# kai422/DAS3R

Measured on AMD Instinct MI355X. Metric: render fwd+bwd Msplats/s at 1080p, higher is better.
Workload: dtype f32; 1 GPU; 1M random splats, 1920x1080, SH degree 3, forward+backward (BASELINE.json configs[3], constant P); splats_per_gpu=1000000, splats_per_gpu_final=1000000, init_steps=30, sh_degree=3, num_rendered=2614506, api=GaussianRasterizer.forward + autograd backward (drop-in surface), parallelism=1 independent scenes, one per GPU

## Files before the change

das3r_amd/_lib.py:

```python
import ctypes as C
import os

_HERE = os.path.dirname(os.path.abspath(__file__))
LIB_PATH = os.path.join(_HERE, "libdas3r_hip.so")
ABI_VERSION = 16

ALLOC_FN = C.CFUNCTYPE(C.c_void_p, C.c_void_p, C.c_size_t)


class RasterArgs(C.Structure):
    _fields_ = [("P", C.c_int32), ("sh_degree", C.c_int32), ("M", C.c_int32), ("image_width", C.c_int32),
                ("image_height", C.c_int32), ("tanfovx", C.c_float), ("tanfovy", C.c_float), ("scale_modifier", C.c_float),
                ("bg", C.c_void_p), ("viewmatrix", C.c_void_p), ("projmatrix", C.c_void_p), ("campos", C.c_void_p),
                ("prefiltered", C.c_int32), ("debug", C.c_int32), ("capacity_hint", C.c_int64)]


class PreTransform(C.Structure):
    _fields_ = [("xyz", C.c_void_p), ("rot", C.c_void_p), ("scaling", C.c_void_p), ("opacity_raw", C.c_void_p), ("conf_flat", C.c_void_p),
                ("mask_index", C.c_void_p), ("R", C.c_void_p), ("t", C.c_void_p), ("Lq", C.c_void_p)]


class RasterIn(C.Structure):
    _fields_ = [("means3D", C.c_void_p), ("opacities", C.c_void_p), ("shs", C.c_void_p), ("colors_precomp", C.c_void_p),
                ("scales", C.c_void_p), ("rotations", C.c_void_p), ("cov3D_precomp", C.c_void_p), ("pre", C.POINTER(PreTransform))]


class RasterOut(C.Structure):
    _fields_ = [("out_color", C.c_void_p), ("radii", C.c_void_p), ("out_invdepth", C.c_void_p)]


class RasterSaved(C.Structure):
    _fields_ = [("geom", C.c_void_p), ("binning", C.c_void_p), ("img", C.c_void_p), ("num_rendered", C.c_int64), ("capacity", C.c_int64),
                ("check_word", C.c_void_p), ("check_tag", C.c_uint32), ("flags", C.c_uint32)]


class AdamSlot(C.Structure):
    _fields_ = [("param", C.c_void_p), ("exp_avg", C.c_void_p), ("exp_avg_sq", C.c_void_p), ("step_size", C.c_float), ("bc2_sqrt", C.c_float)]


class Chain(C.Structure):
    _fields_ = [("g_conf_flat", C.c_void_p), ("g_small", C.c_void_p), ("slots", C.POINTER(AdamSlot)), ("beta1", C.c_float), ("beta2", C.c_float),
                ("eps", C.c_float)]


class RasterGrads(C.Structure):
    _fields_ = [("dL_dmeans2D", C.c_void_p), ("dL_dopacities", C.c_void_p), ("dL_dmeans3D", C.c_void_p),
                ("dL_dshs", C.c_void_p), ("dL_dcolors_precomp", C.c_void_p), ("dL_dscales", C.c_void_p),
                ("dL_drotations", C.c_void_p), ("dL_dcov3D", C.c_void_p), ("scratch", C.c_void_p), ("chain", C.POINTER(Chain))]


class RasterLayout(C.Structure):
    _fields_ = [(n, C.c_size_t) for n in
                ("geom_bytes", "binning_bytes", "img_bytes", "depth_key", "xy", "conic_opacity", "rgbd", "splat_stride", "clamped",
                 "tiles_touched", "sorted_idx", "offsets", "point_list", "final_T", "n_contrib", "ranges")]


EXPORTS = ("das3r_raster_forward", "das3r_raster_backward", "das3r_raster_backward_depth", "das3r_raster_backward_depth_scratch_bytes", "das3r_raster_check", "das3r_raster_backward_scratch_bytes", "das3r_mark_visible", "das3r_knn3_workspace_bytes",
           "das3r_knn3_mean_dist2", "das3r_raster_get_layout", "das3r_abi_version", "das3r_last_error", "das3r_reload_switches", "das3r_get_stats",
           "das3r_raster_forget_shapes", "das3r_raster_learning",
           "das3r_profile_enable", "das3r_profile_report", "das3r_pretransform_forward", "das3r_pretransform_backward", "das3r_pose_matrices", "das3r_pose_chain",
           "das3r_adam_step", "das3r_adam_step_gated", "das3r_photometric_blocks", "das3r_photometric_forward", "das3r_photometric_backward",
           "das3r_has_experiments", "das3r_pair_counters", "das3r_debug_poison_lds", "das3r_debug_inject_fault", "das3r_debug_mutate",
           "das3r_pose_matrices_qt", "das3r_pose_chain_qt", "das3r_photometric_finish", "das3r_pretransform_backward_adam", "das3r_pretransform_pose_sums",
           "das3r_raster_count_live_pairs", "das3r_photometric_backward_finish", "das3r_pose_chain_qt_rearm", "das3r_ssim_map_forward", "das3r_ssim_map_backward")

_lib = None


def load():
    global _lib
    if _lib is not None:
        return _lib
    if not os.path.exists(LIB_PATH):
        raise RuntimeError(
            f"das3r_amd: HIP library not found at {LIB_PATH}. Build it with `python -c 'import __graft_entry__ as g; "
            f"g.build()'` or `make -C das3r_amd/csrc`. There is no CPU fallback.")
    L = C.CDLL(LIB_PATH)
    for name in EXPORTS:
        if not hasattr(L, name):
            raise RuntimeError(f"das3r_amd: {LIB_PATH} does not export {name}; rebuild it")
    L.das3r_abi_version.restype = C.c_int
    if L.das3r_abi_version() != ABI_VERSION:
        raise RuntimeError("das3r_amd: ABI version mismatch between the Python host layer and libdas3r_hip.so; rebuild")
    L.das3r_last_error.restype = C.c_char_p
    L.das3r_raster_forward.restype = C.c_int64
    L.das3r_raster_forward.argtypes = [C.POINTER(RasterArgs), C.POINTER(RasterIn), C.POINTER(RasterOut), ALLOC_FN, ALLOC_FN,
                                       ALLOC_FN, C.c_void_p, C.POINTER(RasterSaved), C.c_void_p]
    L.das3r_raster_backward.restype = C.c_int
    L.das3r_raster_backward.argtypes = [C.POINTER(RasterArgs), C.POINTER(RasterIn), C.POINTER(RasterSaved), C.c_void_p,
                                        C.POINTER(RasterGrads), C.c_void_p]
    L.das3r_raster_backward_scratch_bytes.restype = C.c_size_t
    L.das3r_raster_backward_depth.restype = C.c_int
    L.das3r_raster_backward_depth.argtypes = [C.POINTER(RasterArgs), C.POINTER(RasterIn), C.POINTER(RasterSaved), C.c_void_p, C.c_void_p,
                                              C.POINTER(RasterGrads), C.c_void_p]
    L.das3r_raster_backward_depth_scratch_bytes.restype = C.c_size_t
    L.das3r_raster_backward_depth_scratch_bytes.argtypes = [C.c_int64]
    L.das3r_raster_backward_scratch_bytes.argtypes = [C.c_int64]
    L.das3r_raster_check.restype = C.c_int
    L.das3r_raster_check.argtypes = [C.POINTER(RasterSaved), C.c_void_p]
    L.das3r_mark_visible.restype = C.c_int
    L.das3r_mark_visible.argtypes = [C.c_int32, C.c_void_p, C.c_void_p, C.c_void_p, C.c_void_p, C.c_void_p]
    L.das3r_knn3_workspace_bytes.restype = C.c_size_t
    L.das3r_knn3_workspace_bytes.argtypes = [C.c_int32]
    L.das3r_knn3_mean_dist2.restype = C.c_int
    L.das3r_knn3_mean_dist2.argtypes = [C.c_int32, C.c_void_p, C.c_void_p, C.c_void_p, C.c_void_p]
    L.das3r_pose_matrices.restype = C.c_int
    L.das3r_pose_matrices.argtypes = [C.c_void_p, C.c_void_p, C.c_void_p]
    L.das3r_pose_chain.restype = C.c_int
    L.das3r_pose_chain.argtypes = [C.c_void_p, C.c_void_p, C.c_void_p, C.c_void_p]
    L.das3r_pretransform_forward.restype = C.c_int
    L.das3r_pretransform_forward.argtypes = [C.c_int32] + [C.c_void_p] * 13 + [C.c_void_p]
    L.das3r_pretransform_backward.restype = C.c_int
    L.das3r_pretransform_backward.argtypes = [C.c_int32] + [C.c_void_p] * 18 + [C.c_void_p]
    L.das3r_pretransform_backward_adam.restype = C.c_int
    L.das3r_pretransform_backward_adam.argtypes = [C.c_int32] + [C.c_void_p] * 10 + [C.POINTER(AdamSlot), C.c_float, C.c_float, C.c_float, C.c_void_p]
    L.das3r_pretransform_pose_sums.restype = C.c_int
    L.das3r_pretransform_pose_sums.argtypes = [C.c_int32] + [C.c_void_p] * 7 + [C.c_void_p]
    L.das3r_photometric_blocks.restype = C.c_int64
    L.das3r_photometric_blocks.argtypes = [C.c_int32, C.c_int32]
    L.das3r_photometric_forward.restype = C.c_int
    L.das3r_photometric_forward.argtypes = [C.c_int32, C.c_int32, C.c_void_p, C.c_void_p, C.c_void_p, C.c_float, C.c_void_p, C.c_void_p, C.c_void_p]
    L.das3r_photometric_backward.restype = C.c_int
    L.das3r_photometric_backward.argtypes = [C.c_int32, C.c_int32, C.c_void_p, C.c_void_p, C.c_void_p, C.c_float, C.c_void_p, C.c_void_p,
                                             C.c_void_p, C.c_void_p, C.c_void_p]
    L.das3r_pose_matrices_qt.restype = C.c_int
    L.das3r_pose_matrices_qt.argtypes = [C.c_void_p, C.c_void_p, C.c_void_p, C.c_void_p]
    L.das3r_pose_chain_qt.restype = C.c_int
    L.das3r_pose_chain_qt.argtypes = [C.c_void_p, C.c_void_p, C.c_void_p, C.c_void_p, C.c_void_p]
    L.das3r_pose_chain_qt_rearm.restype = C.c_int
    L.das3r_pose_chain_qt_rearm.argtypes = [C.c_void_p, C.c_void_p, C.c_void_p, C.c_void_p, C.c_void_p, C.c_void_p, C.c_void_p]
    L.das3r_ssim_map_forward.restype = C.c_int
    L.das3r_ssim_map_forward.argtypes = [C.c_int32, C.c_int32, C.c_void_p, C.c_void_p, C.c_void_p, C.c_void_p, C.c_void_p, C.c_void_p]
    L.das3r_ssim_map_backward.restype = C.c_int
    L.das3r_ssim_map_backward.argtypes = [C.c_int32, C.c_int32, C.c_void_p, C.c_void_p, C.c_void_p, C.c_void_p, C.c_void_p, C.c_void_p, C.c_void_p]
    L.das3r_photometric_backward_finish.restype = C.c_int
    L.das3r_photometric_backward_finish.argtypes = [C.c_int32, C.c_int32, C.c_void_p, C.c_void_p, C.c_void_p, C.c_float, C.c_void_p, C.c_void_p,
                                                    C.c_void_p, C.c_void_p, C.c_void_p, C.c_void_p, C.c_void_p]
    L.das3r_photometric_finish.restype = C.c_int
    L.das3r_photometric_finish.argtypes = [C.c_int32, C.c_int32, C.c_void_p, C.c_float, C.c_void_p, C.c_void_p]
    L.das3r_adam_step_gated.restype = C.c_int
    L.das3r_adam_step_gated.argtypes = [C.c_int32, C.c_void_p, C.c_float, C.c_float, C.c_float, C.c_void_p, C.c_float, C.c_void_p, C.c_void_p]
    L.das3r_adam_step.restype = C.c_int
    L.das3r_adam_step.argtypes = [C.c_int32, C.c_void_p, C.c_float, C.c_float, C.c_float, C.c_void_p]
    L.das3r_raster_get_layout.restype = C.c_int
    L.das3r_raster_get_layout.argtypes = [C.c_int32, C.c_int64, C.c_int32, C.c_int32, C.POINTER(RasterLayout)]
    _lib = L
    return L


def reload_switches():
    L = load()
    L.das3r_reload_switches.restype = None
    L.das3r_reload_switches.argtypes = []
    L.das3r_reload_switches()


def has_experiments():
    L = load()
# ... 110 lines not shown
```

das3r_amd/csrc/api.hip:

```cpp
#include <stdarg.h>
#include <string.h>

#include <vector>

#include "common.h"
#include <algorithm>

namespace das3r {

static thread_local char g_err[512] = "";

void set_error(const char *fmt, ...) {
    va_list ap;
    va_start(ap, fmt);
    vsnprintf(g_err, sizeof(g_err), fmt, ap);
    va_end(ap);
}

struct ProfRec {
    const char *name;
    hipEvent_t start, stop;
};
static bool g_prof_on = false;
static std::vector<ProfRec> g_prof;
bool profile_enabled() { return g_prof_on; }
static std::vector<hipEvent_t> g_event_pool;
static hipEvent_t pooled_event() {
    if (!g_event_pool.empty()) { hipEvent_t e = g_event_pool.back(); g_event_pool.pop_back(); return e; }
    hipEvent_t e = nullptr;
    return hipEventCreate(&e) == hipSuccess ? e : nullptr;
}
void profile_begin(const char *name, hipStream_t s) {
    ProfRec r;
    r.name = name;
    r.start = pooled_event();
    r.stop = pooled_event();
    if (!r.start || !r.stop) return;
    (void)hipEventRecord(r.start, s);
    g_prof.push_back(r);
}
void profile_end(hipStream_t s) {
    if (!g_prof.empty()) (void)hipEventRecord(g_prof.back().stop, s);
}

static Switches g_sw;
static bool g_sw_loaded = false;
static int g_inject_fault = 0;
static int g_mutate = 0;
static void load_switches() {
    Switches w;
    memset(&w, 0, sizeof(w));
    auto env = [](const char *k) -> const char * { const char *e = getenv(k); return (e && e[0]) ? e : nullptr; };
    const char *e;
#ifdef DAS3R_EXPERIMENTS
    if ((e = env("DAS3R_SORT_IPL"))) { const int v = atoi(e); w.sort_ipl = (v == 4 || v == 8 || v == 16) ? v : 0; }
    w.sort_classic = (e = env("DAS3R_SORT")) && e[0] == 'c';
    w.no_sh_stage = getenv("DAS3R_NO_SH_STAGE") != nullptr;
    if ((e = env("DAS3R_ABLATE"))) { w.ablate_set = true; w.ablate = atoi(e); }
    if ((e = env("DAS3R_BWD_PAD_LDS"))) w.bwd_pad_lds = atoi(e);
    if ((e = env("DAS3R_FWD_PAD_LDS"))) w.fwd_pad_lds = atoi(e);
    if ((e = env("DAS3R_SCAN_ITEMS"))) { const int v = atoi(e); w.scan_items = (v == 1 || v == 2 || v == 4 || v == 8 || v == 16) ? v : 0; }
    w.fwd_no_prefetch = (e = env("DAS3R_FWD_PREFETCH")) && e[0] == '0';
#endif
    w.rect_upstream = (e = env("DAS3R_RECT")) && e[0] == 'u';
    w.verbose = env("DAS3R_VERBOSE") != nullptr;
    if ((e = env("DAS3R_BINNING"))) w.binning = e[0] == 'l' ? 1 : (e[0] == 'r' ? -1 : (e[0] == 's' ? (strchr(e, '3') ? 3 : 2) : 0));
    w.capacity_exact = (e = env("DAS3R_CAPACITY")) && e[0] == 'e';
    w.fused_emit_off = (e = env("DAS3R_FUSED_EMIT")) && e[0] == '0';
    w.tile_lpt_off = (e = env("DAS3R_TILE_LPT")) && e[0] == '0';
    if ((e = env("DAS3R_RENDER"))) w.render_fwd = e[0] == 'q' ? 1 : (e[0] == 'r' ? 2 : (e[0] == 'l' ? 3 : (e[0] == 's' ? 4 : (e[0] == 'f' ? 5 : 0))));
    if ((e = env("DAS3R_RENDER_BWD"))) {
        w.render_bwd = e[0] == 'd' ? 1 : (e[0] == 'm' ? 2 : (strncmp(e, "stream", 6) == 0 ? 5 : (e[0] == 's' ? 3 : (e[0] == 'b' ? 6 : (e[0] == 'f' ? 7 : 0)))));
        if (w.render_bwd == 6) {
            const char *d = e;
            while (*d && (*d < '0' || *d > '9')) d++;
            w.render_bwd_mb = *d ? atoi(d) : 128;
            const char *pp = strchr(e, 'p');
            w.render_bwd_pix = pp ? atoi(pp + 1) : 0;
            const char *po = strchr(e, 'o');
            w.render_bwd_occ = po ? atoi(po + 1) : 5;
        }
        if (w.render_bwd == 7) {
            const char *d = e;
            while (*d && (*d < '0' || *d > '9')) d++;
            w.render_bwd_mb = *d ? atoi(d) : 128;
            w.render_bwd_pix = strchr(e, 'q') ? 9 : (strchr(e, 's') ? 8 : 0);
        }
        if (w.render_bwd == 3) {
            const char *d = e;
            while (*d && (*d < '0' || *d > '9')) d++;
            w.render_bwd_mb = (*d ? atoi(d) : 256) + (strncmp(e, "scana", 5) == 0 ? 1000 : 0);
        }
    }
    if ((e = env("DAS3R_BWD_REDUCE"))) { w.bwd_reduce_set = true; w.bwd_reduce_shfl = e[0] == 's'; }
    w.tickets = -1;
    if ((e = env("DAS3R_TICKETS"))) w.tickets = e[0] == 'a' ? 0 : (e[0] == 'n' ? 1 << 30 : ((e[0] >= '1' && e[0] <= '9') ? atoi(e) : -1));
    w.deterministic = (e = env("DAS3R_DETERMINISTIC")) && e[0] != '0';
    w.bwd_buckets = -1;
    if ((e = env("DAS3R_BWD_BUCKETS"))) w.bwd_buckets = atoi(e);
    w.tile_strip = 8;
    w.tile_chunk = -1;
    if ((e = env("DAS3R_TILE_CHUNK"))) { const int v = atoi(e); w.tile_chunk = (v >= 0 && v <= 64 && (v & (v - 1)) == 0) ? v : -1; }
    if ((e = env("DAS3R_TILE_STRIP"))) w.tile_strip = std::max(0, std::min(63, atoi(e)));
    w.inject_fault = g_inject_fault;
    w.mutate = g_mutate;
    g_sw = w;
    __atomic_store_n(&g_sw_loaded, true, __ATOMIC_RELEASE);
}
const Switches &switches() {
    if (!__atomic_load_n(&g_sw_loaded, __ATOMIC_ACQUIRE)) load_switches();
    return g_sw;
}

constexpr int MAX_DEVICES = 64;
static int g_threads_on_device[MAX_DEVICES] = {};
struct ThreadRegistrar {
    bool on[MAX_DEVICES] = {};
    void add(int dev) {
        if (!on[dev]) { on[dev] = true; __atomic_fetch_add(&g_threads_on_device[dev], 1, __ATOMIC_RELAXED); }
    }
    ~ThreadRegistrar() {
        for (int d = 0; d < MAX_DEVICES; d++)
            if (on[d]) __atomic_fetch_sub(&g_threads_on_device[d], 1, __ATOMIC_RELAXED);
    }
};
static thread_local ThreadRegistrar g_registrar;
bool grid_is_resident(int nblocks) {
    const int forced = switches().tickets;
    int dev = 0;
    if (hipGetDevice(&dev) != hipSuccess || dev < 0 || dev >= MAX_DEVICES) return false;
    const bool shared = __atomic_load_n(&g_threads_on_device[dev], __ATOMIC_RELAXED) > 1;
    if (forced >= 0) {
        static bool warned = false;
        if (shared && forced > 0 && !__atomic_exchange_n(&warned, true, __ATOMIC_RELAXED))
            fprintf(stderr, "[das3r] DAS3R_TICKETS is set to a bound while several host threads render on device %d: ticket-free chained "
                            "kernels are only safe when a grid has the device to itself\n", dev);
        return nblocks <= forced;
    }
    if (shared) return false;
    static thread_local int cached_dev = -1, cached_limit = 0;
    if (dev != cached_dev) {
        int cus = 0;
        if (hipDeviceGetAttribute(&cus, hipDeviceAttributeMultiprocessorCount, dev) != hipSuccess) return false;
        cached_dev = dev;
        cached_limit = cus * 2;
    }
    return nblocks <= cached_limit;
}

int sort_ipl_override() { return switches().sort_ipl; }
#ifdef DAS3R_EXPERIMENTS
bool use_onesweep() { return !switches().sort_classic; }
#else
bool use_onesweep() { return true; }
#endif
bool use_tight_rect() { return !switches().rect_upstream; }

void compute_layout(int P, int64_t I, int W, int H, Layout *L) {
    memset(L, 0, sizeof(*L));
    const size_t Pn = P > 0 ? (size_t)P : 1, In = I > 0 ? (size_t)I : 1;
    L->capacity = I;
    L->tiles_x = (W + TILE_X - 1) / TILE_X;
    L->tiles_y = (H + TILE_Y - 1) / TILE_Y;
    L->ntiles = L->tiles_x * L->tiles_y;
    L->tbits = tile_bits(L->ntiles);
    L->tile_passes = (L->tbits + 7) / 8;
    L->dbits = 0;
    L->kbits = L->tbits;
    L->kshift = 0;
    L->part_passes = L->tile_passes;
    L->chunksP = sort_num_chunks(P);
    L->chunksI = sort_num_chunks(I);
    size_t o = 0;
    auto take = [&](size_t b) { size_t r = o; o += align_up(b); return r; };
    L->g_keyA = take(4 * Pn);
    L->g_keyB = take(4 * Pn);
    L->g_valA = take(4 * Pn);
    L->g_valB = take(4 * Pn);
    L->pub.sorted_idx = L->g_valA;
    L->pub.depth_key = L->g_keyA;
    L->pub.xy = take(16 * SPLAT_REC * Pn);
    L->pub.conic_opacity = L->pub.xy + 16;
    L->pub.rgbd = L->pub.xy + 32;
    L->pub.splat_stride = 16 * SPLAT_REC;
    L->pub.clamped = take(Pn);
    L->pub.tiles_touched = take(4 * Pn);
    L->pub.offsets = take(4 * Pn);
    L->g_hist = take(4 * (size_t)RADIX_SIZE * (size_t)(L->chunksP > 0 ? L->chunksP : 1));
    L->g_totals = take(4 * RADIX_SIZE);
    L->g_blocksums = take(4 * (size_t)div_up((int64_t)Pn, 4096));
    L->g_count = take(256);
    L->g_off_by_gid = take(4 * Pn);
    L->g_rect = take(4 * Pn);
    L->g_dhist = take(4 * 256);
    L->g_ghist = take(4 * 4 * RADIX_SIZE);
    L->g_ticket = take(256);
    L->g_status = take(onesweep_status_bytes((int64_t)Pn, 4));
    L->g_scan_status = take(scan_status_bytes((int)Pn));
    L->g_ctrl_bytes = o - L->g_ghist;
    L->pub.geom_bytes = o;
    o = 0;
    L->b_keyA = take(4 * In);
    L->b_keyB = take(4 * In);
    L->b_valA = take(4 * In);
    L->b_valB = take(4 * In);
    L->b_hist = take(4 * (size_t)RADIX_SIZE * (size_t)(L->chunksI > 0 ? L->chunksI : 1));
    L->b_totals = take(4 * RADIX_SIZE);
    L->b_gid_of = take(4 * In);
    L->b_slot = take(4 * In);
    L->b_e2 = take(4 * In);
    L->b_ghist = take(4 * 4 * RADIX_SIZE);
    L->b_ticket = take(256);
    L->b_status = take(onesweep_status_bytes((int64_t)In, L->tile_passes + 1));
    L->b_ctrl_bytes = o - L->b_ghist;
    L->b_ckpt = take(((size_t)In / BUCKET + (size_t)(L->ntiles > 0 ? L->ntiles : 1) + 2) * 256 * 16);
    L->pub.binning_bytes = o;
    const size_t npix_d = (size_t)W * (size_t)H;
    L->d_ckpt = take(((size_t)In / BUCKET + (size_t)(L->ntiles > 0 ? L->ntiles : 1) + 2) * 256 * 16);
    L->d_recs = take(16 * SPLAT_REC * Pn);
    L->d_dpix = take(4 * 3 * (npix_d > 0 ? npix_d : 1));
    L->d_bg = take(16);
    L->d_dz = take(4 * Pn);
    L->d_bytes = o;
    L->pub.point_list = (L->tile_passes & 1) ? L->b_valB : L->b_valA;
    o = 0;
    const size_t npix = (size_t)W * (size_t)H;
    L->pub.final_T = take(4 * (npix > 0 ? npix : 1));
    L->pub.n_contrib = take(4 * (npix > 0 ? npix : 1));
    L->pub.ranges = take(8 * (size_t)(L->ntiles > 0 ? L->ntiles : 1));
    L->i_order = take(4 * (size_t)(L->ntiles > 0 ? L->ntiles : 1));
    L->pub.img_bytes = o;
}

static bool dhist_slots(hipStream_t s, uint32_t **use, uint32_t **next) {
    struct Slot { int dev; hipStream_t stream; uint32_t *buf; uint32_t turn; };
    static thread_local std::vector<Slot> slots;
    int dev = 0;
    if (hipGetDevice(&dev) != hipSuccess) return false;
    Slot *e = nullptr;
    for (auto &c : slots)
        if (c.dev == dev && c.stream == s) e = &c;
    if (!e) {
        uint32_t *buf = nullptr;
        if (hipMalloc((void **)&buf, 2 * 256 * sizeof(uint32_t)) != hipSuccess) return false;
        if (hipMemsetAsync(buf, 0, 2 * 256 * sizeof(uint32_t), s) != hipSuccess) return false;
        slots.push_back(Slot{dev, s, buf, 0u});
        e = &slots.back();
    }
    e->turn++;
    *use = e->buf + 256 * (e->turn & 1u);
    *next = e->buf + 256 * ((e->turn + 1u) & 1u);
    return true;
}

static int validate(const das3r_raster_args *a, const das3r_raster_in *in) {
    if (!a || !in) { set_error("null args"); return DAS3R_ERR_INVALID_ARG; }
    if (a->P < 0 || a->image_width <= 0 || a->image_height <= 0) { set_error("bad extents P=%d W=%d H=%d", a->P, a->image_width, a->image_height); return DAS3R_ERR_INVALID_ARG; }
    if ((int64_t)((a->image_width + TILE_X - 1) / TILE_X) * ((a->image_height + TILE_Y - 1) / TILE_Y) >= (1ll << 22)) {
        set_error("image of %d x %d pixels has 2^22 tiles or more", a->image_width, a->image_height);
        return DAS3R_ERR_INVALID_ARG;
    }
    if (a->P == 0) return DAS3R_OK;
    if (!a->bg || !a->viewmatrix || !a->projmatrix || !a->campos) { set_error("bg/viewmatrix/projmatrix/campos must be device pointers"); return DAS3R_ERR_INVALID_ARG; }
    if (in->pre) {
        const das3r_pretransform *p = in->pre;
        if (!p->xyz || !p->rot || !p->scaling || !p->opacity_raw || !p->conf_flat || !p->R || !p->t || !p->Lq) { set_error("das3r_raster_in.pre: xyz / rot / scaling / opacity_raw / conf_flat / R / t / Lq are required"); return DAS3R_ERR_INVALID_ARG; }
        if (in->cov3D_precomp) { set_error("das3r_raster_in.pre excludes cov3D_precomp"); return DAS3R_ERR_INVALID_ARG; }
    } else if (!in->means3D || !in->opacities) { set_error("means3D/opacities are required"); return DAS3R_ERR_INVALID_ARG; }
    if ((in->shs != nullptr) == (in->colors_precomp != nullptr)) { set_error("Please provide excatly one of either SHs or precomputed colors!"); return DAS3R_ERR_INVALID_ARG; }
    const bool sr = in->pre != nullptr || (in->scales != nullptr && in->rotations != nullptr);
    if ((!in->pre && (in->scales != nullptr) != (in->rotations != nullptr)) || sr == (in->cov3D_precomp != nullptr)) {
        set_error("Please provide exactly one of either scale/rotation pair or precomputed 3D covariance!");
        return DAS3R_ERR_INVALID_ARG;
    }
    if (in->shs) {
        if (a->sh_degree < 0 || a->sh_degree > 3) { set_error("sh_degree must be 0..3 (got %d)", a->sh_degree); return DAS3R_ERR_INVALID_ARG; }
        if (a->M < (a->sh_degree + 1) * (a->sh_degree + 1) || a->M > 16) { set_error("M=%d incompatible with sh_degree=%d (need (D+1)^2 <= M <= 16)", a->M, a->sh_degree); return DAS3R_ERR_INVALID_ARG; }
    }
    if (a->tanfovx <= 0.f || a->tanfovy <= 0.f) { set_error("tanfov must be positive"); return DAS3R_ERR_INVALID_ARG; }
    return DAS3R_OK;
}

}

using namespace das3r;

extern "C" int das3r_abi_version(void) { return DAS3R_ABI_VERSION; }
extern "C" void das3r_reload_switches(void) { load_switches(); }
extern "C" void das3r_debug_inject_fault(uint32_t bits) {
    g_inject_fault = (int)bits;
    load_switches();
}
extern "C" void das3r_debug_mutate(uint32_t what) {
    g_mutate = (int)what;
    load_switches();
}
extern "C" const char *das3r_last_error(void) { return g_err; }

extern "C" int das3r_raster_get_layout(int32_t P, int64_t num_rendered, int32_t W, int32_t H, das3r_raster_layout *out) {
    if (!out || P < 0 || num_rendered < 0 || W <= 0 || H <= 0) { set_error("das3r_raster_get_layout: invalid argument"); return DAS3R_ERR_INVALID_ARG; }
    Layout L;
    compute_layout(P, num_rendered, W, H, &L);
    *out = L.pub;
    return DAS3R_OK;
}

struct Mailbox {
    volatile uint32_t *host = nullptr;
    uint32_t *dev = nullptr;
    uint32_t seq = 0;
};
constexpr uint32_t CHECK_SLOTS = 16, CHECK_WORD0 = 16, MAILBOX_BYTES = 4 * (CHECK_WORD0 + 2 * CHECK_SLOTS);
constexpr uint32_t CROWDED16 = 23u * 16u;
struct Verdict { int P, W, H; int64_t last_I, peak_I; int radix_left, backoff; uint32_t gen; int seg_extra; bool last_seg; bool fine; uint32_t forwards; uint32_t clean; uint32_t longest; };
struct PerDevice {
    Mailbox mb;
    uint32_t pending[CHECK_SLOTS] = {};
    unsigned long long *arrive_ring = nullptr;
    Verdict verdict = {0, 0, 0, -1, 0, 0, 64, 0};
    bool pending_fine = false, pending_valid = false;
    uint32_t pending_forwards = 0;
    char *emit_ring = nullptr;
    bool emit_ring_dirty = false;
    uint32_t emit_last_tag = 0;
};
static int per_device(PerDevice **out) {
    static thread_local PerDevice state[MAX_DEVICES];
    int dev = 0;
    HIP_TRY(hipGetDevice(&dev));
    if (dev < 0 || dev >= MAX_DEVICES) { set_error("device ordinal %d not supported", dev); return DAS3R_ERR_INVALID_ARG; }
    PerDevice &T = state[dev];
    g_registrar.add(dev);
    if (!T.mb.host) {
        uint32_t *h = nullptr;
        HIP_TRY(hipHostMalloc((void **)&h, MAILBOX_BYTES, hipHostMallocMapped));
        memset(h, 0, MAILBOX_BYTES);
        HIP_TRY(hipHostGetDevicePointer((void **)&T.mb.dev, h, 0));
        T.mb.host = h;
    }
    *out = &T;
    return DAS3R_OK;
}
static int mailbox_wait(Mailbox *mb, int idx, uint32_t tag, hipStream_t s) {
    for (long spins = 0; spins < 200000000L; spins++) {
        if (__atomic_load_n(&mb->host[idx], __ATOMIC_ACQUIRE) == tag) return DAS3R_OK;
        __builtin_ia32_pause();
        if ((spins & 0xFFFFF) == 0xFFFFF && hipStreamQuery(s) != hipErrorNotReady) break;
    }
    HIP_TRY(hipStreamSynchronize(s));
    if (__atomic_load_n(&mb->host[idx], __ATOMIC_ACQUIRE) == tag) return DAS3R_OK;
    set_error("the device never delivered the result of this forward to the host mailbox");
    return DAS3R_ERR_HIP;
}

static unsigned long long g_stats[4] = {0, 0, 0, 0};
static void stat_add(int i) { __atomic_fetch_add(&g_stats[i], 1ull, __ATOMIC_RELAXED); }
static int examine_check_slot(volatile uint32_t *slot, uint32_t tag, bool wait, hipStream_t s) {
    uint32_t seen = __atomic_load_n(&slot[1], __ATOMIC_ACQUIRE);
    if (seen != tag && wait) {
        for (long spins = 0; spins < 200000000L && seen != tag; spins++) {
            __builtin_ia32_pause();
            seen = __atomic_load_n(&slot[1], __ATOMIC_ACQUIRE);
            if ((spins & 0xFFFFF) == 0xFFFFF && hipStreamQuery(s) != hipErrorNotReady) break;
        }
        if (seen != tag) {
            HIP_TRY(hipStreamSynchronize(s));
            seen = __atomic_load_n(&slot[1], __ATOMIC_ACQUIRE);
        }
    }
    if (seen != tag) return 1;
    const uint32_t all_flags = slot[0], flags = all_flags & ~16u;
    if (all_flags & 0x80000000u) return DAS3R_OK;
    stat_add(1);
    if (all_flags & 16u) stat_add(2);
    if (flags) stat_add(3);
    if ((all_flags & 16u) && switches().verbose) fprintf(stderr, "das3r: a look-back poll needed the read-modify-write path\n");
    if (flags) {
        slot[0] = all_flags | 0x80000000u;
        set_error("a forward's binning failed its self-check (flags 0x%x); its output is invalid", flags);
        return DAS3R_ERR_HIP;
    }
    return DAS3R_OK;
}

extern "C" int das3r_raster_check(const das3r_raster_saved *saved, das3r_stream_t stream) {
    if (!saved) { set_error("das3r_raster_check: null saved state"); return DAS3R_ERR_INVALID_ARG; }
    if (!saved->check_word || !saved->check_tag) return DAS3R_OK;
    const int r = examine_check_slot((volatile uint32_t *)saved->check_word, saved->check_tag, true, (hipStream_t)stream);
    return r < 0 ? r : DAS3R_OK;
}

extern "C" int das3r_raster_forget_shapes(void) {
    PerDevice *T = nullptr;
    int r = per_device(&T);
    if (r) return r;
    const uint32_t gen = T->verdict.gen;
    T->verdict = Verdict{0, 0, 0, -1, 0, 0, 64, gen};
    return DAS3R_OK;
}

extern "C" int das3r_raster_learning(int32_t set, uint32_t state[2]) {
    if (!state) { set_error("das3r_raster_learning: invalid argument"); return DAS3R_ERR_INVALID_ARG; }
    PerDevice *T = nullptr;
    int r = per_device(&T);
    if (r) return r;
    if (!set) {
        state[0] = T->verdict.fine ? 1u : 0u;
        state[1] = T->verdict.forwards;
        return DAS3R_OK;
    }
    const uint32_t gen = T->verdict.gen;
    T->verdict = Verdict{0, 0, 0, -1, 0, 0, 64, gen};
    T->pending_fine = state[0] != 0u;
    T->pending_forwards = state[1];
    T->pending_valid = true;
    return DAS3R_OK;
}

extern "C" void das3r_get_stats(uint64_t out[4]) {
    for (int i = 0; i < 4; i++) out[i] = (uint64_t)__atomic_load_n(&g_stats[i], __ATOMIC_RELAXED);
}

extern "C" int64_t das3r_raster_forward(const das3r_raster_args *a, const das3r_raster_in *in, const das3r_raster_out *out,
                                        das3r_alloc_fn alloc_geom, das3r_alloc_fn alloc_binning, das3r_alloc_fn alloc_img,
                                        void *user, das3r_raster_saved *saved, das3r_stream_t stream) {
    hipStream_t s = (hipStream_t)stream;
    stat_add(0);
    int rc = validate(a, in);
    if (rc) return rc;
    if (!out || !out->out_color || (a->P > 0 && !out->radii) || !alloc_geom || !alloc_binning || !alloc_img || !saved) {
        set_error("das3r_raster_forward: null output/allocator");
        return DAS3R_ERR_INVALID_ARG;
    }
    if (out->out_invdepth && switches().render_fwd == 4) {
        set_error("das3r_raster_forward: DAS3R_RENDER=slices has no inverse-depth form (das3r_raster_out.out_invdepth)");
        return DAS3R_ERR_INVALID_ARG;
    }
    const int P = a->P, W = a->image_width, H = a->image_height;
    const bool depth = out->out_invdepth != nullptr;
    Layout L;
    compute_layout(P, 0, W, H, &L);
    saved->geom = alloc_geom(user, L.pub.geom_bytes);
    saved->img = alloc_img(user, L.pub.img_bytes);
    saved->binning = nullptr;
    saved->num_rendered = 0;
    saved->capacity = 0;
    saved->check_word = nullptr;
    saved->check_tag = 0;
    saved->flags = 0;
    if (!saved->geom || !saved->img) { set_error("scratch allocation failed (geom %zu B, img %zu B)", L.pub.geom_bytes, L.pub.img_bytes); return DAS3R_ERR_ALLOC; }
    if (P == 0) {
        HIP_TRY(hipMemsetAsync(out->out_color, 0, sizeof(float) * 3 * (size_t)W * H, s));
        if (out->out_invdepth) HIP_TRY(hipMemsetAsync(out->out_invdepth, 0, sizeof(float) * (size_t)W * H, s));
        HIP_TRY(hipMemsetAsync(saved->img + L.pub.ranges, 0, 8 * (size_t)L.ntiles, s));
        saved->binning = alloc_binning(user, 256);
        return 0;
    }
    PerDevice *T = nullptr;
    if ((rc = per_device(&T))) return rc;
    Mailbox *mb = &T->mb;
    auto check_slot = [&](uint32_t i, bool wait) -> int {
        if (!T->pending[i]) return DAS3R_OK;
        const int r = examine_check_slot(mb->host + CHECK_WORD0 + 2 * i, T->pending[i], wait, s);
        if (r == 1) return DAS3R_OK;
        T->pending[i] = 0;
        return r;
    };
    for (uint32_t i = 0; i < CHECK_SLOTS; i++)
        if ((rc = check_slot(i, false))) return rc;
    uint32_t late_tag = 0;
    unsigned long long *&arrive_ring = T->arrive_ring;
    constexpr uint32_t ARRIVE_SLOTS = 16, ARRIVE_WORDS = 8 + 64 * 8;
    if (!arrive_ring) {
        HIP_TRY(hipMalloc((void **)&arrive_ring, ARRIVE_SLOTS * ARRIVE_WORDS * sizeof(unsigned long long)));
        HIP_TRY(hipMemsetAsync(arrive_ring, 0, ARRIVE_SLOTS * ARRIVE_WORDS * sizeof(unsigned long long), s));
        HIP_TRY(hipStreamSynchronize(s));
    }
    Verdict &verdict = T->verdict;
    constexpr int64_t LOCAL_AVG = 384;
    const uint32_t too_long = mb->host[10];
    if (too_long) mb->host[10] = 0;
    const uint32_t want_bits = mb->host[11];
    if (want_bits) mb->host[11] = 0;
    if (verdict.P != P || verdict.W != W || verdict.H != H) {
        const uint32_t gen = verdict.gen + 1u ? verdict.gen + 1u : 1u;
        verdict = Verdict{P, W, H, -1, 0, 0, 64, gen};
        if (T->pending_valid) {
            verdict.fine = T->pending_fine;
            verdict.forwards = T->pending_forwards;
            T->pending_valid = false;
        }
    }
    const bool decide_fine = (verdict.forwards++ & 511u) == 0u;
    auto next_gen = [&]() { verdict.gen = verdict.gen + 1u ? verdict.gen + 1u : 1u; };
    if (verdict.last_I < 0) {
    } else if (too_long == verdict.gen && !(verdict.last_seg && verdict.seg_extra == 0 && L.tile_passes < 3 && seg_dbits(L, L.tile_passes + 1) > 0)) {
        if (verdict.clean >= 256u) verdict.backoff = 64;
        verdict.radix_left = verdict.backoff;
        if (verdict.backoff < 4096) verdict.backoff *= 2;
        verdict.clean = 0;
        next_gen();
    } else if (too_long == verdict.gen || want_bits == verdict.gen) {
        verdict.seg_extra = 1;
        next_gen();
    }
    const int forced = switches().binning;
    bool local = use_onesweep() && (forced == 1 || (forced == 0 && verdict.radix_left == 0 && verdict.last_I <= LOCAL_AVG * L.ntiles));
    constexpr int64_t SEG_AVG = 384;
    const int seg_passes = L.tile_passes + ((forced == 3 || (forced == 0 && verdict.seg_extra)) ? 1 : 0);
    const int seg_bits = (use_onesweep() && seg_passes <= 3) ? seg_dbits(L, seg_passes) : 0;
    bool seg = !local && seg_bits > 0 && (forced >= 2 || (forced == 0 && verdict.radix_left == 0 && verdict.last_I >= 0 &&
                                                           (verdict.last_I >> std::min(seg_bits, 20)) <= SEG_AVG * L.ntiles));
    const uint32_t *seg_dhist = nullptr;
    auto apply_seg = [&]() {
        L.dhist_ptr = seg_dhist;
        if (seg) {
            L.dbits = seg_bits;
            L.kbits = L.tbits + seg_bits;
            L.kshift = std::min(16, 32 - L.kbits);
            L.part_passes = seg_passes;
        }
    };
    verdict.last_seg = seg;
    if (local || seg) verdict.clean++;
    if (forced == 0 && verdict.radix_left > 0) verdict.radix_left--;
    const uint32_t count_tag = ++mb->seq ? mb->seq : ++mb->seq;
    unsigned long long *arrive = arrive_ring + (size_t)(count_tag % ARRIVE_SLOTS) * ARRIVE_WORDS;
    auto bin_and_render = [&](int64_t cap, bool local_order, bool ctrl_zeroed, uint32_t *count_out = nullptr, uint32_t count_out_tag = 0,
                              uint32_t *emit_slot = nullptr ) -> int {
        int r;
        const bool fused_scan = use_onesweep();
        const bool seg = L.dbits > 0;
        if (!emit_slot) {
            if (fused_scan) {
                if ((r = launch_binning_scan_emit(P, cap, out->radii, saved->geom, saved->binning, L, ctrl_zeroed, count_out, count_out_tag, a->debug != 0,
                                                  s, local_order || seg))) return r;
            } else if ((r = launch_scan(P, saved->geom, L, nullptr, 0, a->debug != 0, s))) return r;
        }
        uint32_t *host_late = nullptr;
        if (cap > 0) {
            late_tag = ++mb->seq ? mb->seq : ++mb->seq;
            const uint32_t slot = late_tag % CHECK_SLOTS;
            if ((r = check_slot(slot, true))) return r;
            T->pending[slot] = late_tag;
            host_late = mb->dev + CHECK_WORD0 + 2 * slot;
            saved->check_word = (void *)(mb->host + CHECK_WORD0 + 2 * slot);
            saved->check_tag = late_tag;
        }
        uint32_t *dead_keys = nullptr;
        if ((r = launch_binning(P, cap, W, H, out->radii, saved->geom, saved->binning, saved->img, L, fused_scan, host_late, late_tag,
                                a->debug != 0, s, &dead_keys, emit_slot, mb->dev + 10, verdict.gen))) return r;
        LocalBin lb = {(float4 *)(saved->binning + L.b_ckpt), nullptr, nullptr, nullptr, nullptr, verdict.gen, (uint32_t)(P - 1), (uint32_t)cap};
        if (decide_fine && cap > 0 && use_quad_lanes(L, lb)) {
            const uint32_t tag = ++mb->seq ? mb->seq : ++mb->seq;
            if ((r = launch_list_skew(saved->img, saved->binning, saved->geom, L, (uint32_t)cap, (uint32_t)(P - 1), mb->dev + 13, tag, a->debug != 0, s))) return r;
            if ((r = mailbox_wait(mb, 14, tag, s))) return r;
            const int64_t longest = (int64_t)mb->host[13], mean = (verdict.last_I > 0 ? verdict.last_I : cap) / std::max(L.ntiles, 1);
            verdict.longest = (uint32_t)longest;
            const uint32_t crowd16 = mb->host[15];
            verdict.fine = (longest > mean + (mean * 4) / 5 && longest >= 4096) || crowd16 >= CROWDED16;
            if (switches().verbose) fprintf(stderr, "[das3r] tile lists: longest %lld, mean %lld, %.1f of 64 consecutive entries in one quadrant -> %s kernels\n", (long long)longest,
                                            (long long)mean, crowd16 / 16.0, verdict.fine ? "2x2-region" : "block");
        }
        lb.prefer_regions = verdict.fine;
        lb.tile_order = nullptr;
        if (verdict.fine && cap > 0 && use_quad_lanes(L, lb) && L.ntiles <= 1024 && !switches().tile_lpt_off && (switches().render_fwd == 0 || switches().render_fwd == 5)) {
            if ((r = launch_tile_lpt(saved->img, L, (uint32_t)cap, a->debug != 0, s))) return r;
            lb.tile_order = (const uint32_t *)(saved->img + L.i_order);
        }
        if (verdict.fine && cap > 0 && use_quad_lanes(L, lb)) {
            const uint32_t hint = std::min<uint32_t>(63u, verdict.longest / (uint32_t)BUCKET + 2u);
            saved->flags |= 1u | (hint << 8);
        }
        if (local_order && cap > 0) {
            lb.point_list = (uint32_t *)(saved->binning + L.pub.point_list);
            lb.slot_list = (uint32_t *)(saved->binning + L.b_slot);
            lb.keys = dead_keys;
            lb.host_flag = mb->dev + 10;
        }
        return launch_render_forward(a, in->colors_precomp, out->out_color, saved->geom, saved->binning, saved->img, L, lb, s, out->out_invdepth,
                                     depth ? (float4 *)(saved->binning + L.d_ckpt) : nullptr);
    };
    auto prefiltered_ok = [&]() -> int {
        if (!a->prefiltered || mb->host[12] != count_tag) return DAS3R_OK;
        set_error("Point is filtered although prefiltered is set. This shouldn't happen!");
        return DAS3R_ERR_INVALID_ARG;
    };
    int64_t I, cap;
    if ((local || seg) && verdict.last_I >= 0 && a->capacity_hint != -1 && !switches().capacity_exact) {
        cap = std::max(verdict.last_I + verdict.last_I / 4, verdict.peak_I + verdict.peak_I / 20) + 4096;
        if (cap > (int64_t)0x7FFFFF00) cap = (int64_t)0x7FFFFF00;
        compute_layout(P, cap, W, H, &L);
        apply_seg();
        saved->binning = alloc_binning(user, depth ? L.d_bytes : L.pub.binning_bytes);
        if (!saved->binning) { set_error("scratch allocation failed (binning %zu B)", L.pub.binning_bytes); return DAS3R_ERR_ALLOC; }
        char *&emit_ring = T->emit_ring;
        bool &emit_ring_dirty = T->emit_ring_dirty;
        uint32_t &emit_last_tag = T->emit_last_tag;
        constexpr size_t EMIT_SLOT_BYTES = sizeof(uint32_t) * EMIT_SLOT_WORDS + sizeof(unsigned long long) * EMIT_STATUS_GRANULES;
        const bool fused_emit = local && grid_is_resident(div_up(P, 256)) && !switches().fused_emit_off;
        uint32_t *emit_slot = nullptr;
        if (fused_emit) {
            if (!emit_ring) {
                HIP_TRY(hipMalloc((void **)&emit_ring, ARRIVE_SLOTS * EMIT_SLOT_BYTES));
                emit_ring_dirty = true;
            }
            if (emit_ring_dirty || count_tag < emit_last_tag) {
                HIP_TRY(hipMemsetAsync(emit_ring, 0, ARRIVE_SLOTS * EMIT_SLOT_BYTES, s));
                emit_ring_dirty = false;
            }
            emit_last_tag = count_tag;
            emit_slot = (uint32_t *)(emit_ring + (size_t)(count_tag % ARRIVE_SLOTS) * EMIT_SLOT_BYTES);
            const EmitArgs em = {(unsigned long long *)(emit_slot + EMIT_SLOT_WORDS), count_tag, emit_slot + 64, emit_slot,
                                 (uint32_t *)(saved->binning + L.b_keyA), (uint32_t *)(saved->binning + L.b_gid_of),
                                 (uint32_t *)(saved->geom + L.g_off_by_gid), (uint32_t)cap, L.tbits, (uint32_t *)(saved->geom + L.g_count), mb->dev};
            emit_ring_dirty = true;
            if ((rc = launch_preprocess(a, in, out->radii, saved->geom, saved->img, saved->binning + L.b_ghist, L.b_ctrl_bytes, L, nullptr, mb->dev,
                                        count_tag, s, &em))) return rc;
            if ((rc = bin_and_render(cap, true, true, nullptr, 0, emit_slot))) return rc;
            emit_ring_dirty = false;
        } else {
            uint32_t *dhist = nullptr, *dhist_next = nullptr;
            if (seg && !dhist_slots(s, &dhist, &dhist_next)) {
                dhist = (uint32_t *)(saved->geom + L.g_dhist);
                HIP_TRY(hipMemsetAsync(dhist, 0, 4 * 256, s));
            }
            seg_dhist = dhist;
            apply_seg();
            if ((rc = launch_preprocess(a, in, out->radii, saved->geom, saved->img, saved->binning + L.b_ghist, L.b_ctrl_bytes, L, nullptr, mb->dev,
                                        count_tag, s, nullptr, dhist, dhist_next))) return rc;
            if ((rc = bin_and_render(cap, local, true, mb->dev, count_tag))) return rc;
        }
        if ((rc = mailbox_wait(mb, 2, count_tag, s))) return rc;
        if ((rc = prefiltered_ok())) return rc;
        I = (int64_t)mb->host[0];
        if (I > (int64_t)0x7FFFFF00) { set_error("num_rendered %lld exceeds 2^31", (long long)I); return DAS3R_ERR_OVERFLOW; }
        verdict.last_I = I;
        verdict.peak_I = std::max(I, verdict.peak_I - verdict.peak_I / 1024);
        if (I > cap) {
            cap = I;
            compute_layout(P, cap, W, H, &L);
            saved->binning = alloc_binning(user, depth ? L.d_bytes : L.pub.binning_bytes);
            if (!saved->binning) { set_error("scratch allocation failed (binning %zu B)", L.pub.binning_bytes); return DAS3R_ERR_ALLOC; }
            apply_seg();
            HIP_TRY(hipMemsetAsync(saved->geom + L.g_ghist, 0, L.g_ctrl_bytes, s));
            HIP_TRY(hipMemsetAsync(saved->img + L.pub.ranges, 0, 8 * (size_t)L.ntiles, s));
            if ((rc = bin_and_render(cap, local, false))) return rc;
        }
    } else {
        uint32_t *dhist = nullptr, *dhist_next = nullptr;
        if (seg && !dhist_slots(s, &dhist, &dhist_next)) {
            dhist = (uint32_t *)(saved->geom + L.g_dhist);
            HIP_TRY(hipMemsetAsync(dhist, 0, 4 * 256, s));
        }
        seg_dhist = dhist;
        if ((rc = launch_preprocess(a, in, out->radii, saved->geom, saved->img, nullptr, 0, L, arrive, mb->dev, count_tag, s, nullptr, dhist, dhist_next))) return rc;
        if (!local && !seg && (rc = launch_depth_sort(P, saved->geom, L, 0, nullptr, 0, a->debug != 0, s))) return rc;
        if ((rc = mailbox_wait(mb, 2, count_tag, s))) return rc;
        if ((rc = prefiltered_ok())) return rc;
        I = cap = (int64_t)mb->host[0];
        if (cap > (int64_t)0x7FFFFF00) { set_error("num_rendered %lld exceeds 2^31", (long long)cap); return DAS3R_ERR_OVERFLOW; }
        verdict.last_I = I;
        verdict.peak_I = std::max(I, verdict.peak_I - verdict.peak_I / 1024);
        if (local && forced == 0 && I > LOCAL_AVG * L.ntiles) {
            local = false;
            if ((rc = launch_depth_sort(P, saved->geom, L, 0, nullptr, 0, a->debug != 0, s))) return rc;
        }
        compute_layout(P, cap, W, H, &L);
        apply_seg();
        saved->binning = alloc_binning(user, depth ? L.d_bytes : L.pub.binning_bytes);
        if (!saved->binning) { set_error("scratch allocation failed (binning %zu B)", L.pub.binning_bytes); return DAS3R_ERR_ALLOC; }
        if (!local && !seg && (rc = launch_depth_sort(P, saved->geom, L, 1, saved->binning + L.b_ghist, L.b_ctrl_bytes, a->debug != 0, s))) return rc;
        if ((rc = bin_and_render(cap, local, !local && !seg))) return rc;
    }
    if (a->debug && late_tag && (rc = check_slot(late_tag % CHECK_SLOTS, true))) return rc;
    saved->num_rendered = I;
    saved->capacity = cap;
    if (depth) saved->flags |= DEPTH_SAVED_FLAG;
    return I;
}

extern "C" int das3r_raster_backward(const das3r_raster_args *a, const das3r_raster_in *in, const das3r_raster_saved *saved,
                                     const float *dL_dpix, const das3r_raster_grads *g, das3r_stream_t stream) {
    hipStream_t s = (hipStream_t)stream;
    int rc = validate(a, in);
    if (rc) return rc;
    const int P = a->P;
    if (P == 0) return DAS3R_OK;
    const bool chained = g && g->chain;
    if (!saved || !saved->geom || !saved->img || !dL_dpix || !g || !g->dL_dmeans2D || (!chained && (!g->dL_dopacities || !g->dL_dmeans3D)) ||
        (saved && saved->num_rendered > 0 && !g->scratch)) {
        set_error("das3r_raster_backward: null saved state / gradient buffer");
        return DAS3R_ERR_INVALID_ARG;
    }
    const bool has_sh = in->shs != nullptr, has_cov = in->cov3D_precomp != nullptr;
    if ((has_sh && !g->dL_dshs) || (!has_sh && !g->dL_dcolors_precomp) || (has_cov && !g->dL_dcov3D) ||
        (!has_cov && !chained && (!g->dL_dscales || !g->dL_drotations))) {
        set_error("das3r_raster_backward: gradient buffer missing for a provided input");
        return DAS3R_ERR_INVALID_ARG;
    }
    if ((rc = das3r_raster_check(saved, stream))) return rc;
    Layout L;
    compute_layout(P, saved->capacity > 0 ? saved->capacity : saved->num_rendered, a->image_width, a->image_height, &L);
    float *partial = g->scratch;
    bool quad_rows = false;
    if (saved->num_rendered > 0) {
        if (!saved->binning) { set_error("das3r_raster_backward: binning buffer missing"); return DAS3R_ERR_INVALID_ARG; }
        if ((rc = launch_render_backward(a, dL_dpix, saved->geom, saved->binning, saved->img, L, partial, s, &quad_rows, saved->num_rendered, saved->flags))) return rc;
    }
    return launch_preprocess_backward(a, in, saved->geom, saved->binning, L, g, partial, s, quad_rows);
}

extern "C" int das3r_raster_backward_depth(const das3r_raster_args *a, const das3r_raster_in *in, const das3r_raster_saved *saved,
                                           const float *dL_dpix, const float *dL_dinvdepth, const das3r_raster_grads *g, das3r_stream_t stream) {
    hipStream_t s = (hipStream_t)stream;
    int rc = validate(a, in);
    if (rc) return rc;
    const int P = a->P;
    if (P == 0) return DAS3R_OK;
    const bool chained = g && g->chain;
    if (!saved || !saved->geom || !saved->img || !dL_dpix || !dL_dinvdepth || !g || !g->dL_dmeans2D || (!chained && (!g->dL_dopacities || !g->dL_dmeans3D)) ||
        (saved->num_rendered > 0 && !g->scratch)) {
        set_error("das3r_raster_backward_depth: null saved state / upstream gradient / gradient buffer");
        return DAS3R_ERR_INVALID_ARG;
    }
    if (!(saved->flags & DEPTH_SAVED_FLAG)) {
        set_error("das3r_raster_backward_depth: the saved state is not that of a forward with out_invdepth (das3r_raster_saved.flags bit 1 is clear)");
        return DAS3R_ERR_INVALID_ARG;
    }
    const bool has_sh = in->shs != nullptr, has_cov = in->cov3D_precomp != nullptr;
    if ((has_sh && !g->dL_dshs) || (!has_sh && !g->dL_dcolors_precomp) || (has_cov && !g->dL_dcov3D) ||
        (!has_cov && !chained && (!g->dL_dscales || !g->dL_drotations))) {
        set_error("das3r_raster_backward_depth: gradient buffer missing for a provided input");
        return DAS3R_ERR_INVALID_ARG;
    }
    const int kind = switches().render_bwd;
    if (kind == 2 || kind == 3 || kind == 5) {
        set_error("das3r_raster_backward_depth: DAS3R_RENDER_BWD=%s has no inverse-depth form", kind == 3 ? "scan" : (kind == 2 ? "mfma" : "stream"));
        return DAS3R_ERR_INVALID_ARG;
    }
    if ((rc = das3r_raster_check(saved, stream))) return rc;
    Layout L;
    compute_layout(P, saved->capacity > 0 ? saved->capacity : saved->num_rendered, a->image_width, a->image_height, &L);
    float *partial = g->scratch;
    const float *dz = nullptr;
    bool quad_rows = false;
    if (saved->num_rendered > 0) {
        if (!saved->binning) { set_error("das3r_raster_backward_depth: binning buffer missing"); return DAS3R_ERR_INVALID_ARG; }
        const size_t c = L.capacity > 0 ? (size_t)L.capacity : 1;
        float *partial_depth = (float *)((char *)g->scratch + align_up(c * 9 * sizeof(float) + 16));
        if ((rc = launch_render_backward(a, dL_dpix, saved->geom, saved->binning, saved->img, L, partial, s, &quad_rows, saved->num_rendered, saved->flags))) return rc;
        if ((rc = launch_depth_pass_inputs(P, a->image_width * a->image_height, saved->geom, L, saved->binning, dL_dinvdepth, s, a->debug != 0))) return rc;
        Layout Ld = L;
        Ld.pub.xy = L.d_recs;
        Ld.pub.conic_opacity = L.d_recs + 16;
        Ld.pub.rgbd = L.d_recs + 32;
        Ld.b_ckpt = L.d_ckpt;
        das3r_raster_args ad = *a;
        ad.bg = (const float *)(saved->binning + L.d_bg);
        bool quad_rows_d = false;
        if ((rc = launch_render_backward(&ad, (const float *)(saved->binning + L.d_dpix), saved->binning, saved->binning, saved->img, Ld, partial_depth, s,
                                         &quad_rows_d, saved->num_rendered, saved->flags))) return rc;
        float *dzw = (float *)(saved->binning + L.d_dz);
        if ((rc = launch_depth_fold(P, saved->geom, L, partial, partial_depth, dzw, s, a->debug != 0))) return rc;
        dz = dzw;
    }
    return launch_preprocess_backward(a, in, saved->geom, saved->binning, L, g, partial, s, quad_rows, dz);
}

extern "C" size_t das3r_raster_backward_depth_scratch_bytes(int64_t capacity) {
    const size_t c = capacity > 0 ? (size_t)capacity : 1;
    return align_up(c * 9 * sizeof(float) + 16) + c * 9 * sizeof(float) + 16;
}

extern "C" size_t das3r_raster_backward_scratch_bytes(int64_t capacity) {
    const size_t c = capacity > 0 ? (size_t)capacity : 1;
#ifdef DAS3R_EXPERIMENTS
    if (switches().render_bwd == 5) return std::max(c * 9 * sizeof(float) + 16, stream_scratch_bytes(capacity));
#endif
    return c * 9 * sizeof(float) + 16;
}

extern "C" int das3r_has_experiments(void) {
#ifdef DAS3R_EXPERIMENTS
    return 1;
#else
    return 0;
#endif
}

extern "C" int das3r_mark_visible(int32_t P, const float *means3D, const float *viewmatrix, const float *projmatrix,
                                  uint8_t *present, das3r_stream_t stream) {
    (void)projmatrix;
    if (P < 0 || (P > 0 && (!means3D || !viewmatrix || !present))) { set_error("das3r_mark_visible: invalid argument"); return DAS3R_ERR_INVALID_ARG; }
    return launch_mark_visible(P, means3D, viewmatrix, present, (hipStream_t)stream);
}

__global__ void __launch_bounds__(1024) poison_lds_kernel(uint32_t pattern, uint32_t *sink, int words) {
    extern __shared__ uint32_t lds_words[];
    for (int i = threadIdx.x; i < words; i += 1024) lds_words[i] = pattern;
    __syncthreads();
    if (lds_words[(threadIdx.x * 37) % words] != pattern) *sink = 1u;
}
extern "C" int das3r_debug_poison_lds(uint32_t pattern, das3r_stream_t stream) {
    static uint32_t *sinks[MAX_DEVICES] = {};
    int dev = 0, lds_bytes = 0;
    HIP_TRY(hipGetDevice(&dev));
    if (dev < 0 || dev >= MAX_DEVICES) { set_error("device ordinal %d not supported", dev); return DAS3R_ERR_INVALID_ARG; }
    HIP_TRY(hipDeviceGetAttribute(&lds_bytes, hipDeviceAttributeMaxSharedMemoryPerBlock, dev));
    const int words = lds_bytes / 4 - 64;
    if (words <= 0) { set_error("das3r_debug_poison_lds: no LDS"); return DAS3R_ERR_HIP; }
    if (!sinks[dev]) HIP_TRY(hipMalloc((void **)&sinks[dev], 4));
    HIP_TRY(hipFuncSetAttribute((const void *)poison_lds_kernel, hipFuncAttributeMaxDynamicSharedMemorySize, words * 4));
    hipLaunchKernelGGL(poison_lds_kernel, dim3(1024), dim3(1024), words * 4, (hipStream_t)stream, pattern, sinks[dev], words);
    HIP_TRY(hipGetLastError());
    return DAS3R_OK;
}

static unsigned long long *g_pairs = nullptr;
static int g_pairs_dev = -1;
namespace das3r {
unsigned long long *pair_counters() {
    if (!g_pairs) return nullptr;
    int dev = -1;
    return (hipGetDevice(&dev) == hipSuccess && dev == g_pairs_dev) ? g_pairs : nullptr;
}
}
extern "C" int das3r_pair_counters(int enable, uint64_t out[4]) {
    if (enable) {
        int dev = 0;
        HIP_TRY(hipGetDevice(&dev));
        if (g_pairs && dev != g_pairs_dev) { set_error("das3r_pair_counters: already counting on device %d", g_pairs_dev); return DAS3R_ERR_INVALID_ARG; }
        if (!g_pairs) HIP_TRY(hipMalloc((void **)&g_pairs, (4 + PHASE_WORDS * PHASE_COPIES) * sizeof(unsigned long long)));
        g_pairs_dev = dev;
        HIP_TRY(hipMemset(g_pairs, 0, (4 + PHASE_WORDS * PHASE_COPIES) * sizeof(unsigned long long)));
        HIP_TRY(hipDeviceSynchronize());
        return DAS3R_OK;
    }
    if (g_pairs) {
        HIP_TRY(hipDeviceSynchronize());
        if (out) HIP_TRY(hipMemcpy(out, g_pairs, 4 * sizeof(unsigned long long), hipMemcpyDeviceToHost));
        HIP_TRY(hipFree(g_pairs));
        g_pairs = nullptr;
    } else if (out) {
        out[0] = out[1] = out[2] = out[3] = 0;
    }
    return DAS3R_OK;
}

extern "C" int das3r_raster_count_live_pairs(const das3r_raster_args *a, const das3r_raster_saved *saved, uint64_t out[2], das3r_stream_t stream) {
    if (!a || !saved || !out) { set_error("das3r_raster_count_live_pairs: null argument"); return DAS3R_ERR_INVALID_ARG; }
    out[0] = out[1] = 0;
    if (a->P == 0 || saved->num_rendered <= 0) return DAS3R_OK;
    if (!saved->geom || !saved->binning || !saved->img) { set_error("das3r_raster_count_live_pairs: saved buffers missing"); return DAS3R_ERR_INVALID_ARG; }
    hipStream_t s = (hipStream_t)stream;
    Layout L;
    compute_layout(a->P, saved->capacity > 0 ? saved->capacity : saved->num_rendered, a->image_width, a->image_height, &L);
    unsigned long long *dev = nullptr;
    HIP_TRY(hipMalloc((void **)&dev, 2 * sizeof(unsigned long long)));
    int rc = DAS3R_OK;
    if (hipMemsetAsync(dev, 0, 2 * sizeof(unsigned long long), s) != hipSuccess) rc = DAS3R_ERR_HIP;
    if (!rc) rc = launch_count_live_pairs(a, saved->geom, saved->binning, saved->img, L, dev, s);
    if (!rc && (hipStreamSynchronize(s) != hipSuccess || hipMemcpy(out, dev, 2 * sizeof(unsigned long long), hipMemcpyDeviceToHost) != hipSuccess)) {
        set_error("das3r_raster_count_live_pairs: device error");
        rc = DAS3R_ERR_HIP;
    }
    (void)hipFree(dev);
    return rc;
}

#ifdef DAS3R_EXPERIMENTS
static unsigned long long *g_trace = nullptr;
namespace das3r { unsigned long long *wg_trace() { return g_trace; } }
extern "C" int das3r_debug_wg_trace(int enable, uint64_t *out) {
    const size_t words = (size_t)TRACE_PASSES * TRACE_WGS * TRACE_STAMPS;
    if (enable) {
        if (!g_trace) HIP_TRY(hipMalloc((void **)&g_trace, words * 8));
        HIP_TRY(hipMemset(g_trace, 0, words * 8));
        HIP_TRY(hipDeviceSynchronize());
        return DAS3R_OK;
    }
    if (g_trace) {
        HIP_TRY(hipDeviceSynchronize());
        if (out) HIP_TRY(hipMemcpy(out, g_trace, words * 8, hipMemcpyDeviceToHost));
        HIP_TRY(hipFree(g_trace));
        g_trace = nullptr;
    }
    return DAS3R_OK;
}
extern "C" int das3r_debug_phase_clocks(uint64_t out[16]) {
    for (int i = 0; i < PHASE_WORDS; i++) out[i] = 0;
    if (!g_pairs) return DAS3R_OK;
    HIP_TRY(hipDeviceSynchronize());
    std::vector<unsigned long long> all(PHASE_WORDS * PHASE_COPIES);
    HIP_TRY(hipMemcpy(all.data(), g_pairs + 4, all.size() * sizeof(unsigned long long), hipMemcpyDeviceToHost));
    for (size_t i = 0; i < all.size(); i++) out[i % PHASE_WORDS] += all[i];
// ... 31 lines not shown
```

das3r_amd/csrc/common.h:

```cpp
#pragma once
#include <hip/hip_runtime.h>
#include <stdint.h>
#include <stdio.h>

#include "../../include/das3r_raster.h"
#include "pretransform_math.h"

#define TILE_X 16
#define TILE_Y 16
#define TILE_PIX 256
#define WAVE 64
#define NEAR_PLANE 0.001f

namespace das3r {

void set_error(const char *fmt, ...);

struct Switches {
    int sort_ipl;
    bool sort_classic;
    bool rect_upstream;
    bool verbose;
    int binning;
    bool capacity_exact;
    bool fused_emit_off;
    bool no_sh_stage;
    int render_fwd;
    int render_bwd;
    int render_bwd_mb;
    int tile_chunk;
    int scan_items;
    bool deterministic;
    int render_bwd_occ;
    bool tile_lpt_off;
    int render_bwd_pix;
    bool bwd_reduce_set, bwd_reduce_shfl;
    bool ablate_set;
    int ablate;
    int tickets;
    int bwd_pad_lds, fwd_pad_lds;
    int bwd_buckets;
    int inject_fault;
    int mutate;
    bool fwd_no_prefetch;
    int tile_strip;
};
const Switches &switches();

#define HIP_TRY(expr)                                                                          \
    do {                                                                                       \
        hipError_t _e = (expr);                                                                \
        if (_e != hipSuccess) {                                                                \
            das3r::set_error("%s failed: %s (%s:%d)", #expr, hipGetErrorString(_e), __FILE__, __LINE__); \
            return DAS3R_ERR_HIP;                                                              \
        }                                                                                      \
    } while (0)

#define KERNEL_CHECK(stream, debug, name)                                                      \
    do {                                                                                       \
        hipError_t _e = hipGetLastError();                                                     \
        if (_e == hipSuccess && (debug)) _e = hipStreamSynchronize(stream);                    \
        if (_e != hipSuccess) {                                                                \
            das3r::set_error("kernel %s failed: %s", name, hipGetErrorString(_e));             \
            return DAS3R_ERR_HIP;                                                              \
        }                                                                                      \
    } while (0)

bool profile_enabled();
void profile_begin(const char *name, hipStream_t s);
void profile_end(hipStream_t s);
struct ProfTimer {
    hipStream_t s;
    bool on;
    ProfTimer(const char *name, hipStream_t stream) : s(stream), on(profile_enabled()) {
        if (on) profile_begin(name, s);
    }
    ~ProfTimer() {
        if (on) profile_end(s);
    }
};

unsigned long long *pair_counters();
constexpr int PHASE_WORDS = 16, PHASE_COPIES = 64;
#ifdef DAS3R_EXPERIMENTS
#define PHASE_BEGIN()                                                                      \
    __shared__ unsigned long long phase_w_[8];                                             \
    unsigned long long phase_t_ = 0ull;                                                    \
    if (pairs != nullptr && threadIdx.x == 0) {                                            \
        for (int k_ = 0; k_ < 8; k_++) phase_w_[k_] = 0ull;                                \
        phase_t_ = clock64();                                                              \
    }
#define PHASE_MARK(k)                                                                      \
    if (pairs != nullptr && threadIdx.x == 0) {                                            \
        const unsigned long long now_ = clock64();                                         \
        phase_w_[(k) & 7] += now_ - phase_t_;                                              \
        phase_t_ = now_;                                                                   \
    }
#define PHASE_END(base)                                                                    \
    if (pairs != nullptr && threadIdx.x == 0)                                              \
        for (int k_ = 0; k_ < 8; k_++) atomicAdd(pairs + 4 + (blockIdx.x % PHASE_COPIES) * PHASE_WORDS + (base) + k_, phase_w_[k_]);
constexpr int TRACE_WGS = 16384, TRACE_PASSES = 8, TRACE_STAMPS = 8;
unsigned long long *wg_trace();
static inline unsigned long long *pairs_or_trace() {
    unsigned long long *p = pair_counters();
    if (p == nullptr && wg_trace() != nullptr) p = reinterpret_cast<unsigned long long *>(reinterpret_cast<uintptr_t>(wg_trace()) | 1u);
    return p;
}
#define DECODE_PAIRS_OR_TRACE(arg)                                                                                         \
    unsigned long long *const trace = (reinterpret_cast<uintptr_t>(arg) & 1u)                                              \
                                          ? reinterpret_cast<unsigned long long *>(reinterpret_cast<uintptr_t>(arg) & ~(uintptr_t)1) \
                                          : nullptr;                                                                       \
    unsigned long long *const pairs = trace ? nullptr : (arg);
#define WG_STAMP(k)                                                                                   \
    if (trace != nullptr && threadIdx.x == 0 && s_block < (uint32_t)TRACE_WGS)                        \
        trace[((size_t)(shift >> 3) * TRACE_WGS + s_block) * TRACE_STAMPS + (k)] = wall_clock64();
#define SCAN_STAMP(k)                                                                                 \
    if (wg_trace_ptr != nullptr && threadIdx.x == 0 && s_block < (uint32_t)TRACE_WGS)                 \
        wg_trace_ptr[((size_t)(TRACE_PASSES - 1) * TRACE_WGS + s_block) * TRACE_STAMPS + (k)] = wall_clock64();
#define BLK_STAMP(ptr, r, k)                                                                          \
    if ((ptr) != nullptr && threadIdx.x == 0 && blockIdx.x < (uint32_t)TRACE_WGS)                      \
        (ptr)[((size_t)(r) * TRACE_WGS + blockIdx.x) * TRACE_STAMPS + (k)] = wall_clock64();
#define PAIRS_ARG pairs_or_trace()
#else
#define PAIRS_ARG pair_counters()
#define PHASE_MARK(k)
#define PHASE_BEGIN()
#define PHASE_END(base)
#define WG_STAMP(k)
#define SCAN_STAMP(k)
#define BLK_STAMP(ptr, r, k)
#endif

#define DAS3R_LAUNCH(kernel, grid, block, shmem, stream, ...)                \
    do {                                                                     \
        das3r::ProfTimer _pt(#kernel, stream);                               \
        hipLaunchKernelGGL(kernel, grid, block, shmem, stream, __VA_ARGS__); \
    } while (0)

static inline size_t align_up(size_t x, size_t a = 256) { return (x + a - 1) / a * a; }
static inline int div_up(int64_t a, int64_t b) { return (int)((a + b - 1) / b); }

constexpr int RADIX_BITS = 8;
constexpr int RADIX_SIZE = 1 << RADIX_BITS;
constexpr int SORT_WAVES_PER_BLOCK = 4;
int sort_ipl_override();
static inline int sort_items_per_lane(int64_t n) {
    const int o = sort_ipl_override();
    return o ? o : (n >= (int64_t)(1 << 21) ? 16 : (n >= (1 << 17) ? 8 : 4));
}
static inline int sort_num_chunks(int64_t n) { return n == 0 ? 0 : div_up(n, (int64_t)WAVE * sort_items_per_lane(n)); }
__host__ __device__ static inline int tile_digit_width(int tbits) {
    const int passes = (tbits + 7) / 8;
    return passes > 0 ? (tbits + passes - 1) / passes : 8;
}
static inline int tile_bits(int ntiles) {
    int b = 0;
    while ((1 << b) < ntiles) b++;
    return b < 1 ? 1 : b;
}

constexpr int BUCKET = 1024;
constexpr int SPLAT_REC = 4;

constexpr uint32_t DEPTH_SAVED_FLAG = 2u;
struct Layout {
    das3r_raster_layout pub;
    size_t g_keyA, g_keyB, g_valA, g_valB, g_hist, g_totals, g_blocksums, g_count, g_off_by_gid, g_rect;
    size_t b_keyA, b_keyB, b_valA, b_valB, b_hist, b_totals, b_gid_of, b_slot;
    size_t b_e2;
    size_t b_ckpt;
    size_t d_ckpt, d_recs, d_dpix, d_bg, d_dz, d_bytes;
    size_t g_ghist, g_ticket, g_status, g_scan_status, g_ctrl_bytes;
    int64_t capacity;
    size_t b_ghist, b_ticket, b_status, b_ctrl_bytes;
    int tiles_x, tiles_y, ntiles, tbits, tile_passes;
    int chunksP, chunksI;
    int dbits, kbits, kshift;
    int part_passes;
    size_t g_dhist;
    const uint32_t *dhist_ptr;
    size_t i_order;
};
static inline int seg_dbits(const Layout &L, int passes) { return 8 * (passes < 3 ? passes : 3) - L.tbits; }

struct LocalBin {
    float4 *ckpt;
    uint32_t *point_list, *slot_list;
    uint32_t *keys;
    uint32_t *host_flag;
    uint32_t flag_value;
    uint32_t last_g, cap;
    bool prefer_regions;
    const uint32_t *tile_order;
};
void compute_layout(int P, int64_t I, int W, int H, Layout *L);

struct EmitArgs {
    unsigned long long *status;
    uint32_t tag;
    uint32_t *ghist;
    uint32_t *err;
    uint32_t *tile_keys, *gids, *off_by_gid;
    uint32_t cap;
    int tbits;
    uint32_t *count;
    uint32_t *count_out;
};
constexpr int EMIT_SLOT_WORDS = 64 + 4 * 256;
constexpr int EMIT_STATUS_GRANULES = 1024;

int launch_preprocess(const das3r_raster_args *a, const das3r_raster_in *in, int32_t *radii, char *geom, char *img, char *binning_ctrl,
                      size_t binning_ctrl_bytes, const Layout &L, unsigned long long *arrive, uint32_t *host_out, uint32_t tag,
                      hipStream_t s, const EmitArgs *emit = nullptr, uint32_t *dhist = nullptr, uint32_t *dhist_next = nullptr);
int launch_mark_visible(int P, const float *means3D, const float *viewmatrix, uint8_t *present, hipStream_t s);
int launch_depth_sort(int P, char *geom, const Layout &L, int part, char *binning_ctrl, size_t binning_ctrl_bytes, bool debug, hipStream_t s);
int launch_scan(int P, char *geom, const Layout &L, uint32_t *host_out, uint32_t tag, bool debug, hipStream_t s, bool index_order = false);
int launch_scan_emit(int P, int64_t cap, const int32_t *radii, char *geom, char *binning, const Layout &L, uint32_t *host_out, uint32_t tag,
                     bool debug, hipStream_t s, bool index_order = false);
size_t scan_status_bytes(int P);
int launch_binning_scan_emit(int P, int64_t I, const int32_t *radii, char *geom, char *binning, const Layout &L, bool ctrl_zeroed,
                             uint32_t *host_out, uint32_t tag, bool debug, hipStream_t s, bool index_order = false);
size_t onesweep_status_bytes(int64_t n, int passes);
int launch_onesweep_depth_sort(int P, char *geom, const Layout &L, int part, uint32_t *zero_ptr, uint32_t zero_words, bool debug,
                               hipStream_t s);
int launch_onesweep_partition(int64_t cap, char *geom, char *binning, const Layout &L, uint32_t **keys_final, bool debug, hipStream_t s,
                              uint32_t *ghist_override = nullptr, uint32_t *err_override = nullptr);
bool use_row_private(int64_t instances, int ntiles);
bool use_quad_lanes(const Layout &L, const LocalBin &lb);
inline PreXform pre_xform(const das3r_raster_in *in) {
    PreXform x = {nullptr, nullptr, nullptr, nullptr, nullptr, nullptr, nullptr, nullptr, nullptr};
    if (in && in->pre) {
        const das3r_pretransform *p = in->pre;
        x = PreXform{p->xyz, p->rot, p->scaling, p->opacity_raw, p->conf_flat, p->mask_index, p->R, p->t, p->Lq};
    }
    return x;
}
int launch_render_forward_regions(const das3r_raster_args *a, float *out_color, char *geom, char *binning, char *img, const Layout &L, const LocalBin &lb,
                                  hipStream_t s, float *out_invdepth, float4 *dckpt);
int launch_tile_lpt(char *img, const Layout &L, uint32_t cap, bool debug, hipStream_t s);
int launch_list_skew(const char *img, const char *binning, const char *geom, const Layout &L, uint32_t cap, uint32_t last_g, uint32_t *mailbox_words, uint32_t tag,
                     bool debug, hipStream_t s);
int launch_render_forward_slices(const das3r_raster_args *a, float *out_color, char *geom, char *binning, char *img, const Layout &L, const LocalBin &lb,
                                 hipStream_t s);
int launch_render_forward_lanes(const das3r_raster_args *a, float *out_color, char *geom, char *binning, char *img, const Layout &L,
                                const LocalBin &lb, hipStream_t s, float *out_invdepth, float4 *dckpt);
int launch_render_forward_rows(const das3r_raster_args *a, float *out_color, char *geom, char *binning, char *img, const Layout &L,
                               const LocalBin &lb, hipStream_t s, float *out_invdepth, float4 *dckpt);
int launch_render_backward_mfma(const das3r_raster_args *a, const float *dL_dpix, char *geom, char *binning, char *img, const Layout &L,
                                float *partial, hipStream_t s);
size_t stream_scratch_bytes(int64_t capacity);
int launch_render_backward_stream(const das3r_raster_args *a, const float *dL_dpix, char *geom, char *binning, char *img, const Layout &L,
                                  float *scratch, hipStream_t s);
int launch_render_backward_scan(const das3r_raster_args *a, const float *dL_dpix, char *geom, char *binning, char *img, const Layout &L,
                                float *partial, int mb, int slices, hipStream_t s);
int launch_render_backward_blk(const das3r_raster_args *a, const float *dL_dpix, char *geom, char *binning, char *img, const Layout &L,
                               float *partial, int mb, int slices, hipStream_t s);
int launch_render_backward_regions(const das3r_raster_args *a, const float *dL_dpix, char *geom, char *binning, char *img, const Layout &L,
                               float *partial, int mb, int slices, hipStream_t s);
constexpr int LOCAL_MAX = 1024;
bool grid_is_resident(int nblocks);
bool use_onesweep();
bool use_tight_rect();
int launch_binning(int P, int64_t I, int W, int H, const int32_t *radii, char *geom, char *binning, char *img, const Layout &L,
                   bool fused_scan, uint32_t *host_late, uint32_t tag, bool debug, hipStream_t s, uint32_t **dead_keys = nullptr,
                   uint32_t *emit_slot = nullptr ,
                   uint32_t *seg_host_flag = nullptr, uint32_t seg_flag_value = 0 );
int launch_segment_sort(int64_t cap, const uint32_t *n_ptr, const uint32_t *keys_final, int fbits, uint32_t *point_list, uint32_t *slot_list,
                        const uint32_t *depth_key, uint32_t last_g, uint32_t *scratch_keys, uint32_t *host_flag, uint32_t flag_value, bool debug,
                        hipStream_t s, int dbits, uint2 *ranges, const uint32_t *err, uint32_t *host_late, uint32_t tag, uint32_t inject);
int launch_render_forward(const das3r_raster_args *a, const float *colors_precomp, float *out_color, char *geom, char *binning,
                          char *img, const Layout &L, const LocalBin &lb, hipStream_t s, float *out_invdepth ,
                          float4 *dckpt );
int launch_depth_pass_inputs(int P, int npix, const char *geom, const Layout &L, char *binning, const float *dL_dinvdepth, hipStream_t s, bool debug);
int launch_depth_fold(int P, const char *geom, const Layout &L, float *partial, const float *partial_depth, float *dz, hipStream_t s, bool debug);
int launch_render_backward(const das3r_raster_args *a, const float *dL_dpix, char *geom, char *binning, char *img, const Layout &L,
                           float *partial, hipStream_t s, bool *quad_rows, int64_t num_rendered, uint32_t fwd_flags );
int launch_count_live_pairs(const das3r_raster_args *a, char *geom, char *binning, char *img, const Layout &L, unsigned long long *out, hipStream_t s);
int launch_preprocess_backward(const das3r_raster_args *a, const das3r_raster_in *in, char *geom, char *binning, const Layout &L,
                               const das3r_raster_grads *g, const float *partial, hipStream_t s, bool quad_rows, const float *dz = nullptr );

#ifdef __HIPCC__
__device__ __forceinline__ int lane_id() { return __lane_id(); }

template <int CTRL, int ROW_MASK>
__device__ __forceinline__ float dpp_step(float v) {
    int moved = __builtin_amdgcn_update_dpp(0, __float_as_int(v), CTRL, ROW_MASK, 0xf, true);
    return v + __int_as_float(moved);
}
__device__ __forceinline__ float wave_sum_to_lane63(float v) {
    v = dpp_step<0x111, 0xf>(v);
    v = dpp_step<0x112, 0xf>(v);
    v = dpp_step<0x114, 0xf>(v);
    v = dpp_step<0x118, 0xf>(v);
    v = dpp_step<0x142, 0xa>(v);
    v = dpp_step<0x143, 0xc>(v);
    return v;
}
__device__ __forceinline__ float row_sum_to_lane15(float v) {
    v = dpp_step<0x111, 0xf>(v);
    v = dpp_step<0x112, 0xf>(v);
    v = dpp_step<0x114, 0xf>(v);
    v = dpp_step<0x118, 0xf>(v);
    return v;
}
__device__ __forceinline__ float wave_sum_shfl(float v) {
#pragma unroll
    for (int o = 32; o >= 1; o >>= 1) v += __shfl_xor(v, o, 64);
    return v;
}
#endif

}
```

das3r_amd/csrc/preprocess.hip:

```cpp
#include "common.h"
#include "granule.h"
#include "segkey.h"
#include "splat_math.h"
#include "pretransform_math.h"

namespace das3r {

template <bool HAS_SH, bool HAS_COV, bool STAGE>
__global__ void __launch_bounds__(256) preprocess_kernel(
    int P, int D, int M, const float *__restrict__ means3D, const float *__restrict__ scales, float scale_modifier,
    const float *__restrict__ rotations, const float *__restrict__ opacities, const float *__restrict__ shs,
    const float *__restrict__ cov3D_precomp, const float *__restrict__ colors_precomp, const float *__restrict__ viewmatrix,
    const float *__restrict__ projmatrix, const float *__restrict__ campos, int W, int H, float tanfovx, float tanfovy,
    int tiles_x, int tiles_y, int32_t *__restrict__ radii, uint32_t *__restrict__ depth_key, float4 *__restrict__ xyh,
    float4 *__restrict__ conic_opacity, float4 *__restrict__ rgbd, uint8_t *__restrict__ clamped,
    uint32_t *__restrict__ tiles_touched, uint32_t *__restrict__ rect32, int tight_rect , uint32_t *__restrict__ zero_a, uint32_t zero_a_words, uint32_t *__restrict__ zero_b,
    uint32_t zero_b_words, uint32_t *__restrict__ zero_c, uint32_t zero_c_words, unsigned long long *__restrict__ arrive,
    uint32_t *__restrict__ host_out, uint32_t tag, const EmitArgs em,
    uint32_t *__restrict__ dhist ,
    uint32_t dhist_mask ,
    uint32_t *__restrict__ dhist_next ,
    const PreXform pre ) {
    const int gidx = blockIdx.x * blockDim.x + threadIdx.x;
    bool sampled = false;
    if (dhist != nullptr) {
        uint32_t h = blockIdx.x * 0x9E3779B1u;
        h ^= h >> 15; h *= 0x85EBCA6Bu; h ^= h >> 13; h *= 0xC2B2AE35u; h ^= h >> 16;
        sampled = (h & dhist_mask) == 0u;
    }
    const bool live = gidx < P;
    const int idx = live ? gidx : P - 1;
    float3 p, s_in = make_float3(0.f, 0.f, 0.f);
    float op;
    float4 q_in = make_float4(0.f, 0.f, 0.f, 0.f);
    float c3_in[6] = {0.f, 0.f, 0.f, 0.f, 0.f, 0.f};
    if (!HAS_COV && pre.xyz != nullptr) {
        PoseRegs pose;
        load_pose(pre.Rm, pre.tv, pre.Lq, pose);
        const float rx = pre.xyz[3 * idx], ry = pre.xyz[3 * idx + 1], rz = pre.xyz[3 * idx + 2];
        const float4 rq = reinterpret_cast<const float4 *>(pre.rot)[idx];
        const float r0 = pre.scaling[3 * idx], r1 = pre.scaling[3 * idx + 1], r2 = pre.scaling[3 * idx + 2];
        const float ro = pre.opacity_raw[idx];
        const float rc = pre.conf_flat[pre.mask_index ? pre.mask_index[idx] : (int64_t)idx];
        p = pre_mean(pose, rx, ry, rz);
        q_in = pre_rot(pose, rq);
        s_in = make_float3(pre_scale(r0), pre_scale(r1), pre_scale(r2));
        op = pre_opacity(ro, rc);
    } else {
        p = make_float3(means3D[3 * idx], means3D[3 * idx + 1], means3D[3 * idx + 2]);
        op = opacities[idx];
        if (HAS_COV) {
#pragma unroll
            for (int i = 0; i < 6; i++) c3_in[i] = cov3D_precomp[6 * idx + i];
        } else {
            s_in = make_float3(scales[3 * idx], scales[3 * idx + 1], scales[3 * idx + 2]);
            q_in = reinterpret_cast<const float4 *>(rotations)[idx];
        }
    }
    __shared__ uint32_t s_tiles;
    if (threadIdx.x == 0) s_tiles = 0;
    if (!STAGE) __syncthreads();
    for (uint32_t i = gidx; i < zero_a_words; i += gridDim.x * blockDim.x) zero_a[i] = 0u;
    for (uint32_t i = gidx; i < zero_b_words; i += gridDim.x * blockDim.x) zero_b[i] = 0u;
    for (uint32_t i = gidx; i < zero_c_words; i += gridDim.x * blockDim.x) zero_c[i] = 0u;
    if (dhist_next != nullptr && gidx < DBINS) dhist_next[gidx] = 0u;
    __shared__ float4 sh_lds[STAGE ? 256 * 13 : 256 * 5];
    if (STAGE) {
        const float4 *src = reinterpret_cast<const float4 *>(shs) + (size_t)blockIdx.x * 256 * 12;
        const size_t limit = (size_t)P * 12 - (size_t)blockIdx.x * 256 * 12;
        float4 v[12];
#pragma unroll
        for (int i = 0; i < 12; i++) {
            const size_t f = (size_t)(i * 256 + threadIdx.x);
            v[i] = src[f < limit ? f : limit - 1];
        }
#pragma unroll
        for (int i = 0; i < 12; i++) {
            const int f = i * 256 + threadIdx.x;
            sh_lds[(f / 12) * 13 + (f % 12)] = v[i];
        }
        __syncthreads();
    }
    float V[16], PM[16];
#pragma unroll
    for (int i = 0; i < 16; i++) {
        V[i] = viewmatrix[i];
        PM[i] = projmatrix[i];
    }
    const float focal_x = W / (2.0f * tanfovx), focal_y = H / (2.0f * tanfovy);

    int radius_out = 0;
    uint32_t key_out = 0xFFFFFFFFu, tiles_out = 0;
    uint8_t clamp_out = 0;
    float4 xy_out = make_float4(0.f, 0.f, -1e30f, -1e30f);
    float4 co_out = make_float4(0.f, 0.f, 0.f, 0.f);
    float4 rgbd_out = make_float4(0.f, 0.f, 0.f, 0.f);
    int bx0 = 0, by0 = 0, bx1 = 0, by1 = 0;

    const float3 p_view = xform43(p, V);
    if (p_view.z > NEAR_PLANE) {
        const float4 p_hom = xform44(p, PM);
        const float p_w = 1.0f / (p_hom.w + 0.0000001f);
        const float ndc_x = p_hom.x * p_w, ndc_y = p_hom.y * p_w;

        float c3[6];
        if (HAS_COV) {
#pragma unroll
            for (int i = 0; i < 6; i++) c3[i] = c3_in[i];
        } else {
            cov3d_from_scale_rot(s_in, scale_modifier, q_in, c3);
        }
        float T[2][3];
        float3 t;
        bool cx, cy;
        ewa_T(p_view, V, focal_x, focal_y, tanfovx, tanfovy, T, t, cx, cy);
        float a, b, c;
        cov2d_from_T(T, c3, a, b, c);
        const float det = a * c - b * b;
        if (det != 0.0f) {
            const float det_inv = 1.f / det;
            const float conA = c * det_inv, conB = -b * det_inv, conC = a * det_inv;
            const float mid = 0.5f * (a + c);
            const float lambda1 = mid + sqrtf(fmaxf(0.1f, mid * mid - det));
            const float lambda2 = mid - sqrtf(fmaxf(0.1f, mid * mid - det));
            const float my_radius = ceilf(3.f * sqrtf(fmaxf(lambda1, lambda2)));
            const float px = ((ndc_x + 1.0f) * W - 1.0f) * 0.5f;
            const float py = ((ndc_y + 1.0f) * H - 1.0f) * 0.5f;
            const int r = (int)my_radius;
            int rminx, rminy, rmaxx, rmaxy;
            tile_rect(px, py, r, tiles_x, tiles_y, rminx, rminy, rmaxx, rmaxy);
            const int area = (rmaxx - rminx) * (rmaxy - rminy);
            if (area != 0) {
                float3 col;
                if (HAS_SH && STAGE) {
                    float sh[48];
                    const int n4 = (3 * (D + 1) * (D + 1) + 3) >> 2;
#pragma unroll
                    for (int i = 0; i < 12; i++) {
                        if (i < n4) {
                            const float4 v = sh_lds[threadIdx.x * 13 + i];
                            sh[4 * i] = v.x; sh[4 * i + 1] = v.y; sh[4 * i + 2] = v.z; sh[4 * i + 3] = v.w;
                        }
                    }
                    col = sh_regs_to_rgb(D, sh, p, campos, clamp_out);
                } else if (HAS_SH) {
                    col = sh_to_rgb(D, M, shs + (size_t)idx * M * 3, p, campos, clamp_out);
                } else {
                    col = make_float3(colors_precomp[3 * idx], colors_precomp[3 * idx + 1], colors_precomp[3 * idx + 2]);
                }
                radius_out = r;
                key_out = __float_as_uint(p_view.z);
                float hx = -1e30f, hy = -1e30f;
                if (255.0f * op > 1.0f) {
                    const float tau2 = 2.0f * __logf(255.0f * op) * 1.0005f + 1e-3f;
                    hx = sqrtf(tau2 * a) * 1.0005f + 0.02f;
                    hy = sqrtf(tau2 * c) * 1.0005f + 0.02f;
                }
                xy_out = make_float4(px, py, hx, hy);
                binned_rect(xy_out, r, tiles_x, tiles_y, (tight_rect & 1) != 0, bx0, by0, bx1, by1);
                tiles_out = (uint32_t)((bx1 - bx0) * (by1 - by0));
                co_out = make_float4(conA, conB, conC, op);
                rgbd_out = make_float4(col.x, col.y, col.z, p_view.z);
            }
        }
    } else if ((tight_rect & 2) && live) {
        __hip_atomic_store(host_out + 12, tag, __ATOMIC_RELAXED, __HIP_MEMORY_SCOPE_SYSTEM);
        __threadfence_system();
    }
    if (live) {
    radii[idx] = radius_out;
    depth_key[idx] = key_out;
    tiles_touched[idx] = tiles_out;
    rect32[idx] = tiles_out ? ((uint32_t)bx0 | ((uint32_t)bx1 << 8) | ((uint32_t)by0 << 16) | ((uint32_t)by1 << 24)) : 0u;
    clamped[idx] = clamp_out;
    }
    {
        __syncthreads();
        float4 *rec = sh_lds;
        const int t = threadIdx.x, slot = t * 5;
        rec[slot] = xy_out;
        rec[slot + 1] = co_out;
        rec[slot + 2] = rgbd_out;
        rec[slot + 3] = make_float4(__int_as_float(radius_out), __uint_as_float(tiles_out), 0.f, 0.f);
        __syncthreads();
        float4 *dst = xyh + (size_t)blockIdx.x * 256 * SPLAT_REC;
        const size_t lim = ((size_t)P - (size_t)blockIdx.x * 256) * SPLAT_REC;
#pragma unroll
        for (int i = 0; i < 4; i++) {
            const int f = i * 256 + t;
            if ((size_t)f < lim) dst[f] = rec[f + (f >> 2)];
        }
        if (em.status != nullptr || sampled) __syncthreads();
    }
    if (sampled) {
        uint32_t *lh = reinterpret_cast<uint32_t *>(sh_lds);
        lh[threadIdx.x] = 0u;
        __syncthreads();
        if (live && tiles_out) atomicAdd(&lh[depth_bin(key_out)], tiles_out);
        __syncthreads();
        const uint32_t c = lh[threadIdx.x];
        if (c) atomicAdd(&dhist[threadIdx.x], c);
    }

    if (em.status != nullptr) {
        __shared__ uint32_t ws[4], s_carry;
        uint32_t(*h)[RADIX_SIZE] = reinterpret_cast<uint32_t(*)[RADIX_SIZE]>(sh_lds);
        const int tid = threadIdx.x, lane = __lane_id(), wave = tid >> 6;
        const uint32_t b = blockIdx.x;
        const uint32_t mine = live ? tiles_out : 0u;
        uint32_t total;
        const uint32_t ex = block_exclusive_scan_256(mine, ws, &total);
#pragma unroll
        for (int q = 0; q < 4; q++) h[q][tid] = 0u;
        if (wave == 0) {
            constexpr uint32_t GS = 64u;
            const uint32_t grp = b / GS, r = b % GS, nblocks = gridDim.x;
            const u64 t64 = (u64)em.tag << 32;
            if (lane == 0) granule_store(em.status + b, t64 | total);
            uint32_t in_group = 0, before = 0;
            unsigned spins = 0;
            {
                const bool has = (uint32_t)lane < r;
                u64 x = t64;
                while (true) {
                    if (has) x = granule_poll(em.status + (b - r) + lane, spins);
                    if (__all((x >> 32) == (u64)em.tag)) break;
                    if (spins == SOFT_SPINS && lane == 0) atomicOr(em.err, ERR_HARD_POLL);
                    if (++spins > SPIN_LIMIT) { if (lane == 0) atomicOr(em.err, ERR_TIMEOUT); break; }
                    __builtin_amdgcn_s_sleep(2);
                }
                in_group = has ? (uint32_t)x : 0u;
#pragma unroll
                for (int o = 32; o >= 1; o >>= 1) in_group += (uint32_t)__shfl_xor((int)in_group, o, 64);
            }
            if (r == GS - 1u && lane == 0) granule_store(em.status + nblocks + grp, t64 | (u64)(in_group + total));
            for (uint32_t p0 = 0; p0 < grp; p0 += 64u) {
                const bool has = p0 + (uint32_t)lane < grp;
                u64 x = t64;
                while (true) {
                    if (has) x = granule_poll(em.status + nblocks + p0 + lane, spins);
                    if (__all((x >> 32) == (u64)em.tag)) break;
                    if (spins == SOFT_SPINS && lane == 0) atomicOr(em.err, ERR_HARD_POLL);
                    if (++spins > SPIN_LIMIT) { if (lane == 0) atomicOr(em.err, ERR_TIMEOUT); break; }
                    __builtin_amdgcn_s_sleep(2);
                }
                uint32_t v = has ? (uint32_t)x : 0u;
#pragma unroll
                for (int o = 32; o >= 1; o >>= 1) v += (uint32_t)__shfl_xor((int)v, o, 64);
                before += v;
            }
            if (lane == 0) s_carry = in_group + before;
        }
        __syncthreads();
        uint32_t o = s_carry + ex;
        if (live) {
            em.off_by_gid[idx] = o;
            for (int y = by0; y < by1; y++)
                for (int x = bx0; x < bx1; x++) {
                    if (o < em.cap) {
                        const uint32_t t = (uint32_t)(y * tiles_x + x);
                        em.tile_keys[o] = t;
                        em.gids[o] = (uint32_t)idx;
                        for (int q = 0, sh = 0, dw = tile_digit_width(em.tbits); sh < em.tbits; q++, sh += dw) {
                            const int bits = (em.tbits - sh) < dw ? (em.tbits - sh) : dw;
                            atomicAdd(&h[q][(t >> sh) & ((1u << bits) - 1u)], 1u);
                        }
                    }
                    o++;
                }
        }
        if (b == gridDim.x - 1 && tid == 0) {
            const uint32_t count = s_carry + total, flags = *em.err;
            em.count[0] = count;
            em.count[1] = flags;
            em.count_out[0] = count;
            em.count_out[1] = flags;
            __hip_atomic_store(em.count_out + 2, em.tag, __ATOMIC_RELEASE, __HIP_MEMORY_SCOPE_SYSTEM);
        }
        __syncthreads();
        for (int q = 0, sh = 0, dw = tile_digit_width(em.tbits); sh < em.tbits; q++, sh += dw) {
            const uint32_t c = h[q][tid];
            if (c) atomicAdd(&em.ghist[q * RADIX_SIZE + tid], c);
        }
        return;
    }
    if (arrive == nullptr) return;
    uint32_t wsum = live ? tiles_out : 0u;
#pragma unroll
    for (int o = 32; o >= 1; o >>= 1) wsum += (uint32_t)__shfl_xor((int)wsum, o, 64);
    if (__lane_id() == 0 && wsum) atomicAdd(&s_tiles, wsum);
    __syncthreads();
    if (threadIdx.x == 0) {
        constexpr unsigned long long LOW = (1ull << 40) - 1ull;
        const unsigned r = blockIdx.x & 63u;
        const unsigned long long expected = (gridDim.x - r + 63u) / 64u;
        unsigned long long mine = (1ull << 40) | (unsigned long long)s_tiles;
        unsigned long long *sub = arrive + 8 + 8 * r;
        unsigned long long old = atomicAdd(sub, mine);
        if ((old >> 40) + 1ull == expected) {
            __hip_atomic_store(sub, 0ull, __ATOMIC_RELAXED, __HIP_MEMORY_SCOPE_AGENT);
            mine = (1ull << 40) | ((old + mine) & LOW);
            old = atomicAdd(arrive, mine);
            const unsigned long long subs = gridDim.x < 64u ? gridDim.x : 64u;
            if ((old >> 40) + 1ull == subs) {
                const unsigned long long total = (old + mine) & LOW;
                __hip_atomic_store(arrive, 0ull, __ATOMIC_RELAXED, __HIP_MEMORY_SCOPE_AGENT);
                host_out[0] = (uint32_t)(total > 0xFFFFFFFFull ? 0xFFFFFFFFull : total);
                __hip_atomic_store(host_out + 2, tag, __ATOMIC_RELEASE, __HIP_MEMORY_SCOPE_SYSTEM);
            }
        }
    }
}

__global__ void __launch_bounds__(256) mark_visible_kernel(int P, const float *__restrict__ means3D,
                                                           const float *__restrict__ viewmatrix, uint8_t *__restrict__ present) {
    const int idx = blockIdx.x * blockDim.x + threadIdx.x;
    if (idx >= P) return;
    float V[16];
#pragma unroll
    for (int i = 0; i < 16; i++) V[i] = viewmatrix[i];
    const float3 p = make_float3(means3D[3 * idx], means3D[3 * idx + 1], means3D[3 * idx + 2]);
    present[idx] = xform43(p, V).z > NEAR_PLANE ? 1 : 0;
}

int launch_preprocess(const das3r_raster_args *a, const das3r_raster_in *in, int32_t *radii, char *geom, char *img, char *binning_ctrl,
                      size_t binning_ctrl_bytes, const Layout &L, unsigned long long *arrive, uint32_t *host_out, uint32_t tag,
                      hipStream_t s, const EmitArgs *emit, uint32_t *dhist, uint32_t *dhist_next) {
    const int P = a->P;
    if (P == 0) return DAS3R_OK;
    const EmitArgs em = emit ? *emit : EmitArgs{nullptr, 0u, nullptr, nullptr, nullptr, nullptr, nullptr, 0u, 0, nullptr, nullptr};
    dim3 grid(div_up(P, 256)), block(256);
    uint32_t dhist_mask = 0u;
    while ((grid.x >> __builtin_popcount(dhist_mask)) > 512u) dhist_mask = (dhist_mask << 1) | 1u;
    const bool has_sh = in->shs != nullptr, has_cov = in->cov3D_precomp != nullptr;
    const PreXform pre = pre_xform(in);
#define ARGS                                                                                                              \
    P, a->sh_degree, a->M, in->means3D, in->scales, a->scale_modifier, in->rotations, in->opacities, in->shs,             \
        in->cov3D_precomp, in->colors_precomp, a->viewmatrix, a->projmatrix, a->campos, a->image_width, a->image_height,  \
        a->tanfovx, a->tanfovy, L.tiles_x, L.tiles_y, radii, (uint32_t *)(geom + L.g_keyA), (float4 *)(geom + L.pub.xy),  \
        (float4 *)(geom + L.pub.conic_opacity), (float4 *)(geom + L.pub.rgbd), (uint8_t *)(geom + L.pub.clamped),         \
        (uint32_t *)(geom + L.pub.tiles_touched), (uint32_t *)(geom + L.g_rect), (use_tight_rect() ? 1 : 0) | (a->prefiltered ? 2 : 0), (uint32_t *)(geom + L.g_ghist), (uint32_t)(L.g_ctrl_bytes / 4),                 \
        (uint32_t *)(img + L.pub.ranges), (uint32_t)(2 * L.ntiles), (uint32_t *)binning_ctrl, (uint32_t)(binning_ctrl_bytes / 4), arrive, host_out, tag, em, dhist, dhist_mask, dhist_next, pre
    const bool stage = has_sh && a->M == 16 && a->sh_degree >= 2 && ((uintptr_t)in->shs & 15) == 0 && !switches().no_sh_stage;
    if (has_sh && !has_cov && stage) DAS3R_LAUNCH((preprocess_kernel<true, false, true>), grid, block, 0, s, ARGS);
    else if (has_sh && has_cov && stage) DAS3R_LAUNCH((preprocess_kernel<true, true, true>), grid, block, 0, s, ARGS);
    else if (has_sh && !has_cov) DAS3R_LAUNCH((preprocess_kernel<true, false, false>), grid, block, 0, s, ARGS);
    else if (has_sh && has_cov) DAS3R_LAUNCH((preprocess_kernel<true, true, false>), grid, block, 0, s, ARGS);
    else if (!has_sh && !has_cov) DAS3R_LAUNCH((preprocess_kernel<false, false, false>), grid, block, 0, s, ARGS);
    else DAS3R_LAUNCH((preprocess_kernel<false, true, false>), grid, block, 0, s, ARGS);
#undef ARGS
    KERNEL_CHECK(s, a->debug, "preprocess");
    return DAS3R_OK;
}

int launch_mark_visible(int P, const float *means3D, const float *viewmatrix, uint8_t *present, hipStream_t s) {
    if (P == 0) return DAS3R_OK;
    DAS3R_LAUNCH(mark_visible_kernel, dim3(div_up(P, 256)), dim3(256), 0, s, P, means3D, viewmatrix, present);
    KERNEL_CHECK(s, false, "mark_visible");
    return DAS3R_OK;
}

}
```

das3r_amd/csrc/preprocess_bwd.hip:

```cpp
#include <string.h>

#include <algorithm>
#include <vector>

#include "common.h"
#include "splat_math.h"
#include "pretransform_math.h"
#include "pretransform_chain.h"

namespace das3r {

__device__ __forceinline__ void sh_basis(const int D, const float x, const float y, const float z, float b[16]) {
    b[0] = SH_C0;
    if (D > 0) {
        b[1] = -SH_C1 * y;
        b[2] = SH_C1 * z;
        b[3] = -SH_C1 * x;
        if (D > 1) {
            const float xx = x * x, yy = y * y, zz = z * z, xy = x * y, yz = y * z, xz = x * z;
            b[4] = SH_C2_0 * xy;
            b[5] = SH_C2_1 * yz;
            b[6] = SH_C2_2 * (2.f * zz - xx - yy);
            b[7] = SH_C2_3 * xz;
            b[8] = SH_C2_4 * (xx - yy);
            if (D > 2) {
                b[9] = SH_C3_0 * y * (3.f * xx - yy);
                b[10] = SH_C3_1 * xy * z;
                b[11] = SH_C3_2 * y * (4.f * zz - xx - yy);
                b[12] = SH_C3_3 * z * (2.f * zz - 3.f * xx - 3.f * yy);
                b[13] = SH_C3_4 * x * (4.f * zz - xx - yy);
                b[14] = SH_C3_5 * z * (xx - yy);
                b[15] = SH_C3_6 * x * (xx - 3.f * yy);
            }
        }
    }
}

#define SH_DDIR(SHC, dRdx, dRdy, dRdz)                                                                                          \
    do {                                                                                                                        \
        dRdx = 0.f; dRdy = 0.f; dRdz = 0.f;                                                                                     \
        if (D > 0) {                                                                                                            \
            dRdx = -SH_C1 * SHC(3);                                                                                             \
            dRdy = -SH_C1 * SHC(1);                                                                                             \
            dRdz = SH_C1 * SHC(2);                                                                                              \
            if (D > 1) {                                                                                                        \
                dRdx += SH_C2_0 * y * SHC(4) + SH_C2_2 * 2.f * -x * SHC(6) + SH_C2_3 * z * SHC(7) + SH_C2_4 * 2.f * x * SHC(8); \
                dRdy += SH_C2_0 * x * SHC(4) + SH_C2_1 * z * SHC(5) + SH_C2_2 * 2.f * -y * SHC(6) + SH_C2_4 * 2.f * -y * SHC(8); \
                dRdz += SH_C2_1 * y * SHC(5) + SH_C2_2 * 2.f * 2.f * z * SHC(6) + SH_C2_3 * x * SHC(7);                       \
                if (D > 2) {                                                                                                    \
                    dRdx += SH_C3_0 * SHC(9) * 3.f * 2.f * xy + SH_C3_1 * SHC(10) * yz + SH_C3_2 * SHC(11) * -2.f * xy +       \
                            SH_C3_3 * SHC(12) * -3.f * 2.f * xz + SH_C3_4 * SHC(13) * (-3.f * xx + 4.f * zz - yy) +            \
                            SH_C3_5 * SHC(14) * 2.f * xz + SH_C3_6 * SHC(15) * 3.f * (xx - yy);                                \
                    dRdy += SH_C3_0 * SHC(9) * 3.f * (xx - yy) + SH_C3_1 * SHC(10) * xz +                                      \
                            SH_C3_2 * SHC(11) * (-3.f * yy + 4.f * zz - xx) + SH_C3_3 * SHC(12) * -3.f * 2.f * yz +            \
                            SH_C3_4 * SHC(13) * -2.f * xy + SH_C3_5 * SHC(14) * -2.f * yz + SH_C3_6 * SHC(15) * -3.f * 2.f * xy; \
                    dRdz += SH_C3_1 * SHC(10) * xy + SH_C3_2 * SHC(11) * 4.f * 2.f * yz +                                      \
                            SH_C3_3 * SHC(12) * 3.f * (2.f * zz - xx - yy) + SH_C3_4 * SHC(13) * 4.f * 2.f * xz +              \
                            SH_C3_5 * SHC(14) * (xx - yy);                                                                      \
                }                                                                                                               \
            }                                                                                                                   \
        }                                                                                                                       \
    } while (0)

template <int K>
__device__ __forceinline__ void wave_store_rows(float *__restrict__ dst , const int rows_valid, const float (&v)[K],
                                                float *scratch , const int lane) {
#pragma unroll
    for (int q = 0; q < K; q++) scratch[lane * K + q] = v[q];
    __builtin_amdgcn_fence(__ATOMIC_ACQ_REL, "workgroup");
    const int n = rows_valid * K;
#pragma unroll
    for (int q = 0; q < K; q++) {
        const int e = q * 64 + lane;
        if (e < n) dst[e] = scratch[e];
    }
    __builtin_amdgcn_fence(__ATOMIC_ACQ_REL, "workgroup");
}

struct ChainArgs {
    GeometryAdam A;
    float *g_conf_flat, *g_small, *det_partials;
    uint32_t *arrived;
};
template <bool HAS_SH, bool HAS_COV, bool STAGE_IN, bool STAGE_OUT, bool DEG0 = false, bool CHAIN = false, bool DEPTH = false>
__global__ void __launch_bounds__(256, DEG0 ? (CHAIN ? 4 : 6) : 3) preprocess_backward_kernel(
    int P, int D_in, int M, const float *__restrict__ means3D, const float *__restrict__ scales, float scale_modifier,
    const float *__restrict__ rotations, const float *__restrict__ shs, const float *__restrict__ cov3D_precomp,
    const float *__restrict__ viewmatrix, const float *__restrict__ projmatrix, const float *__restrict__ campos, int W, int H,
    float tanfovx, float tanfovy, const uint32_t *__restrict__ tiles_touched, const uint8_t *__restrict__ clamped,
    const float *__restrict__ partial ,
    const uint8_t *__restrict__ row_exists , const uint32_t *__restrict__ off_by_gid,
    float *__restrict__ dL_dmeans2D , float *__restrict__ dL_dopacity ,
    float *__restrict__ dL_dcolors_precomp , float *__restrict__ dL_dmeans3D,
    float *__restrict__ dL_dscales, float *__restrict__ dL_drot, float *__restrict__ dL_dsh, float *__restrict__ dL_dcov3D,
    const PreXform pre ,
    const ChainArgs ch , const float *__restrict__ dz_g
#ifdef DAS3R_EXPERIMENTS
    , unsigned long long *__restrict__ trace
#endif
    ) {
#ifndef DAS3R_EXPERIMENTS
    constexpr unsigned long long *trace = nullptr;
#endif
    BLK_STAMP(trace, 6, 0)
    __shared__ float4 sh_lds[(STAGE_IN || STAGE_OUT) ? 256 * 13 : 1];
    const int idx = blockIdx.x * blockDim.x + threadIdx.x;
    const int D = DEG0 ? 0 : D_in;
    const int ic = idx < P ? idx : P - 1;
    const uint32_t ntiles_g = idx < P ? tiles_touched[ic] : 0u;
    const uint32_t e0_in = off_by_gid[ic];
    float3 mean_in, sc_in = make_float3(0.f, 0.f, 0.f);
    float4 q_in = make_float4(0.f, 0.f, 0.f, 0.f);
    float c3_in[6] = {0.f, 0.f, 0.f, 0.f, 0.f, 0.f};
    float raw_x = 0.f, raw_y = 0.f, raw_z = 0.f, raw_s0 = 0.f, raw_s1 = 0.f, raw_s2 = 0.f, raw_o = 0.f, raw_c = 0.f;
    float4 raw_q = make_float4(0.f, 0.f, 0.f, 0.f);
    long long raw_ci = 0;
    ChainMoments moments;
    if (!HAS_COV && (CHAIN || pre.xyz != nullptr)) {
        PoseRegs pose;
        load_pose(pre.Rm, pre.tv, pre.Lq, pose);
        const float rx = pre.xyz[3 * ic], ry = pre.xyz[3 * ic + 1], rz = pre.xyz[3 * ic + 2];
        const float4 rq = reinterpret_cast<const float4 *>(pre.rot)[ic];
        const float r0 = pre.scaling[3 * ic], r1 = pre.scaling[3 * ic + 1], r2 = pre.scaling[3 * ic + 2];
        if constexpr (CHAIN) {
            raw_x = rx; raw_y = ry; raw_z = rz; raw_q = rq; raw_s0 = r0; raw_s1 = r1; raw_s2 = r2;
            raw_o = pre.opacity_raw[ic];
            raw_ci = pre.mask_index ? (long long)pre.mask_index[ic] : (long long)ic;
            raw_c = pre.conf_flat[raw_ci];
            chain_load_moments(ch.A, (size_t)ic, moments);
        }
        mean_in = pre_mean(pose, rx, ry, rz);
        q_in = pre_rot(pose, rq);
        sc_in = make_float3(pre_scale(r0), pre_scale(r1), pre_scale(r2));
    } else {
        mean_in = make_float3(means3D[3 * ic], means3D[3 * ic + 1], means3D[3 * ic + 2]);
        if (HAS_COV) {
#pragma unroll
            for (int i = 0; i < 6; i++) c3_in[i] = cov3D_precomp[6 * ic + i];
        } else {
            sc_in = make_float3(scales[3 * ic], scales[3 * ic + 1], scales[3 * ic + 2]);
            q_in = reinterpret_cast<const float4 *>(rotations)[ic];
        }
    }
    const size_t blk4 = (size_t)blockIdx.x * 256 * 12;
    const size_t limit4 = (size_t)P * 12 > blk4 ? (size_t)P * 12 - blk4 : 0;
    constexpr bool LDS_GATHER = STAGE_OUT;
    constexpr int CHUNK_ROWS = 1020;
    float acc[9];
#pragma unroll
    for (int q = 0; q < 9; q++) acc[q] = 0.f;
    float4 sh_in[STAGE_IN ? 12 : 1];
    auto request_sh = [&]() {
        if (STAGE_IN) {
            const float4 *src = reinterpret_cast<const float4 *>(shs) + blk4;
#pragma unroll
            for (int i = 0; i < 12; i++) {
                const size_t f = (size_t)(i * 256 + threadIdx.x);
                sh_in[i] = limit4 ? src[f < limit4 ? f : limit4 - 1] : make_float4(0.f, 0.f, 0.f, 0.f);
            }
        }
    };
    bool gathered = false;
    uint32_t run0 = 0u, run1 = 0u;
    if (LDS_GATHER && !row_exists) {
        __shared__ uint32_t s_run[4][3];
        uint32_t lo = ntiles_g ? e0_in : 0xFFFFFFFFu, hi = ntiles_g ? e0_in + ntiles_g : 0u, cnt = ntiles_g;
#pragma unroll
        for (int o = 32; o >= 1; o >>= 1) {
            lo = min(lo, (uint32_t)__shfl_xor((int)lo, o, 64));
            hi = max(hi, (uint32_t)__shfl_xor((int)hi, o, 64));
            cnt += (uint32_t)__shfl_xor((int)cnt, o, 64);
        }
        if ((threadIdx.x & 63) == 0) {
            s_run[threadIdx.x >> 6][0] = lo;
            s_run[threadIdx.x >> 6][1] = hi;
            s_run[threadIdx.x >> 6][2] = cnt;
        }
        __syncthreads();
        run0 = min(min(s_run[0][0], s_run[1][0]), min(s_run[2][0], s_run[3][0]));
        run1 = max(max(s_run[0][1], s_run[1][1]), max(s_run[2][1], s_run[3][1]));
        const uint32_t rows = s_run[0][2] + s_run[1][2] + s_run[2][2] + s_run[3][2];
        gathered = rows == 0u || rows == run1 - run0;
        BLK_STAMP(trace, 6, 1)
    }
    if (gathered) {
        float *const buf = reinterpret_cast<float *>(sh_lds);
        float4 *const buf4 = sh_lds;
        const uint32_t mine0 = e0_in, mine1 = e0_in + ntiles_g;
        const bool aligned_base = (reinterpret_cast<uintptr_t>(partial) & 15u) == 0;
        bool sh_requested = false;
        for (uint32_t c0 = run0; c0 < run1; c0 += CHUNK_ROWS) {
            const uint32_t nrows = min((uint32_t)CHUNK_ROWS, run1 - c0);
            const float *src = partial + (size_t)c0 * 9;
            const int n9 = (int)nrows * 9;
            int head = 0;
            if (aligned_base) {
                head = (int)((reinterpret_cast<uintptr_t>(src) & 15u) >> 2);
                const float4 *src4 = reinterpret_cast<const float4 *>(src - head);
                const int n4 = (head + n9 + 3) >> 2;
                float4 w[9];
#pragma unroll
                for (int i = 0; i < 9; i++) {
                    const int f = i * 256 + (int)threadIdx.x;
                    w[i] = src4[f < n4 ? f : n4 - 1];
                }
                if (!sh_requested) request_sh();
#pragma unroll
                for (int i = 0; i < 9; i++) {
                    const int f = i * 256 + (int)threadIdx.x;
                    if (f < n4) buf4[f] = w[i];
                }
            } else {
                if (!sh_requested) request_sh();
#pragma unroll 4
                for (int f = threadIdx.x; f < n9; f += 256) buf[f] = src[f];
            }
            sh_requested = true;
            __syncthreads();
            BLK_STAMP(trace, 6, 2)
            const uint32_t k0 = max(mine0, c0), k1 = min(mine1, c0 + nrows);
            for (uint32_t k = k0; k < k1; k++) {
                const float *row = buf + head + (k - c0) * 9;
#pragma unroll
                for (int q = 0; q < 9; q++) acc[q] += row[q];
            }
            __syncthreads();
        }
        if (!sh_requested) request_sh();
    } else {
        request_sh();
    }
    BLK_STAMP(trace, 6, 3)
    if (STAGE_IN) {
#pragma unroll
        for (int i = 0; i < 12; i++) {
            const int f = i * 256 + threadIdx.x;
            if ((size_t)f < limit4) sh_lds[(f / 12) * 13 + (f % 12)] = sh_in[i];
        }
        __syncthreads();
    }
    BLK_STAMP(trace, 6, 4)

    constexpr bool XPOSE = !STAGE_OUT;
    __shared__ float xp_lds[XPOSE ? 4 * 64 * 6 : 1];
    float *const xp = xp_lds + (XPOSE ? (threadIdx.x >> 6) * 64 * 6 : 0);
    const int lane = threadIdx.x & 63;
    const int wave_first = blockIdx.x * 256 + (int)(threadIdx.x & ~63u);
    const int rows_valid = min(max(P - wave_first, 0), 64);
    float o_m2d[3] = {0.f, 0.f, 0.f}, o_m3d[3] = {0.f, 0.f, 0.f}, o_sc[3] = {0.f, 0.f, 0.f}, o_cov[6] = {0.f, 0.f, 0.f, 0.f, 0.f, 0.f};
    float o_col[3] = {0.f, 0.f, 0.f}, o_sh0[3] = {0.f, 0.f, 0.f};
    static_assert(!CHAIN || (XPOSE && HAS_SH && !HAS_COV), "the chained backward: unstaged SH layouts, scales + rotations");
    float o_rot[4] = {0.f, 0.f, 0.f, 0.f}, o_op = 0.f;

    if (idx < P) {
        const bool visible = ntiles_g > 0;

        if (visible && !gathered) {
            const uint32_t e0 = e0_in;
#ifdef DAS3R_EXPERIMENTS
            if (row_exists) {
                for (uint32_t k = 0; k < ntiles_g; k++) {
                    const uint32_t have = *reinterpret_cast<const uint32_t *>(row_exists + (size_t)(e0 + k) * 4);
#pragma unroll
                    for (int w = 0; w < 4; w++) {
                        if ((have >> (8 * w)) & 0xffu) {
                            const float4 *row = reinterpret_cast<const float4 *>(partial + ((size_t)(e0 + k) * 4 + w) * 12);
                            const float4 r0 = row[0], r1 = row[1];
                            const float r2 = reinterpret_cast<const float *>(row)[8];
                            acc[0] += r0.x; acc[1] += r0.y; acc[2] += r0.z; acc[3] += r0.w;
                            acc[4] += r1.x; acc[5] += r1.y; acc[6] += r1.z; acc[7] += r1.w;
                            acc[8] += r2;
                        }
                    }
                }
            } else
#endif
            {
                for (uint32_t k = 0; k < ntiles_g; k++) {
                    const float *row = partial + (size_t)(e0 + k) * 9;
#pragma unroll
                    for (int q = 0; q < 9; q++) acc[q] += row[q];
                }
            }
        }
        if constexpr (CHAIN) o_op = acc[8];
        else dL_dopacity[idx] = acc[8];
        if (XPOSE) {
            o_m2d[0] = acc[3]; o_m2d[1] = acc[4];
            o_col[0] = acc[0]; o_col[1] = acc[1]; o_col[2] = acc[2];
        } else {
            dL_dmeans2D[3 * (size_t)idx] = acc[3];
            dL_dmeans2D[3 * (size_t)idx + 1] = acc[4];
            dL_dmeans2D[3 * (size_t)idx + 2] = 0.f;
            if (!HAS_SH) {
                dL_dcolors_precomp[3 * (size_t)idx] = acc[0];
                dL_dcolors_precomp[3 * (size_t)idx + 1] = acc[1];
                dL_dcolors_precomp[3 * (size_t)idx + 2] = acc[2];
            }
        }

        float dmean[3] = {0.f, 0.f, 0.f};
        float dcov[6] = {0.f, 0.f, 0.f, 0.f, 0.f, 0.f};
        float dscale[3] = {0.f, 0.f, 0.f};
        float drot[4] = {0.f, 0.f, 0.f, 0.f};
        float basis[16];
        float g[3] = {0.f, 0.f, 0.f};

        if (visible) {
            float V[16], PM[16];
#pragma unroll
            for (int i = 0; i < 16; i++) {
                V[i] = viewmatrix[i];
                PM[i] = projmatrix[i];
            }
            const float focal_x = W / (2.0f * tanfovx), focal_y = H / (2.0f * tanfovy);
            const float3 mean = mean_in;
            const float3 sc = sc_in;
            const float4 q = q_in;
            float c3[6];
            if (HAS_COV) {
#pragma unroll
                for (int i = 0; i < 6; i++) c3[i] = c3_in[i];
            } else {
                cov3d_from_scale_rot(sc, scale_modifier, q, c3);
            }
            {
                const float3 p_view = xform43(mean, V);
                float T[2][3];
                float3 t;
                bool cx, cy;
                ewa_T(p_view, V, focal_x, focal_y, tanfovx, tanfovy, T, t, cx, cy);
                const float x_grad_mul = cx ? 0.f : 1.f, y_grad_mul = cy ? 0.f : 1.f;
                const float S[3][3] = {{c3[0], c3[1], c3[2]}, {c3[1], c3[3], c3[4]}, {c3[2], c3[4], c3[5]}};
                float TS0[3], TS1[3];
#pragma unroll
                for (int j = 0; j < 3; j++) {
                    TS0[j] = T[0][0] * S[j][0] + T[0][1] * S[j][1] + T[0][2] * S[j][2];
                    TS1[j] = T[1][0] * S[j][0] + T[1][1] * S[j][1] + T[1][2] * S[j][2];
                }
                const float ca = TS0[0] * T[0][0] + TS0[1] * T[0][1] + TS0[2] * T[0][2] + 0.3f;
                const float cb = TS0[0] * T[1][0] + TS0[1] * T[1][1] + TS0[2] * T[1][2];
                const float cc = TS1[0] * T[1][0] + TS1[1] * T[1][1] + TS1[2] * T[1][2] + 0.3f;
                const float gA = acc[5], gB = acc[6], gC = acc[7];
                const float denom = ca * cc - cb * cb;
                float dL_da = 0.f, dL_db = 0.f, dL_dc = 0.f;
                const float denom2inv = 1.0f / ((denom * denom) + 0.0000001f);
                if (denom2inv != 0.f) {
                    dL_da = denom2inv * (-cc * cc * gA + 2 * cb * cc * gB + (denom - ca * cc) * gC);
                    dL_dc = denom2inv * (-ca * ca * gC + 2 * ca * cb * gB + (denom - ca * cc) * gA);
                    dL_db = denom2inv * 2 * (cb * cc * gA - (denom + 2 * cb * cb) * gB + ca * cb * gC);
                    dcov[0] = (T[0][0] * T[0][0] * dL_da + T[0][0] * T[1][0] * dL_db + T[1][0] * T[1][0] * dL_dc);
                    dcov[3] = (T[0][1] * T[0][1] * dL_da + T[0][1] * T[1][1] * dL_db + T[1][1] * T[1][1] * dL_dc);
                    dcov[5] = (T[0][2] * T[0][2] * dL_da + T[0][2] * T[1][2] * dL_db + T[1][2] * T[1][2] * dL_dc);
                    dcov[1] = 2 * T[0][0] * T[0][1] * dL_da + (T[0][0] * T[1][1] + T[0][1] * T[1][0]) * dL_db + 2 * T[1][0] * T[1][1] * dL_dc;
                    dcov[2] = 2 * T[0][0] * T[0][2] * dL_da + (T[0][0] * T[1][2] + T[0][2] * T[1][0]) * dL_db + 2 * T[1][0] * T[1][2] * dL_dc;
                    dcov[4] = 2 * T[0][2] * T[0][1] * dL_da + (T[0][1] * T[1][2] + T[0][2] * T[1][1]) * dL_db + 2 * T[1][1] * T[1][2] * dL_dc;
                }
                float dT0[3], dT1[3];
#pragma unroll
                for (int j = 0; j < 3; j++) {
                    dT0[j] = 2 * TS0[j] * dL_da + TS1[j] * dL_db;
                    dT1[j] = 2 * TS1[j] * dL_dc + TS0[j] * dL_db;
                }
                const float dJ00 = V[0] * dT0[0] + V[4] * dT0[1] + V[8] * dT0[2];
                const float dJ02 = V[2] * dT0[0] + V[6] * dT0[1] + V[10] * dT0[2];
                const float dJ11 = V[1] * dT1[0] + V[5] * dT1[1] + V[9] * dT1[2];
                const float dJ12 = V[2] * dT1[0] + V[6] * dT1[1] + V[10] * dT1[2];
                const float tz = 1.f / t.z, tz2 = tz * tz, tz3 = tz2 * tz;
                const float dtx = x_grad_mul * -focal_x * tz2 * dJ02;
                const float dty = y_grad_mul * -focal_y * tz2 * dJ12;
                const float dtz = -focal_x * tz2 * dJ00 - focal_y * tz2 * dJ11 + (2 * focal_x * t.x) * tz3 * dJ02 + (2 * focal_y * t.y) * tz3 * dJ12;
                dmean[0] = V[0] * dtx + V[1] * dty + V[2] * dtz;
                dmean[1] = V[4] * dtx + V[5] * dty + V[6] * dtz;
                dmean[2] = V[8] * dtx + V[9] * dty + V[10] * dtz;
            }
            {
                const float4 m_hom = xform44(mean, PM);
                const float m_w = 1.0f / (m_hom.w + 0.0000001f);
                const float mul1 = (PM[0] * mean.x + PM[4] * mean.y + PM[8] * mean.z + PM[12]) * m_w * m_w;
                const float mul2 = (PM[1] * mean.x + PM[5] * mean.y + PM[9] * mean.z + PM[13]) * m_w * m_w;
                const float gx = acc[3], gy = acc[4];
                dmean[0] += (PM[0] * m_w - PM[3] * mul1) * gx + (PM[1] * m_w - PM[3] * mul2) * gy;
                dmean[1] += (PM[4] * m_w - PM[7] * mul1) * gx + (PM[5] * m_w - PM[7] * mul2) * gy;
                dmean[2] += (PM[8] * m_w - PM[11] * mul1) * gx + (PM[9] * m_w - PM[11] * mul2) * gy;
            }
            if (HAS_SH) {
                const float dox = mean.x - campos[0], doy = mean.y - campos[1], doz = mean.z - campos[2];
                const float inv_len = 1.f / sqrtf(dox * dox + doy * doy + doz * doz);
                const float x = dox * inv_len, y = doy * inv_len, z = doz * inv_len;
                const float xx = x * x, yy = y * y, zz = z * z, xy = x * y, yz = y * z, xz = x * z;
                const uint8_t cl = clamped[idx];
#pragma unroll
                for (int c = 0; c < 3; c++) g[c] = ((cl >> c) & 1) ? 0.f : acc[c];
                sh_basis(D, x, y, z, basis);
                float ddir[3] = {0.f, 0.f, 0.f};
                if (D > 0) {
                    if (STAGE_IN) {
                        float shl[48];
#pragma unroll
                        for (int i = 0; i < 12; i++) {
                            const float4 v = sh_lds[threadIdx.x * 13 + i];
                            shl[4 * i] = v.x; shl[4 * i + 1] = v.y; shl[4 * i + 2] = v.z; shl[4 * i + 3] = v.w;
                        }
#pragma unroll
                        for (int c = 0; c < 3; c++) {
                            float dRdx, dRdy, dRdz;
#define SHC_LDS(k) shl[(k) * 3 + c]
                            SH_DDIR(SHC_LDS, dRdx, dRdy, dRdz);
#undef SHC_LDS
                            ddir[0] += dRdx * g[c];
                            ddir[1] += dRdy * g[c];
                            ddir[2] += dRdz * g[c];
                        }
                    } else {
                        const float *row = shs + (size_t)idx * M * 3;
                        float sh[48];
                        load_sh_row(row, D, sh_vec_ok(row, D, M), sh);
#pragma unroll
                        for (int c = 0; c < 3; c++) {
                            float dRdx, dRdy, dRdz;
#define SHC_REG(k) sh[(k) * 3 + c]
                            SH_DDIR(SHC_REG, dRdx, dRdy, dRdz);
#undef SHC_REG
                            ddir[0] += dRdx * g[c];
                            ddir[1] += dRdy * g[c];
                            ddir[2] += dRdz * g[c];
                        }
                    }
                }
                const float sum2 = dox * dox + doy * doy + doz * doz;
                const float invsum32 = 1.0f / sqrtf(sum2 * sum2 * sum2);
                dmean[0] += ((+sum2 - dox * dox) * ddir[0] - doy * dox * ddir[1] - doz * dox * ddir[2]) * invsum32;
                dmean[1] += (-dox * doy * ddir[0] + (sum2 - doy * doy) * ddir[1] - doz * doy * ddir[2]) * invsum32;
                dmean[2] += (-dox * doz * ddir[0] - doy * doz * ddir[1] + (sum2 - doz * doz) * ddir[2]) * invsum32;
            }
            if (!HAS_COV) {
                float R[3][3];
                quat_to_R(q, R);
                const float sv[3] = {scale_modifier * sc.x, scale_modifier * sc.y, scale_modifier * sc.z};
                const float Gs[3][3] = {{dcov[0], 0.5f * dcov[1], 0.5f * dcov[2]}, {0.5f * dcov[1], dcov[3], 0.5f * dcov[4]},
                                        {0.5f * dcov[2], 0.5f * dcov[4], dcov[5]}};
                float Mm[3][3], dM[3][3], dR[3][3];
#pragma unroll
                for (int i = 0; i < 3; i++)
#pragma unroll
                    for (int k = 0; k < 3; k++) Mm[i][k] = R[i][k] * sv[k];
#pragma unroll
                for (int i = 0; i < 3; i++)
#pragma unroll
                    for (int k = 0; k < 3; k++) dM[i][k] = 2.f * (Gs[i][0] * Mm[0][k] + Gs[i][1] * Mm[1][k] + Gs[i][2] * Mm[2][k]);
#pragma unroll
                for (int k = 0; k < 3; k++) dscale[k] = R[0][k] * dM[0][k] + R[1][k] * dM[1][k] + R[2][k] * dM[2][k];
#pragma unroll
                for (int i = 0; i < 3; i++)
#pragma unroll
                    for (int k = 0; k < 3; k++) dR[i][k] = dM[i][k] * sv[k];
                const float r = q.x, x = q.y, y = q.z, z = q.w;
                drot[0] = 2 * z * (dR[1][0] - dR[0][1]) + 2 * y * (dR[0][2] - dR[2][0]) + 2 * x * (dR[2][1] - dR[1][2]);
                drot[1] = 2 * y * (dR[0][1] + dR[1][0]) + 2 * z * (dR[0][2] + dR[2][0]) + 2 * r * (dR[2][1] - dR[1][2]) - 4 * x * (dR[2][2] + dR[1][1]);
                drot[2] = 2 * x * (dR[0][1] + dR[1][0]) + 2 * r * (dR[0][2] - dR[2][0]) + 2 * z * (dR[2][1] + dR[1][2]) - 4 * y * (dR[2][2] + dR[0][0]);
                drot[3] = 2 * r * (dR[1][0] - dR[0][1]) + 2 * x * (dR[0][2] + dR[2][0]) + 2 * y * (dR[2][1] + dR[1][2]) - 4 * z * (dR[1][1] + dR[0][0]);
            }
        }

        if constexpr (DEPTH) {
            if (visible) {
                const float dz = dz_g[idx];
                dmean[0] += dz * viewmatrix[2];
                dmean[1] += dz * viewmatrix[6];
                dmean[2] += dz * viewmatrix[10];
            }
        }
        if (XPOSE) {
#pragma unroll
            for (int k = 0; k < 3; k++) o_m3d[k] = dmean[k], o_sc[k] = dscale[k];
#pragma unroll
            for (int i = 0; i < 6; i++) o_cov[i] = dcov[i];
        } else {
            dL_dmeans3D[3 * (size_t)idx] = dmean[0];
            dL_dmeans3D[3 * (size_t)idx + 1] = dmean[1];
            dL_dmeans3D[3 * (size_t)idx + 2] = dmean[2];
            if (HAS_COV) {
#pragma unroll
                for (int i = 0; i < 6; i++) dL_dcov3D[6 * (size_t)idx + i] = dcov[i];
            } else {
#pragma unroll
                for (int k = 0; k < 3; k++) dL_dscales[3 * (size_t)idx + k] = dscale[k];
            }
        }
        if constexpr (CHAIN) {
#pragma unroll
            for (int k = 0; k < 4; k++) o_rot[k] = drot[k];
        } else if (!HAS_COV) reinterpret_cast<float4 *>(dL_drot)[idx] = make_float4(drot[0], drot[1], drot[2], drot[3]);
        if (HAS_SH) {
            const int nk = visible ? (D + 1) * (D + 1) : 0;
            if (STAGE_OUT) {
#pragma unroll
                for (int i = 0; i < 12; i++) {
                    float o[4];
#pragma unroll
                    for (int e = 0; e < 4; e++) {
                        const int f = 4 * i + e, k = f / 3, c = f - 3 * k;
                        o[e] = k < nk ? basis[k] * g[c] : 0.f;
                    }
                    sh_lds[threadIdx.x * 13 + i] = make_float4(o[0], o[1], o[2], o[3]);
                }
            } else if (XPOSE && M == 1) {
#pragma unroll
                for (int c = 0; c < 3; c++) o_sh0[c] = nk > 0 ? basis[0] * g[c] : 0.f;
            } else {
                float *row = dL_dsh + (size_t)idx * M * 3;
#pragma unroll
                for (int k = 0; k < 16; k++) {
                    if (k < M) {
                        row[3 * k] = k < nk ? basis[k] * g[0] : 0.f;
                        row[3 * k + 1] = k < nk ? basis[k] * g[1] : 0.f;
                        row[3 * k + 2] = k < nk ? basis[k] * g[2] : 0.f;
                    }
                }
            }
        }
    }
    if (XPOSE) {
        wave_store_rows<3>(dL_dmeans2D + 3 * (size_t)wave_first, rows_valid, o_m2d, xp, lane);
        if (!CHAIN) wave_store_rows<3>(dL_dmeans3D + 3 * (size_t)wave_first, rows_valid, o_m3d, xp, lane);
        if (HAS_COV) wave_store_rows<6>(dL_dcov3D + 6 * (size_t)wave_first, rows_valid, o_cov, xp, lane);
        else if (!CHAIN) wave_store_rows<3>(dL_dscales + 3 * (size_t)wave_first, rows_valid, o_sc, xp, lane);
        if (!HAS_SH) wave_store_rows<3>(dL_dcolors_precomp + 3 * (size_t)wave_first, rows_valid, o_col, xp, lane);
        else if (M == 1) wave_store_rows<3>(dL_dsh + 3 * (size_t)wave_first, rows_valid, o_sh0, xp, lane);
    }
    BLK_STAMP(trace, 6, 5)
    if (STAGE_OUT) {
        __syncthreads();
        float4 *dst = reinterpret_cast<float4 *>(dL_dsh) + blk4;
#pragma unroll
        for (int i = 0; i < 12; i++) {
            const int f = i * 256 + threadIdx.x;
            if ((size_t)f < limit4) dst[f] = sh_lds[(f / 12) * 13 + (f % 12)];
        }
    }
#ifdef DAS3R_EXPERIMENTS
    if (trace != nullptr) {
        BLK_STAMP(trace, 6, 6)
        asm volatile("s_waitcnt vmcnt(0)" ::: "memory");
        BLK_STAMP(trace, 6, 7)
    }
#endif
    if constexpr (CHAIN) {
        __shared__ float red[4][28];
        float Rp[9], Lp[16], pacc[28];
#pragma unroll
        for (int i = 0; i < 9; i++) Rp[i] = pre.Rm[i];
#pragma unroll
        for (int i = 0; i < 16; i++) Lp[i] = pre.Lq[i];
#pragma unroll
        for (int i = 0; i < 28; i++) pacc[i] = 0.f;
        if (idx < P) {
            ChainIn in;
            in.x = raw_x; in.y = raw_y; in.z = raw_z; in.q = raw_q;
            in.sc[0] = raw_s0; in.sc[1] = raw_s1; in.sc[2] = raw_s2; in.o = raw_o; in.c = raw_c;
            in.gx = o_m3d[0]; in.gy = o_m3d[1]; in.gz = o_m3d[2];
            in.gq = make_float4(o_rot[0], o_rot[1], o_rot[2], o_rot[3]);
            in.gs[0] = o_sc[0]; in.gs[1] = o_sc[1]; in.gs[2] = o_sc[2]; in.go = o_op;
            chain_pose_acc(in, pacc);
            ChainOut o;
            chain_grads(Rp, Lp, in, o);
            ch.g_conf_flat[raw_ci] = o.gconf;
            chain_adam(ch.A, (size_t)idx, in, o, moments);
        }
        pose_sums_finish(pacc, red, ch.det_partials, ch.arrived, ch.g_small);
    }
}

static float *chain_scratch(hipStream_t s, size_t blocks, uint32_t **arrived) {
    struct Slot { int dev; hipStream_t stream; float *buf; size_t rows; };
    static thread_local std::vector<Slot> slots;
    *arrived = nullptr;
    int dev = 0;
    if (hipGetDevice(&dev) != hipSuccess) return nullptr;
    Slot *hit = nullptr;
    for (auto &e : slots)
        if (e.dev == dev && e.stream == s) hit = &e;
    if (!hit || hit->rows < blocks) {
        auto complain = [] {
            static bool said = false;
            if (!__atomic_exchange_n(&said, true, __ATOMIC_RELAXED))
                fprintf(stderr, "[das3r] no scratch for the fixed-order pose sums: this thread's pose gradients are summed with float atomics (not bit-reproducible)\n");
        };
        const size_t rows = std::max(blocks, (size_t)4096) * 2;
        float *buf = nullptr;
        if (hit) { (void)hipStreamSynchronize(s); (void)hipFree(hit->buf); hit->buf = nullptr; hit->rows = 0; }
        if (hipMalloc((void **)&buf, (rows * 28 + 4) * sizeof(float)) != hipSuccess) { complain(); return nullptr; }
        if (hipMemsetAsync(buf, 0, (rows * 28 + 4) * sizeof(float), s) != hipSuccess || hipStreamSynchronize(s) != hipSuccess) { (void)hipFree(buf); complain(); return nullptr; }
        if (hit) { hit->buf = buf; hit->rows = rows; }
        else { slots.push_back({dev, s, buf, rows}); hit = &slots.back(); }
    }
    if (!hit->buf) return nullptr;
    *arrived = reinterpret_cast<uint32_t *>(hit->buf + hit->rows * 28);
    return hit->buf;
}

int launch_preprocess_backward(const das3r_raster_args *a, const das3r_raster_in *in, char *geom, char *binning, const Layout &L,
                               const das3r_raster_grads *g, const float *partial, hipStream_t s, bool quad_rows, const float *dz) {
    const int P = a->P;
    if (P == 0) return DAS3R_OK;
    dim3 grid(div_up(P, 256)), block(256);
    const bool has_sh = in->shs != nullptr, has_cov = in->cov3D_precomp != nullptr;
    const bool nostage = switches().no_sh_stage;
    const size_t cap_rows = L.capacity > 0 ? (size_t)L.capacity : 1;
    const uint8_t *exists = quad_rows ? reinterpret_cast<const uint8_t *>(partial) + align_up(cap_rows * 4 * 12 * sizeof(float)) : nullptr;
    const bool stage_out = has_sh && a->M == 16 && ((uintptr_t)g->dL_dshs & 15) == 0 && !nostage;
    const bool stage_in = stage_out && a->sh_degree >= 2 && ((uintptr_t)in->shs & 15) == 0;
#ifdef DAS3R_EXPERIMENTS
#define PB_TRACE_ARG , wg_trace()
#else
#define PB_TRACE_ARG
#endif
    const PreXform pre = pre_xform(in);
#define ARGS                                                                                                                 \
    P, a->sh_degree, a->M, in->means3D, in->scales, a->scale_modifier, in->rotations, in->shs, in->cov3D_precomp,            \
        a->viewmatrix, a->projmatrix, a->campos, a->image_width, a->image_height, a->tanfovx, a->tanfovy,                    \
        (const uint32_t *)(geom + L.pub.tiles_touched), (const uint8_t *)(geom + L.pub.clamped), partial, exists,        \
        (const uint32_t *)(geom + L.g_off_by_gid), g->dL_dmeans2D, g->dL_dopacities, g->dL_dcolors_precomp, g->dL_dmeans3D,  \
        g->dL_dscales, g->dL_drotations, g->dL_dshs, g->dL_dcov3D, pre, ch, dz PB_TRACE_ARG
    ChainArgs ch;
    memset(&ch, 0, sizeof(ch));
    if (g->chain) {
        const das3r_chain *c = g->chain;
        if (!pre.xyz || !pre.opacity_raw || !pre.conf_flat || !has_sh || has_cov || stage_out || quad_rows || !c->slots || !c->g_conf_flat || !c->g_small) {
            set_error("das3r_raster_backward: grads->chain needs in->pre, SH coefficients in an unstaged layout (M < 16 or the active degree below 2 ...), "
                      "scales + rotations, and g_conf_flat / g_small / slots");
            return DAS3R_ERR_INVALID_ARG;
        }
        for (int k = 0; k < 4; k++) {
            if (!c->slots[k].param || !c->slots[k].exp_avg || !c->slots[k].exp_avg_sq || !(c->slots[k].bc2_sqrt > 0.f)) {
                set_error("das3r_raster_backward: grads->chain: bad slot %d", k);
                return DAS3R_ERR_INVALID_ARG;
            }
            ch.A.p[k] = c->slots[k].param; ch.A.m[k] = c->slots[k].exp_avg; ch.A.v[k] = c->slots[k].exp_avg_sq;
            ch.A.step_size[k] = c->slots[k].step_size; ch.A.bc2_sqrt[k] = c->slots[k].bc2_sqrt;
        }
        if (ch.A.p[0] != pre.xyz || ch.A.p[1] != pre.rot || ch.A.p[2] != pre.scaling || ch.A.p[3] != pre.opacity_raw) {
            set_error("das3r_raster_backward: grads->chain: the slots must be the tensors of in->pre (xyz, rot, scaling, opacity_raw)");
            return DAS3R_ERR_INVALID_ARG;
        }
        ch.A.beta1 = c->beta1; ch.A.beta2 = c->beta2; ch.A.eps = c->eps;
        ch.g_conf_flat = c->g_conf_flat; ch.g_small = c->g_small;
        ch.det_partials = chain_scratch(s, (size_t)grid.x, &ch.arrived);
    }
#define LAUNCH6(SH, COV, SI, SO, D0, CH)                                                                             \
    do {                                                                                                             \
        if (dz) DAS3R_LAUNCH((preprocess_backward_kernel<SH, COV, SI, SO, D0, CH, true>), grid, block, 0, s, ARGS); \
        else DAS3R_LAUNCH((preprocess_backward_kernel<SH, COV, SI, SO, D0, CH>), grid, block, 0, s, ARGS);          \
    } while (0)
#define LAUNCH(SH, COV, SI, SO) LAUNCH6(SH, COV, SI, SO, false, false)
#define LAUNCH0(SH, COV) LAUNCH6(SH, COV, false, false, true, false)
    const bool deg0 = a->sh_degree == 0 && !stage_out;
    if (g->chain) {
        if (deg0) LAUNCH6(true, false, false, false, true, true);
        else LAUNCH6(true, false, false, false, false, true);
    } else if (has_sh && !has_cov) {
        if (stage_in) LAUNCH(true, false, true, true);
        else if (stage_out) LAUNCH(true, false, false, true);
        else if (deg0) LAUNCH0(true, false);
        else LAUNCH(true, false, false, false);
    } else if (has_sh && has_cov) {
        if (stage_in) LAUNCH(true, true, true, true);
        else if (stage_out) LAUNCH(true, true, false, true);
        else if (deg0) LAUNCH0(true, true);
        else LAUNCH(true, true, false, false);
    } else if (!has_sh && !has_cov) {
        LAUNCH(false, false, false, false);
    } else {
        LAUNCH(false, true, false, false);
    }
#undef LAUNCH
#undef LAUNCH0
#undef LAUNCH6
#undef ARGS
    KERNEL_CHECK(s, a->debug, "preprocess_backward");
    return DAS3R_OK;
}

__global__ void __launch_bounds__(256) depth_pass_inputs_kernel(int P, int npix, const float4 *__restrict__ rec_in , float4 *__restrict__ rec_out,
                                                                const float *__restrict__ dL_dinvdepth, float *__restrict__ dpix, float *__restrict__ bg) {
    const int i = blockIdx.x * blockDim.x + threadIdx.x;
    if (i < P) {
        const float4 *r = rec_in + (size_t)i * SPLAT_REC;
        float4 *o = rec_out + (size_t)i * SPLAT_REC;
        const float4 c = r[2];
        o[0] = r[0];
        o[1] = r[1];
        o[2] = make_float4(c.w > 0.f ? 1.0f / c.w : 0.f, 0.f, 0.f, c.w);
    }
    if (i < npix) {
        dpix[i] = dL_dinvdepth[i];
        dpix[(size_t)npix + i] = 0.f;
        dpix[2 * (size_t)npix + i] = 0.f;
    }
    if (i < 4) bg[i] = 0.f;
}
__global__ void __launch_bounds__(256) depth_fold_kernel(int P, const uint32_t *__restrict__ tiles_touched, const uint32_t *__restrict__ off_by_gid,
                                                         const float4 *__restrict__ rgbd, float *__restrict__ partial, const float *__restrict__ partial_depth,
                                                         float *__restrict__ dz) {
    const int i = blockIdx.x * blockDim.x + threadIdx.x;
    if (i >= P) return;
    const uint32_t n = tiles_touched[i];
    float s = 0.f;
    if (n > 0u) {
        const uint32_t e0 = off_by_gid[i];
        for (uint32_t k = 0; k < n; k++) {
            const size_t row = (size_t)(e0 + k) * 9;
            s += partial_depth[row];
#pragma unroll
            for (int q = 3; q < 9; q++) partial[row + q] += partial_depth[row + q];
        }
    }
    const float z = rgbd[(size_t)i * SPLAT_REC].w;
    dz[i] = n > 0u ? -s / (z * z) : 0.f;
}
int launch_depth_pass_inputs(int P, int npix, const char *geom, const Layout &L, char *binning, const float *dL_dinvdepth, hipStream_t s, bool debug) {
    const int n = std::max(std::max(P, npix), 4);
    DAS3R_LAUNCH(depth_pass_inputs_kernel, dim3(div_up(n, 256)), dim3(256), 0, s, P, npix, (const float4 *)(geom + L.pub.xy), (float4 *)(binning + L.d_recs),
                 dL_dinvdepth, (float *)(binning + L.d_dpix), (float *)(binning + L.d_bg));
    KERNEL_CHECK(s, debug, "depth_pass_inputs");
    return DAS3R_OK;
}
int launch_depth_fold(int P, const char *geom, const Layout &L, float *partial, const float *partial_depth, float *dz, hipStream_t s, bool debug) {
    DAS3R_LAUNCH(depth_fold_kernel, dim3(div_up(P, 256)), dim3(256), 0, s, P, (const uint32_t *)(geom + L.pub.tiles_touched),
                 (const uint32_t *)(geom + L.g_off_by_gid), (const float4 *)(geom + L.pub.rgbd), partial, partial_depth, dz);
    KERNEL_CHECK(s, debug, "depth_fold");
    return DAS3R_OK;
}

}
```

das3r_amd/csrc/splat_math.h:

```cpp
#pragma once
#include <hip/hip_runtime.h>

namespace das3r {

__device__ constexpr float SH_C0 = 0.28209479177387814f;
__device__ constexpr float SH_C1 = 0.4886025119029199f;
__device__ constexpr float SH_C2_0 = 1.0925484305920792f, SH_C2_1 = -1.0925484305920792f, SH_C2_2 = 0.31539156525252005f,
                           SH_C2_3 = -1.0925484305920792f, SH_C2_4 = 0.5462742152960396f;
__device__ constexpr float SH_C3_0 = -0.5900435899266435f, SH_C3_1 = 2.890611442640554f, SH_C3_2 = -0.4570457994644658f,
                           SH_C3_3 = 0.3731763325901154f, SH_C3_4 = -0.4570457994644658f, SH_C3_5 = 1.445305721320277f,
                           SH_C3_6 = -0.5900435899266435f;

__device__ __forceinline__ float3 xform43(const float3 p, const float *m) {
    return make_float3(m[0] * p.x + m[4] * p.y + m[8] * p.z + m[12], m[1] * p.x + m[5] * p.y + m[9] * p.z + m[13],
                       m[2] * p.x + m[6] * p.y + m[10] * p.z + m[14]);
}
__device__ __forceinline__ float4 xform44(const float3 p, const float *m) {
    return make_float4(m[0] * p.x + m[4] * p.y + m[8] * p.z + m[12], m[1] * p.x + m[5] * p.y + m[9] * p.z + m[13],
                       m[2] * p.x + m[6] * p.y + m[10] * p.z + m[14], m[3] * p.x + m[7] * p.y + m[11] * p.z + m[15]);
}

__device__ __forceinline__ void quat_to_R(const float4 q, float R[3][3]) {
    const float r = q.x, x = q.y, y = q.z, z = q.w;
    R[0][0] = 1.f - 2.f * (y * y + z * z); R[0][1] = 2.f * (x * y - r * z);       R[0][2] = 2.f * (x * z + r * y);
    R[1][0] = 2.f * (x * y + r * z);       R[1][1] = 1.f - 2.f * (x * x + z * z); R[1][2] = 2.f * (y * z - r * x);
    R[2][0] = 2.f * (x * z - r * y);       R[2][1] = 2.f * (y * z + r * x);       R[2][2] = 1.f - 2.f * (x * x + y * y);
}

__device__ __forceinline__ void cov3d_from_scale_rot(const float3 scale, const float mod, const float4 q, float *cov) {
    float R[3][3];
    quat_to_R(q, R);
    const float s[3] = {mod * scale.x, mod * scale.y, mod * scale.z};
    float Mm[3][3];
#pragma unroll
    for (int i = 0; i < 3; i++)
#pragma unroll
        for (int k = 0; k < 3; k++) Mm[i][k] = R[i][k] * s[k];
#define SIG(i, j) (Mm[i][0] * Mm[j][0] + Mm[i][1] * Mm[j][1] + Mm[i][2] * Mm[j][2])
    cov[0] = SIG(0, 0); cov[1] = SIG(0, 1); cov[2] = SIG(0, 2); cov[3] = SIG(1, 1); cov[4] = SIG(1, 2); cov[5] = SIG(2, 2);
#undef SIG
}

__device__ __forceinline__ void ewa_T(const float3 p_view, const float *V, const float focal_x, const float focal_y,
                                      const float tanfovx, const float tanfovy, float T[2][3], float3 &t, bool &clampx, bool &clampy) {
    t = p_view;
    const float limx = 1.3f * tanfovx, limy = 1.3f * tanfovy;
    const float txtz = t.x / t.z, tytz = t.y / t.z;
    clampx = (txtz < -limx || txtz > limx);
    clampy = (tytz < -limy || tytz > limy);
    t.x = fminf(limx, fmaxf(-limx, txtz)) * t.z;
    t.y = fminf(limy, fmaxf(-limy, tytz)) * t.z;
    const float J00 = focal_x / t.z, J02 = -(focal_x * t.x) / (t.z * t.z);
    const float J11 = focal_y / t.z, J12 = -(focal_y * t.y) / (t.z * t.z);
#pragma unroll
    for (int j = 0; j < 3; j++) {
        T[0][j] = J00 * V[4 * j + 0] + 0.f * V[4 * j + 1] + J02 * V[4 * j + 2];
        T[1][j] = 0.f * V[4 * j + 0] + J11 * V[4 * j + 1] + J12 * V[4 * j + 2];
    }
}

__device__ __forceinline__ void cov2d_from_T(const float T[2][3], const float *c3, float &a, float &b, float &c) {
    const float S[3][3] = {{c3[0], c3[1], c3[2]}, {c3[1], c3[3], c3[4]}, {c3[2], c3[4], c3[5]}};
    float TS[2][3];
#pragma unroll
    for (int i = 0; i < 2; i++)
#pragma unroll
        for (int j = 0; j < 3; j++) TS[i][j] = T[i][0] * S[0][j] + T[i][1] * S[1][j] + T[i][2] * S[2][j];
    a = TS[0][0] * T[0][0] + TS[0][1] * T[0][1] + TS[0][2] * T[0][2] + 0.3f;
    b = TS[0][0] * T[1][0] + TS[0][1] * T[1][1] + TS[0][2] * T[1][2];
    c = TS[1][0] * T[1][0] + TS[1][1] * T[1][1] + TS[1][2] * T[1][2] + 0.3f;
}

__device__ __forceinline__ void tile_rect(const float px, const float py, const int r, const int tiles_x, const int tiles_y,
                                          int &rminx, int &rminy, int &rmaxx, int &rmaxy) {
    rminx = min(tiles_x, max(0, (int)((px - r) / TILE_X)));
    rminy = min(tiles_y, max(0, (int)((py - r) / TILE_Y)));
    rmaxx = min(tiles_x, max(0, (int)((px + r + TILE_X - 1) / TILE_X)));
    rmaxy = min(tiles_y, max(0, (int)((py + r + TILE_Y - 1) / TILE_Y)));
}

__device__ __forceinline__ void binned_rect(const float4 xyh, const int r, const int tiles_x, const int tiles_y, const bool tight,
                                            int &rminx, int &rminy, int &rmaxx, int &rmaxy) {
    tile_rect(xyh.x, xyh.y, r, tiles_x, tiles_y, rminx, rminy, rmaxx, rmaxy);
    if (tight) {
        if (xyh.z < 0.f) {
            rmaxx = rminx;
            return;
        }
        const float px0 = ceilf(xyh.x - xyh.z), px1 = floorf(xyh.x + xyh.z);
        const float py0 = ceilf(xyh.y - xyh.w), py1 = floorf(xyh.y + xyh.w);
        if (px1 < px0 || py1 < py0 || px1 < 0.f || py1 < 0.f) {
            rmaxx = rminx;
            return;
        }
        const int tx0 = (int)fmaxf(px0, 0.f) >> 4, ty0 = (int)fmaxf(py0, 0.f) >> 4;
        const int tx1 = ((int)fminf(px1, 1.0e6f) >> 4) + 1, ty1 = ((int)fminf(py1, 1.0e6f) >> 4) + 1;
        rminx = max(rminx, tx0);
        rminy = max(rminy, ty0);
        rmaxx = max(rminx, min(rmaxx, tx1));
        rmaxy = max(rminy, min(rmaxy, ty1));
    }
}

__device__ __forceinline__ void load_sh_row(const float *__restrict__ row, const int D, const bool vec_ok, float sh[48]) {
    const int n3 = 3 * (D + 1) * (D + 1);
    if (vec_ok) {
        const float4 *r4 = reinterpret_cast<const float4 *>(row);
#pragma unroll
        for (int i = 0; i < 12; i++) {
            if (4 * i < n3) {
                const float4 v = r4[i];
                sh[4 * i] = v.x; sh[4 * i + 1] = v.y; sh[4 * i + 2] = v.z; sh[4 * i + 3] = v.w;
            }
        }
    } else {
#pragma unroll
        for (int i = 0; i < 48; i++)
            if (i < n3) sh[i] = row[i];
    }
}

__device__ __forceinline__ float3 sh_eval(const int deg, const float sh[48], const float x, const float y, const float z) {
    float out[3];
#pragma unroll
    for (int c = 0; c < 3; c++) {
#define SHC(k) sh[(k) * 3 + c]
        float r = SH_C0 * SHC(0);
        if (deg > 0) {
            r = r - SH_C1 * y * SHC(1) + SH_C1 * z * SHC(2) - SH_C1 * x * SHC(3);
            if (deg > 1) {
                const float xx = x * x, yy = y * y, zz = z * z, xy = x * y, yz = y * z, xz = x * z;
                r = r + SH_C2_0 * xy * SHC(4) + SH_C2_1 * yz * SHC(5) + SH_C2_2 * (2.f * zz - xx - yy) * SHC(6) +
                    SH_C2_3 * xz * SHC(7) + SH_C2_4 * (xx - yy) * SHC(8);
                if (deg > 2) {
                    r = r + SH_C3_0 * y * (3.f * xx - yy) * SHC(9) + SH_C3_1 * xy * z * SHC(10) +
                        SH_C3_2 * y * (4.f * zz - xx - yy) * SHC(11) + SH_C3_3 * z * (2.f * zz - 3.f * xx - 3.f * yy) * SHC(12) +
                        SH_C3_4 * x * (4.f * zz - xx - yy) * SHC(13) + SH_C3_5 * z * (xx - yy) * SHC(14) +
                        SH_C3_6 * x * (xx - 3.f * yy) * SHC(15);
                }
            }
        }
#undef SHC
        out[c] = r + 0.5f;
    }
    return make_float3(out[0], out[1], out[2]);
}

__device__ __forceinline__ bool sh_vec_ok(const float *row, const int D, const int M) {
    const int n3 = 3 * (D + 1) * (D + 1);
    return (((uintptr_t)row & 15) == 0) && (((n3 + 3) & ~3) <= 3 * M);
}

__device__ __forceinline__ float3 sh_regs_to_rgb(const int D, const float sh[48], const float3 p, const float *campos,
                                                 uint8_t &clamp_bits) {
    const float dx = p.x - campos[0], dy = p.y - campos[1], dz = p.z - campos[2];
    const float inv = 1.f / sqrtf(dx * dx + dy * dy + dz * dz);
    const float3 r = sh_eval(D, sh, dx * inv, dy * inv, dz * inv);
    clamp_bits = (uint8_t)((r.x < 0.f ? 1 : 0) | (r.y < 0.f ? 2 : 0) | (r.z < 0.f ? 4 : 0));
    return make_float3(fmaxf(r.x, 0.f), fmaxf(r.y, 0.f), fmaxf(r.z, 0.f));
}

__device__ __forceinline__ float3 sh_to_rgb(const int D, const int M, const float *__restrict__ row, const float3 p,
                                            const float *campos, uint8_t &clamp_bits) {
    float sh[48];
    load_sh_row(row, D, sh_vec_ok(row, D, M), sh);
    const float dx = p.x - campos[0], dy = p.y - campos[1], dz = p.z - campos[2];
    const float inv = 1.f / sqrtf(dx * dx + dy * dy + dz * dz);
    const float3 r = sh_eval(D, sh, dx * inv, dy * inv, dz * inv);
    clamp_bits = (uint8_t)((r.x < 0.f ? 1 : 0) | (r.y < 0.f ? 2 : 0) | (r.z < 0.f ? 4 : 0));
    return make_float3(fmaxf(r.x, 0.f), fmaxf(r.y, 0.f), fmaxf(r.z, 0.f));
}

}
```

das3r_amd/offline.py:

```python
import argparse
import os
import re
import time
from types import SimpleNamespace

import numpy as np
import torch

from .model import SplatModel
from .render import das3r_render


def tensor_from_camera(RT, device="cuda"):
    from .io_formats import matrix_to_quat_wxyz
    m = RT.detach().cpu().numpy() if torch.is_tensor(RT) else np.asarray(RT)
    return torch.from_numpy(np.concatenate([matrix_to_quat_wxyz(m[:3, :3]), m[:3, 3]]).astype(np.float32)).to(device)


def save_image(chw, path):
    from PIL import Image
    arr = chw.detach().float().mul(255).add_(0.5).clamp_(0, 255).permute(1, 2, 0).to("cpu", torch.uint8).numpy()
    os.makedirs(os.path.dirname(os.path.abspath(path)), exist_ok=True)
    Image.fromarray(arr).save(path, format="PNG")
    return arr


def search_for_max_iteration(folder):
    its = [int(m.group(1)) for m in (re.fullmatch(r"iteration_(\d+)", f) for f in os.listdir(folder)) if m]
    if not its:
        raise FileNotFoundError(f"no iteration_* under {folder}")
    return max(its)


def load_trained_model(model_path, iteration=-1, sh_degree=3, device="cuda"):
    from .io_formats import load_gaussians_ply
    if iteration == -1:
        iteration = search_for_max_iteration(os.path.join(model_path, "point_cloud"))
    g = load_gaussians_ply(os.path.join(model_path, "point_cloud", f"iteration_{iteration}", "point_cloud.ply"), max_sh_degree=sh_degree)
    t = lambda a: torch.from_numpy(np.ascontiguousarray(a)).to(device=device, dtype=torch.float32)
    m = SplatModel(sh_degree)
    m._xyz, m._features_dc, m._features_rest = t(g["xyz"]), t(g["features_dc"]), t(g["features_rest"])
    m._opacity, m._conf_static, m._scaling, m._rotation = t(g["opacity"]), t(g["conf_static"]), t(g["scaling"]), t(g["rotation"])
    m.active_sh_degree = sh_degree
    return m, iteration


def save_interpolate_pose(model_path, iteration):
    src = os.path.join(model_path, "pose", f"pose_{iteration}.npy")
    if not os.path.exists(src):
        return None
    org = np.load(src)
    out = np.stack([np.block([[p[:3, :3], p[:3, 3:4]], [np.zeros((1, 3)), np.ones((1, 1))]]) for p in org], 0)
    np.save(os.path.join(model_path, "pose", "pose_interpolated.npy"), out)
    return out


def sequence_cameras(seq, device="cuda"):
    from .train import make_camera
    K = seq["K"]
    cams = []
    for i in range(seq["images"].shape[0]):
        c = make_camera(i, seq["images"][i].to(device), float(K[i, 0, 0]), seq["W"], seq["H"], device, focal_y=float(K[i, 1, 1]),
                        camera_center=seq["cam2world"][i][:3, 3])
        c.pose7 = seq["w2c_pose7"][i].to(device=device, dtype=torch.float32)
        cams.append(c)
    return cams


PIPE = SimpleNamespace(debug=False, compute_cov3D_python=False, convert_SHs_python=False)


class _EvalState:

    def __init__(self, model):
        dev = model._xyz.device
        self.mats = torch.empty(28, device=dev)
        self.e = torch.empty(0, device=dev)
        self.shs, self.versions = None, None

    def packed_sh(self, model):
        v = (model._features_dc._version, model._features_rest._version, model._features_dc.data_ptr(), model._features_rest.data_ptr())
        if self.shs is None or v != self.versions:
            self.shs, self.versions = model.get_features.detach().contiguous(), v
        return self.shs


@torch.no_grad()
def render_view_fused(model, view, pose7, background, pipe=PIPE, invdepth=False):
    import ctypes as C
    from . import _lib
    from .rasterizer import _forward_full, _on_device, _stream, check_forward
    from .render import _settings
    st = model.__dict__.get("_das3r_eval")
    if st is None:
        st = model.__dict__["_das3r_eval"] = _EvalState(model)
    dev = model._xyz.device
    lib = _lib.load()
    pose7 = pose7.detach().to(device=dev, dtype=torch.float32).contiguous()
    conf = model._conf_static.detach().reshape(-1)
    if conf.shape[0] != model._xyz.shape[0]:
        raise RuntimeError("render_view_fused renders a LOADED model (one conf_static value per Gaussian: load_trained_model)")
    with _on_device(dev):
        _lib.check(lib.das3r_pose_matrices(C.c_void_p(pose7.data_ptr()), C.c_void_p(st.mats.data_ptr()), _stream(dev)), "das3r_pose_matrices")
    pre = _lib.PreTransform()
    xyz, rot, sc, op = model._xyz.detach(), model._rotation.detach(), model._scaling.detach(), model._opacity.detach()
    pre.xyz, pre.rot, pre.scaling, pre.opacity_raw = xyz.data_ptr(), rot.data_ptr(), sc.data_ptr(), op.data_ptr()
    pre.conf_flat, pre.mask_index = conf.data_ptr(), None
    pre.R, pre.t, pre.Lq = st.mats.data_ptr(), st.mats.data_ptr() + 36, st.mats.data_ptr() + 48
    rs = _settings(view, model, pipe, background, 1.0, dev)
    res = _forward_full(rs, xyz, st.packed_sh(model), st.e, op, sc, rot, st.e, pre=pre, invdepth=invdepth)
    check_forward(res[6], dev)
    return (res[1], res[2], res[7]) if invdepth else (res[1], res[2])


def invdepth_median_rel_error(invdepth, depth):
    inv = torch.as_tensor(invdepth).detach().reshape(-1).float().cpu()
    d = torch.as_tensor(depth).detach().reshape(-1).float().cpu()
    sel = (inv > 0) & (d > 0)
    if not bool(sel.any()):
        return float("nan")
    return float(((1.0 / inv[sel] - d[sel]).abs() / d[sel]).median())


@torch.no_grad()
def render_set(model_path, name, iteration, views, model, pipe=PIPE, background=None, poses=None, write=True, fused=False, invdepth=None):
    dev = model.get_xyz.device
    background = background if background is not None else torch.zeros(3, device=dev)
    render_path = os.path.join(model_path, name, f"ours_{iteration}", "renders")
    depth_path = os.path.join(model_path, name, f"ours_{iteration}", "invdepth")
    want = invdepth is not None
    out = []
    for idx, view in enumerate(views):
        pose = view.pose7 if poses is None else tensor_from_camera(poses[idx], dev)
        if fused:
            res = render_view_fused(model, view, pose, background, pipe, invdepth=want)
            img, inv = res[0], (res[2] if want else None)
        else:
            pkg = das3r_render(view, model, pipe, background, camera_pose=pose, variant="test", return_invdepth=want)
            img, inv = pkg["render"], pkg.get("invdepth")
        out.append(img)
        if want:
            invdepth.append(inv)
        if write:
            save_image(img, os.path.join(render_path, f"{idx:05d}.png"))
            if want:
                os.makedirs(depth_path, exist_ok=True)
                np.save(os.path.join(depth_path, f"{idx:05d}.npy"), inv[0].detach().cpu().numpy())
    return out


def render_sets(model_path, seq, iteration=-1, sh_degree=3, white_background=False, optimised_poses=False, device="cuda", write=True, fused=False,
                depth=False):
    model, iteration = load_trained_model(model_path, iteration, sh_degree, device)
    inter = save_interpolate_pose(model_path, iteration)
    bg = torch.tensor([1.0, 1.0, 1.0] if white_background else [0.0, 0.0, 0.0], dtype=torch.float32, device=device)
    views = sequence_cameras(seq, device)
    frames = list(range(len(views)))
    poses = None
    if optimised_poses:
        if inter is None:
            raise FileNotFoundError(f"--optimised-poses: no pose/pose_{iteration}.npy under {model_path}")
        if len(inter) != len(views):
            from .train import split_sequence
            tr, _ = split_sequence(seq)
            if len(inter) != len(tr):
                raise ValueError(f"pose_{iteration}.npy holds {len(inter)} poses, the sequence {len(views)} frames ({len(tr)} training frames)")
            views = [views[i] for i in tr]
            frames = list(tr)
        poses = inter
    inv = [] if depth else None
    imgs = render_set(model_path, "interp", iteration, views, model, PIPE, bg, poses=poses, write=write, fused=fused, invdepth=inv)
    if depth and seq.get("depths") is not None:
        for idx, (f, d) in enumerate(zip(frames, inv)):
            print(f"view {idx:05d} (frame {f}): median |1/invdepth - depth| / depth = {invdepth_median_rel_error(d, seq['depths'][f]):.4f}")
    return iteration, imgs


@torch.no_grad()
def forward_throughput(model, views, repeats=3, background=None, fused=False):
    dev = model.get_xyz.device
    background = background if background is not None else torch.zeros(3, device=dev)
    run = ((lambda: [render_view_fused(model, v, v.pose7, background)[0] for v in views]) if fused
           else (lambda: [das3r_render(v, model, PIPE, background, camera_pose=v.pose7, variant="test")["render"] for v in views]))
    run()
    torch.cuda.current_stream(dev).synchronize()
    t0 = time.perf_counter()
    for _ in range(repeats):
        run()
    torch.cuda.current_stream(dev).synchronize()
    dt = (time.perf_counter() - t0) / (repeats * len(views))
    return dict(ms_per_view=dt * 1e3, views_per_s=1.0 / dt, views=len(views), splats=int(model.get_xyz.shape[0]))


def main(argv=None):
    ap = argparse.ArgumentParser(description="Testing script parameters (render.py)")
    ap.add_argument("--model-path", "-m", "--model_path", dest="model_path", required=True)
    ap.add_argument("--source-path", "-s", "--source_path", dest="source_path", required=True, help="the preprocessed sequence directory the model was trained on")
    ap.add_argument("--iteration", type=int, default=-1)
    ap.add_argument("--sh-degree", "--sh_degree", dest="sh_degree", type=int, default=3)
    ap.add_argument("--white-background", "--white_background", dest="white_background", action="store_true")
    ap.add_argument("--optimised-poses", action="store_true", help="render from pose/pose_N.npy instead of the poses the cameras were loaded with")
    ap.add_argument("--dataset", default="sintel", choices=("sintel", "davis"))
    ap.add_argument("--fused", action="store_true", help="the pose pre-transform inside the rasterizer's kernels instead of the reference's PyTorch glue (render_view_fused)")
    ap.add_argument("--depth", action="store_true", help="also write the inverse-depth images (invdepth/%%05d.npy next to renders/) and print each view's "
                                                         "median relative error of 1/invdepth against the sequence's depth_maps")
    args = ap.parse_args(argv)
    from .io_formats import load_sequence
    print("Rendering " + args.model_path)
    seq = load_sequence(args.source_path, device="cuda", dataset=args.dataset)
    it, imgs = render_sets(args.model_path, seq, args.iteration, args.sh_degree, args.white_background, args.optimised_poses, fused=args.fused,
                           depth=args.depth)
    print(f"wrote {len(imgs)} images to {os.path.join(args.model_path, 'interp', f'ours_{it}', 'renders')}")


if __name__ == "__main__":
    main()
```

das3r_amd/rasterizer.py:

```python
import ctypes as C
import threading
from typing import NamedTuple

import torch
import torch.nn as nn

from . import _lib


class GaussianRasterizationSettings(NamedTuple):
    image_height: int
    image_width: int
    tanfovx: float
    tanfovy: float
    bg: torch.Tensor
    scale_modifier: float
    viewmatrix: torch.Tensor
    projmatrix: torch.Tensor
    sh_degree: int
    campos: torch.Tensor
    prefiltered: bool
    debug: bool


def cpu_deep_copy_tuple(input_tuple):
    return tuple(item.cpu().clone() if isinstance(item, torch.Tensor) else item for item in input_tuple)


def _ptr(t):
    return None if t is None or t.numel() == 0 else C.c_void_p(t.data_ptr())


_EMPTY = {}


def _empty(device):
    t = _EMPTY.get(device)
    if t is None:
        t = _EMPTY[device] = torch.empty(0, dtype=torch.float32, device=device)
    return t


def _prep(t, device, name):
    if t is None:
        return _empty(device)
    if t.dtype == torch.float32 and t.device == device and t.is_contiguous():
        return t
    if t.numel() == 0:
        return t.to(device=device, dtype=torch.float32)
    if t.numel() and t.dtype != torch.float32:
        raise TypeError(f"{name} must be float32 (got {t.dtype})")
    if t.device != device:
        raise RuntimeError(f"{name} is on {t.device}, expected {device}")
    return t.contiguous()


def _small(t, device, n, name):
    if not (isinstance(t, torch.Tensor) and t.dtype == torch.float32 and t.device == device and t.is_contiguous()):
        t = torch.as_tensor(t, dtype=torch.float32, device=device).contiguous()
    if t.numel() != n:
        raise ValueError(f"{name} must have {n} elements")
    return t


class _Alloc:

    _local = threading.local()

    @classmethod
    def get(cls, device):
        per_device = getattr(cls._local, "per_device", None)
        if per_device is None:
            per_device = cls._local.per_device = {}
        a = per_device.get(device)
        if a is None:
            a = per_device[device] = cls(device)
        a.bufs = {}
        return a

    def take(self):
        b, self.bufs = self.bufs, {}
        return b

    def __init__(self, device):
        self.device = device
        self.bufs = {}
        self.fns = {k: _lib.ALLOC_FN(self._make(k)) for k in ("geom", "binning", "img")}

    def _make(self, key):
        def fn(_user, nbytes):
            try:
                t = torch.empty(max(int(nbytes), 1), dtype=torch.uint8, device=self.device)
                self.bufs[key] = t
                return t.data_ptr()
            except Exception:
                return 0
        return fn


def _fill_args(rs, P, M, device, keep):
    a = _lib.RasterArgs()
    a.P, a.sh_degree, a.M = P, int(rs.sh_degree), M
    a.image_width, a.image_height = int(rs.image_width), int(rs.image_height)
    a.tanfovx, a.tanfovy, a.scale_modifier = float(rs.tanfovx), float(rs.tanfovy), float(rs.scale_modifier)
    bg = _small(rs.bg, device, 3, "bg")
    vm = _small(rs.viewmatrix, device, 16, "viewmatrix")
    pm = _small(rs.projmatrix, device, 16, "projmatrix")
    cp = _small(rs.campos, device, 3, "campos")
    keep.extend([bg, vm, pm, cp])
    a.bg, a.viewmatrix, a.projmatrix, a.campos = bg.data_ptr(), vm.data_ptr(), pm.data_ptr(), cp.data_ptr()
    a.prefiltered, a.debug = int(bool(rs.prefiltered)), int(bool(rs.debug))
    return a


def _fill_in(means3D, opacities, sh, colors_precomp, scales, rotations, cov3Ds_precomp, pre=None):
    i = _lib.RasterIn()
    i.means3D, i.opacities = _ptr(means3D), _ptr(opacities)
    i.shs, i.colors_precomp = _ptr(sh), _ptr(colors_precomp)
    i.scales, i.rotations, i.cov3D_precomp = _ptr(scales), _ptr(rotations), _ptr(cov3Ds_precomp)
    if pre is not None:
        i.pre = C.pointer(pre)
    return i


_raw_stream = getattr(torch._C, "_cuda_getCurrentRawStream", None)


def _stream(device):
    if _raw_stream is not None and device.index is not None:
        return C.c_void_p(_raw_stream(device.index))
    return C.c_void_p(torch.cuda.current_stream(device).cuda_stream)


class _on_device:

    def __init__(self, device):
        self.ctx = None if device.index is None or torch.cuda.current_device() == device.index else torch.cuda.device(device)

    def __enter__(self):
        if self.ctx is not None:
            self.ctx.__enter__()

    def __exit__(self, *exc):
        if self.ctx is not None:
            return self.ctx.__exit__(*exc)
        return False


class _Capacity(int):
    check_word = None
    check_tag = 0
    flags = 0


def check_forward(capacity, device):
    if not getattr(capacity, "check_tag", 0):
        return
    saved = _lib.RasterSaved()
    saved.check_word, saved.check_tag = capacity.check_word, capacity.check_tag
    with _on_device(device):
        rc = _lib.load().das3r_raster_check(C.byref(saved), _stream(device))
    _lib.check(rc, "das3r_raster_check")


def _forward_impl(rs, means3D, sh, colors_precomp, opacities, scales, rotations, cov3Ds_precomp):
    return _forward_full(rs, means3D, sh, colors_precomp, opacities, scales, rotations, cov3Ds_precomp, exact=True)[:6]


def _forward_full(rs, means3D, sh, colors_precomp, opacities, scales, rotations, cov3Ds_precomp, exact=False, pre=None, invdepth=False):
    lib = _lib.load()
    device = means3D.device
    if device.type != "cuda":
        raise RuntimeError("das3r_amd rasterizer: tensors must live on a HIP device (torch device 'cuda'); "
                           "there is no CPU path")
    if means3D.dim() != 2 or means3D.shape[1] != 3:
        raise RuntimeError("means3D must have dimensions (num_points, 3)")
    P = means3D.shape[0]
    H, W = int(rs.image_height), int(rs.image_width)
    M = 0
    if sh.numel():
        if sh.dim() != 3 or sh.shape[0] != P or sh.shape[2] != 3:
            raise RuntimeError("shs must have dimensions (num_points, M, 3)")
        M = sh.shape[1]
    if P == 0:
        e = torch.empty(0, dtype=torch.uint8, device=device)
        out = (0, torch.zeros(3, H, W, dtype=torch.float32, device=device), torch.zeros(0, dtype=torch.int32, device=device),
               e, e, e, 0)
        return out + (torch.zeros(1, H, W, dtype=torch.float32, device=device),) if invdepth else out
    color = torch.empty(3, H, W, dtype=torch.float32, device=device)
    radii = torch.empty(P, dtype=torch.int32, device=device)
    alloc = _Alloc.get(device)
    keep = []
    a = _fill_args(rs, P, M, device, keep)
    a.capacity_hint = -1 if exact else 0
    i = _fill_in(means3D, opacities, sh, colors_precomp, scales, rotations, cov3Ds_precomp, pre)
    o = _lib.RasterOut()
    o.out_color, o.radii = color.data_ptr(), radii.data_ptr()
    inv = torch.empty(1, H, W, dtype=torch.float32, device=device) if invdepth else None
    o.out_invdepth = _ptr(inv)
    saved = _lib.RasterSaved()
    with _on_device(device):
        rc = lib.das3r_raster_forward(C.byref(a), C.byref(i), C.byref(o), alloc.fns["geom"], alloc.fns["binning"],
                                      alloc.fns["img"], None, C.byref(saved), _stream(device))
    _lib.check(rc, "das3r_raster_forward")
    empty = torch.empty(0, dtype=torch.uint8, device=device)
    bufs = alloc.take()
    cap = _Capacity(saved.capacity)
    cap.check_word, cap.check_tag, cap.flags = saved.check_word, int(saved.check_tag), int(saved.flags)
    out = (int(rc), color, radii, bufs.get("geom", empty), bufs.get("binning", empty), bufs.get("img", empty), cap)
    return out + (inv,) if invdepth else out


def _backward_impl(rs, num_rendered, grad_out_color, means3D, sh, colors_precomp, opacities, scales, rotations, cov3Ds_precomp,
                   geom, binning, img, capacity=None, _scratch_misalign=0, pre=None, chain=None, grad_invdepth=None):
    ticket = capacity
    capacity = int(num_rendered) if capacity is None else int(capacity)
    lib = _lib.load()
    device = means3D.device
    P = means3D.shape[0]
    M = sh.shape[1] if sh.numel() else 0
    z = lambda *shape: torch.empty(*shape, dtype=torch.float32, device=device)
    has_sh, has_cov = sh.numel() > 0, cov3Ds_precomp.numel() > 0
    g_means2D = z(P, 3)
    g_opac, g_means3D = (None, None) if chain is not None else (z(P, 1), z(P, 3))
    g_sh = z(P, M, 3) if has_sh else None
    g_colors = None if has_sh else z(P, 3)
    g_scales, g_rot = (None, None) if (has_cov or chain is not None) else (z(P, 3), z(P, 4))
    g_cov = z(P, 6) if has_cov else None
    if P == 0:
        return g_means2D, g_colors, g_opac, g_means3D, g_cov, g_sh, g_scales, g_rot
    depth = grad_invdepth is not None
    nbytes = (lib.das3r_raster_backward_depth_scratch_bytes if depth else lib.das3r_raster_backward_scratch_bytes)(max(capacity, 1))
    scratch = torch.empty(int(nbytes) + int(_scratch_misalign), dtype=torch.uint8, device=device)
    keep = []
    a = _fill_args(rs, P, M, device, keep)
    i = _fill_in(means3D, opacities, sh, colors_precomp, scales, rotations, cov3Ds_precomp, pre)
    saved = _lib.RasterSaved()
    saved.geom, saved.binning, saved.img = _ptr(geom), _ptr(binning), _ptr(img)
    saved.num_rendered = int(num_rendered)
    saved.capacity = capacity
    if getattr(ticket, "check_tag", 0):
        saved.check_word, saved.check_tag = ticket.check_word, ticket.check_tag
    saved.flags = int(getattr(ticket, "flags", 0))
    g = _lib.RasterGrads()
    g.dL_dmeans2D, g.dL_dopacities, g.dL_dmeans3D = g_means2D.data_ptr(), _ptr(g_opac), _ptr(g_means3D)
    if chain is not None:
        g.chain = C.pointer(chain)
    g.dL_dshs = _ptr(g_sh)
    g.dL_dcolors_precomp = _ptr(g_colors)
    g.dL_dscales, g.dL_drotations = _ptr(g_scales), _ptr(g_rot)
    g.dL_dcov3D = _ptr(g_cov)
    g.scratch = scratch.data_ptr() + int(_scratch_misalign)
    H, W = int(rs.image_height), int(rs.image_width)
    dL = grad_out_color.contiguous() if grad_out_color is not None else torch.zeros(3, H, W, dtype=torch.float32, device=device)
    if dL.dtype != torch.float32:
        dL = dL.float()
    if depth:
        dD = grad_invdepth.contiguous()
        if dD.dtype != torch.float32:
            dD = dD.float()
        with _on_device(device):
            rc = lib.das3r_raster_backward_depth(C.byref(a), C.byref(i), C.byref(saved), C.c_void_p(dL.data_ptr()), C.c_void_p(dD.data_ptr()),
                                                 C.byref(g), _stream(device))
        _lib.check(rc, "das3r_raster_backward_depth")
        return g_means2D, g_colors, g_opac, g_means3D, g_cov, g_sh, g_scales, g_rot
    with _on_device(device):
        rc = lib.das3r_raster_backward(C.byref(a), C.byref(i), C.byref(saved), C.c_void_p(dL.data_ptr()), C.byref(g),
                                       _stream(device))
    _lib.check(rc, "das3r_raster_backward")
    return g_means2D, g_colors, g_opac, g_means3D, g_cov, g_sh, g_scales, g_rot


def count_live_pairs(rs, P, M, num_rendered, geom, binning, img, capacity):
    lib = _lib.load()
    device = geom.device
    keep = []
    a = _fill_args(rs, P, M, device, keep)
    saved = _lib.RasterSaved()
    saved.geom, saved.binning, saved.img = _ptr(geom), _ptr(binning), _ptr(img)
    saved.num_rendered, saved.capacity = int(num_rendered), int(capacity)
    out = (C.c_uint64 * 2)()
    lib.das3r_raster_count_live_pairs.restype = C.c_int
    lib.das3r_raster_count_live_pairs.argtypes = [C.c_void_p, C.c_void_p, C.POINTER(C.c_uint64), C.c_void_p]
    with _on_device(device):
        rc = lib.das3r_raster_count_live_pairs(C.byref(a), C.byref(saved), out, _stream(device))
    _lib.check(rc, "das3r_raster_count_live_pairs")
    return int(out[0]), int(out[1])


def rasterize_gaussians(means3D, means2D, sh, colors_precomp, opacities, scales, rotations, cov3Ds_precomp, raster_settings):
    return _RasterizeGaussians.apply(means3D, means2D, sh, colors_precomp, opacities, scales, rotations, cov3Ds_precomp,
                                     raster_settings)


_last = threading.local()


class _RasterizeGaussians(torch.autograd.Function):
    @staticmethod
    def forward(ctx, means3D, means2D, sh, colors_precomp, opacities, scales, rotations, cov3Ds_precomp, raster_settings):
        return _RasterizeGaussians._forward(ctx, False, means3D, sh, colors_precomp, opacities, scales, rotations, cov3Ds_precomp, raster_settings)

    @staticmethod
    def _forward(ctx, invdepth, means3D, sh, colors_precomp, opacities, scales, rotations, cov3Ds_precomp, raster_settings):
        device = means3D.device
        means3D = _prep(means3D, device, "means3D")
        sh = _prep(sh, device, "shs")
        colors_precomp = _prep(colors_precomp, device, "colors_precomp")
        opacities = _prep(opacities, device, "opacities")
        scales = _prep(scales, device, "scales")
        rotations = _prep(rotations, device, "rotations")
        cov3Ds_precomp = _prep(cov3Ds_precomp, device, "cov3D_precomp")
        args = (raster_settings, means3D, sh, colors_precomp, opacities, scales, rotations, cov3Ds_precomp)
        if raster_settings.debug:
            cpu_args = cpu_deep_copy_tuple(args)
            try:
                res = _forward_full(*args, invdepth=invdepth)
            except Exception as ex:
                torch.save(cpu_args, "snapshot_fw.dump")
                print("\nAn error occured in forward. Please forward snapshot_fw.dump for debugging.")
                raise ex
        else:
            res = _forward_full(*args, invdepth=invdepth)
        num_rendered, color, radii, geomBuffer, binningBuffer, imgBuffer, capacity = res[:7]
        ctx.raster_settings = raster_settings
        ctx.num_rendered = num_rendered
        ctx.capacity = capacity
        _last.capacity = capacity
        ctx.save_for_backward(colors_precomp, means3D, scales, rotations, cov3Ds_precomp, radii, sh, opacities, geomBuffer,
                              binningBuffer, imgBuffer)
        ctx.mark_non_differentiable(radii)
        ctx.set_materialize_grads(False)
        return (color, radii, res[7]) if invdepth else (color, radii)

    @staticmethod
    def backward(ctx, grad_out_color, _grad_radii):
        return _RasterizeGaussians._backward(ctx, grad_out_color, None)

    @staticmethod
    def _backward(ctx, grad_out_color, grad_invdepth):
        rs = ctx.raster_settings
        if grad_out_color is None and grad_invdepth is None:
            return (None,) * 9
        (colors_precomp, means3D, scales, rotations, cov3Ds_precomp, radii, sh, opacities, geomBuffer, binningBuffer,
         imgBuffer) = ctx.saved_tensors
        args = (rs, ctx.num_rendered, grad_out_color, means3D, sh, colors_precomp, opacities, scales, rotations, cov3Ds_precomp,
                geomBuffer, binningBuffer, imgBuffer, ctx.capacity)
        kw = {} if grad_invdepth is None else {"grad_invdepth": grad_invdepth}
        if rs.debug:
            cpu_args = cpu_deep_copy_tuple(args)
            try:
                out = _backward_impl(*args, **kw)
            except Exception as ex:
                torch.save(cpu_args, "snapshot_bw.dump")
                print("\nAn error occured in backward. Writing snapshot_bw.dump for debugging.\n")
                raise ex
        else:
            out = _backward_impl(*args, **kw)
        g_means2D, g_colors, g_opac, g_means3D, g_cov, g_sh, g_scales, g_rot = out
        return (g_means3D, g_means2D, g_sh if sh.numel() else None, g_colors if colors_precomp.numel() else None, g_opac,
                g_scales if scales.numel() else None, g_rot if rotations.numel() else None,
                g_cov if cov3Ds_precomp.numel() else None, None)


class _RasterizeGaussiansInvDepth(torch.autograd.Function):
    @staticmethod
    def forward(ctx, means3D, means2D, sh, colors_precomp, opacities, scales, rotations, cov3Ds_precomp, raster_settings):
        return _RasterizeGaussians._forward(ctx, True, means3D, sh, colors_precomp, opacities, scales, rotations, cov3Ds_precomp, raster_settings)

    @staticmethod
    def backward(ctx, grad_out_color, _grad_radii, grad_invdepth):
        return _RasterizeGaussians._backward(ctx, grad_out_color, grad_invdepth)


class GaussianRasterizer(nn.Module):
    def __init__(self, raster_settings):
        super().__init__()
        self.raster_settings = raster_settings

    def markVisible(self, positions):
        with torch.no_grad():
            rs = self.raster_settings
            device = positions.device
            if device.type != "cuda":
                raise RuntimeError("das3r_amd rasterizer: positions must live on a HIP device; there is no CPU path")
            pos = _prep(positions, device, "positions")
            P = pos.shape[0]
            present = torch.zeros(P, dtype=torch.uint8, device=device)
            if P:
                vm = _small(rs.viewmatrix, device, 16, "viewmatrix")
                pm = _small(rs.projmatrix, device, 16, "projmatrix")
                with torch.cuda.device(device):
                    rc = _lib.load().das3r_mark_visible(P, _ptr(pos), _ptr(vm), _ptr(pm), _ptr(present), _stream(device))
                _lib.check(rc, "das3r_mark_visible")
            return present.bool()

    def forward(self, means3D, means2D, opacities, shs=None, colors_precomp=None, scales=None, rotations=None,
                cov3D_precomp=None, return_invdepth=False):
        raster_settings = self.raster_settings
        if (shs is None and colors_precomp is None) or (shs is not None and colors_precomp is not None):
            raise Exception("Please provide excatly one of either SHs or precomputed colors!")
        if ((scales is None or rotations is None) and cov3D_precomp is None) or \
                ((scales is not None or rotations is not None) and cov3D_precomp is not None):
            raise Exception("Please provide exactly one of either scale/rotation pair or precomputed 3D covariance!")
        e = _empty(means3D.device)
        if shs is None:
            shs = e
        if colors_precomp is None:
            colors_precomp = e
        if scales is None:
            scales = e
        if rotations is None:
            rotations = e
        if cov3D_precomp is None:
            cov3D_precomp = e
        _last.capacity = None
        if return_invdepth:
            color, radii, invdepth = _RasterizeGaussiansInvDepth.apply(means3D, means2D, shs, colors_precomp, opacities, scales, rotations,
                                                                       cov3D_precomp, raster_settings)
        else:
            color, radii = rasterize_gaussians(means3D, means2D, shs, colors_precomp, opacities, scales, rotations, cov3D_precomp,
                                               raster_settings)
        if not color.requires_grad and getattr(_last, "capacity", None) is not None:
            check_forward(_last.capacity, means3D.device)
        _last.capacity = None
        return (color, radii, invdepth) if return_invdepth else (color, radii)
```

Measured before the change: 1106 Msplats/s.

## Precompute SH direction Jacobian in forward and reuse it in backward

```diff
diff --git a/das3r_amd/_lib.py b/das3r_amd/_lib.py
--- a/das3r_amd/_lib.py
+++ b/das3r_amd/_lib.py
@@ -4,6 +4,7 @@
 _HERE = os.path.dirname(os.path.abspath(__file__))
 LIB_PATH = os.path.join(_HERE, "libdas3r_hip.so")
 ABI_VERSION = 16
+NO_BACKWARD_IN_FLAG = 8
 
 ALLOC_FN = C.CFUNCTYPE(C.c_void_p, C.c_void_p, C.c_size_t)
 
diff --git a/das3r_amd/csrc/api.hip b/das3r_amd/csrc/api.hip
--- a/das3r_amd/csrc/api.hip
+++ b/das3r_amd/csrc/api.hip
@@ -156,7 +156,7 @@
 #endif
 bool use_tight_rect() { return !switches().rect_upstream; }
 
-void compute_layout(int P, int64_t I, int W, int H, Layout *L) {
+void compute_layout(int P, int64_t I, int W, int H, Layout *L, bool shjac) {
     memset(L, 0, sizeof(*L));
     const size_t Pn = P > 0 ? (size_t)P : 1, In = I > 0 ? (size_t)I : 1;
     L->capacity = I;
@@ -198,6 +198,7 @@
     L->g_status = take(onesweep_status_bytes((int64_t)Pn, 4));
     L->g_scan_status = take(scan_status_bytes((int)Pn));
     L->g_ctrl_bytes = o - L->g_ghist;
+    if (shjac) L->g_shjac = take(4 * 9 * Pn);
     L->pub.geom_bytes = o;
     o = 0;
     L->b_keyA = take(4 * In);
@@ -438,8 +439,9 @@
     }
     const int P = a->P, W = a->image_width, H = a->image_height;
     const bool depth = out->out_invdepth != nullptr;
+    const bool shjac = in->shs != nullptr && a->sh_degree >= 2 && !(saved->flags & NO_BACKWARD_IN_FLAG);
     Layout L;
-    compute_layout(P, 0, W, H, &L);
+    compute_layout(P, 0, W, H, &L, shjac);
     saved->geom = alloc_geom(user, L.pub.geom_bytes);
     saved->img = alloc_img(user, L.pub.img_bytes);
     saved->binning = nullptr;
@@ -590,7 +592,7 @@
     if ((local || seg) && verdict.last_I >= 0 && a->capacity_hint != -1 && !switches().capacity_exact) {
         cap = std::max(verdict.last_I + verdict.last_I / 4, verdict.peak_I + verdict.peak_I / 20) + 4096;
         if (cap > (int64_t)0x7FFFFF00) cap = (int64_t)0x7FFFFF00;
-        compute_layout(P, cap, W, H, &L);
+        compute_layout(P, cap, W, H, &L, shjac);
         apply_seg();
         saved->binning = alloc_binning(user, depth ? L.d_bytes : L.pub.binning_bytes);
         if (!saved->binning) { set_error("scratch allocation failed (binning %zu B)", L.pub.binning_bytes); return DAS3R_ERR_ALLOC; }
@@ -639,7 +641,7 @@
         verdict.peak_I = std::max(I, verdict.peak_I - verdict.peak_I / 1024);
         if (I > cap) {
             cap = I;
-            compute_layout(P, cap, W, H, &L);
+            compute_layout(P, cap, W, H, &L, shjac);
             saved->binning = alloc_binning(user, depth ? L.d_bytes : L.pub.binning_bytes);
             if (!saved->binning) { set_error("scratch allocation failed (binning %zu B)", L.pub.binning_bytes); return DAS3R_ERR_ALLOC; }
             apply_seg();
@@ -666,7 +668,7 @@
             local = false;
             if ((rc = launch_depth_sort(P, saved->geom, L, 0, nullptr, 0, a->debug != 0, s))) return rc;
         }
-        compute_layout(P, cap, W, H, &L);
+        compute_layout(P, cap, W, H, &L, shjac);
         apply_seg();
         saved->binning = alloc_binning(user, depth ? L.d_bytes : L.pub.binning_bytes);
         if (!saved->binning) { set_error("scratch allocation failed (binning %zu B)", L.pub.binning_bytes); return DAS3R_ERR_ALLOC; }
@@ -677,7 +679,12 @@
     saved->num_rendered = I;
     saved->capacity = cap;
     if (depth) saved->flags |= DEPTH_SAVED_FLAG;
+    if (shjac) saved->flags |= SHJAC_SAVED_FLAG;
     return I;
+}
+
+static bool shjac_saved(const das3r_raster_args *a, const das3r_raster_in *in, const das3r_raster_saved *saved) {
+    return (saved->flags & SHJAC_SAVED_FLAG) != 0 && in->shs != nullptr && a->sh_degree >= 2;
 }
 
 extern "C" int das3r_raster_backward(const das3r_raster_args *a, const das3r_raster_in *in, const das3r_raster_saved *saved,
@@ -701,7 +708,7 @@
     }
     if ((rc = das3r_raster_check(saved, stream))) return rc;
     Layout L;
-    compute_layout(P, saved->capacity > 0 ? saved->capacity : saved->num_rendered, a->image_width, a->image_height, &L);
+    compute_layout(P, saved->capacity > 0 ? saved->capacity : saved->num_rendered, a->image_width, a->image_height, &L, shjac_saved(a, in, saved));
     float *partial = g->scratch;
     bool quad_rows = false;
     if (saved->num_rendered > 0) {
@@ -741,7 +748,7 @@
     }
     if ((rc = das3r_raster_check(saved, stream))) return rc;
     Layout L;
-    compute_layout(P, saved->capacity > 0 ? saved->capacity : saved->num_rendered, a->image_width, a->image_height, &L);
+    compute_layout(P, saved->capacity > 0 ? saved->capacity : saved->num_rendered, a->image_width, a->image_height, &L, shjac_saved(a, in, saved));
     float *partial = g->scratch;
     const float *dz = nullptr;
     bool quad_rows = false;
diff --git a/das3r_amd/csrc/common.h b/das3r_amd/csrc/common.h
--- a/das3r_amd/csrc/common.h
+++ b/das3r_amd/csrc/common.h
@@ -163,6 +163,8 @@
 constexpr int SPLAT_REC = 4;
 
 constexpr uint32_t DEPTH_SAVED_FLAG = 2u;
+constexpr uint32_t SHJAC_SAVED_FLAG = 4u;
+constexpr uint32_t NO_BACKWARD_IN_FLAG = 8u;
 struct Layout {
     das3r_raster_layout pub;
     size_t g_keyA, g_keyB, g_valA, g_valB, g_hist, g_totals, g_blocksums, g_count, g_off_by_gid, g_rect;
@@ -178,6 +180,7 @@
     int dbits, kbits, kshift;
     int part_passes;
     size_t g_dhist;
+    size_t g_shjac;
     const uint32_t *dhist_ptr;
     size_t i_order;
 };
@@ -193,7 +196,7 @@
     bool prefer_regions;
     const uint32_t *tile_order;
 };
-void compute_layout(int P, int64_t I, int W, int H, Layout *L);
+void compute_layout(int P, int64_t I, int W, int H, Layout *L, bool shjac = false);
 
 struct EmitArgs {
     unsigned long long *status;
diff --git a/das3r_amd/csrc/preprocess.hip b/das3r_amd/csrc/preprocess.hip
--- a/das3r_amd/csrc/preprocess.hip
+++ b/das3r_amd/csrc/preprocess.hip
@@ -20,7 +20,8 @@
     uint32_t *__restrict__ dhist ,
     uint32_t dhist_mask ,
     uint32_t *__restrict__ dhist_next ,
-    const PreXform pre ) {
+    const PreXform pre ,
+    float *__restrict__ shjac ) {
     const int gidx = blockIdx.x * blockDim.x + threadIdx.x;
     bool sampled = false;
     if (dhist != nullptr) {
@@ -95,6 +96,7 @@
     float4 xy_out = make_float4(0.f, 0.f, -1e30f, -1e30f);
     float4 co_out = make_float4(0.f, 0.f, 0.f, 0.f);
     float4 rgbd_out = make_float4(0.f, 0.f, 0.f, 0.f);
+    float jac_out[9] = {0.f, 0.f, 0.f, 0.f, 0.f, 0.f, 0.f, 0.f, 0.f};
     int bx0 = 0, by0 = 0, bx1 = 0, by1 = 0;
 
     const float3 p_view = xform43(p, V);
@@ -143,8 +145,13 @@
                         }
                     }
                     col = sh_regs_to_rgb(D, sh, p, campos, clamp_out);
+                    if (shjac != nullptr) sh_ddir_regs(D, sh, p, campos, jac_out);
                 } else if (HAS_SH) {
-                    col = sh_to_rgb(D, M, shs + (size_t)idx * M * 3, p, campos, clamp_out);
+                    float sh[48];
+                    const float *row = shs + (size_t)idx * M * 3;
+                    load_sh_row(row, D, sh_vec_ok(row, D, M), sh);
+                    col = sh_regs_to_rgb(D, sh, p, campos, clamp_out);
+                    if (shjac != nullptr) sh_ddir_regs(D, sh, p, campos, jac_out);
                 } else {
                     col = make_float3(colors_precomp[3 * idx], colors_precomp[3 * idx + 1], colors_precomp[3 * idx + 2]);
                 }
@@ -173,6 +180,10 @@
     tiles_touched[idx] = tiles_out;
     rect32[idx] = tiles_out ? ((uint32_t)bx0 | ((uint32_t)bx1 << 8) | ((uint32_t)by0 << 16) | ((uint32_t)by1 << 24)) : 0u;
     clamped[idx] = clamp_out;
+    if (HAS_SH && shjac != nullptr) {
+#pragma unroll
+        for (int j = 0; j < 9; j++) shjac[(size_t)j * P + idx] = jac_out[j];
+    }
     }
     {
         __syncthreads();
@@ -334,13 +345,14 @@
     while ((grid.x >> __builtin_popcount(dhist_mask)) > 512u) dhist_mask = (dhist_mask << 1) | 1u;
     const bool has_sh = in->shs != nullptr, has_cov = in->cov3D_precomp != nullptr;
     const PreXform pre = pre_xform(in);
+    float *const shjac = has_sh && L.g_shjac ? (float *)(geom + L.g_shjac) : nullptr;
 #define ARGS                                                                                                              \
     P, a->sh_degree, a->M, in->means3D, in->scales, a->scale_modifier, in->rotations, in->opacities, in->shs,             \
         in->cov3D_precomp, in->colors_precomp, a->viewmatrix, a->projmatrix, a->campos, a->image_width, a->image_height,  \
         a->tanfovx, a->tanfovy, L.tiles_x, L.tiles_y, radii, (uint32_t *)(geom + L.g_keyA), (float4 *)(geom + L.pub.xy),  \
         (float4 *)(geom + L.pub.conic_opacity), (float4 *)(geom + L.pub.rgbd), (uint8_t *)(geom + L.pub.clamped),         \
         (uint32_t *)(geom + L.pub.tiles_touched), (uint32_t *)(geom + L.g_rect), (use_tight_rect() ? 1 : 0) | (a->prefiltered ? 2 : 0), (uint32_t *)(geom + L.g_ghist), (uint32_t)(L.g_ctrl_bytes / 4),                 \
-        (uint32_t *)(img + L.pub.ranges), (uint32_t)(2 * L.ntiles), (uint32_t *)binning_ctrl, (uint32_t)(binning_ctrl_bytes / 4), arrive, host_out, tag, em, dhist, dhist_mask, dhist_next, pre
+        (uint32_t *)(img + L.pub.ranges), (uint32_t)(2 * L.ntiles), (uint32_t *)binning_ctrl, (uint32_t)(binning_ctrl_bytes / 4), arrive, host_out, tag, em, dhist, dhist_mask, dhist_next, pre, shjac
     const bool stage = has_sh && a->M == 16 && a->sh_degree >= 2 && ((uintptr_t)in->shs & 15) == 0 && !switches().no_sh_stage;
     if (has_sh && !has_cov && stage) DAS3R_LAUNCH((preprocess_kernel<true, false, true>), grid, block, 0, s, ARGS);
     else if (has_sh && has_cov && stage) DAS3R_LAUNCH((preprocess_kernel<true, true, true>), grid, block, 0, s, ARGS);
diff --git a/das3r_amd/csrc/preprocess_bwd.hip b/das3r_amd/csrc/preprocess_bwd.hip
--- a/das3r_amd/csrc/preprocess_bwd.hip
+++ b/das3r_amd/csrc/preprocess_bwd.hip
@@ -36,32 +36,6 @@
     }
 }
 
-#define SH_DDIR(SHC, dRdx, dRdy, dRdz)                                                                                          \
-    do {                                                                                                                        \
-        dRdx = 0.f; dRdy = 0.f; dRdz = 0.f;                                                                                     \
-        if (D > 0) {                                                                                                            \
-            dRdx = -SH_C1 * SHC(3);                                                                                             \
-            dRdy = -SH_C1 * SHC(1);                                                                                             \
-            dRdz = SH_C1 * SHC(2);                                                                                              \
-            if (D > 1) {                                                                                                        \
-                dRdx += SH_C2_0 * y * SHC(4) + SH_C2_2 * 2.f * -x * SHC(6) + SH_C2_3 * z * SHC(7) + SH_C2_4 * 2.f * x * SHC(8); \
-                dRdy += SH_C2_0 * x * SHC(4) + SH_C2_1 * z * SHC(5) + SH_C2_2 * 2.f * -y * SHC(6) + SH_C2_4 * 2.f * -y * SHC(8); \
-                dRdz += SH_C2_1 * y * SHC(5) + SH_C2_2 * 2.f * 2.f * z * SHC(6) + SH_C2_3 * x * SHC(7);                       \
-                if (D > 2) {                                                                                                    \
-                    dRdx += SH_C3_0 * SHC(9) * 3.f * 2.f * xy + SH_C3_1 * SHC(10) * yz + SH_C3_2 * SHC(11) * -2.f * xy +       \
-                            SH_C3_3 * SHC(12) * -3.f * 2.f * xz + SH_C3_4 * SHC(13) * (-3.f * xx + 4.f * zz - yy) +            \
-                            SH_C3_5 * SHC(14) * 2.f * xz + SH_C3_6 * SHC(15) * 3.f * (xx - yy);                                \
-                    dRdy += SH_C3_0 * SHC(9) * 3.f * (xx - yy) + SH_C3_1 * SHC(10) * xz +                                      \
-                            SH_C3_2 * SHC(11) * (-3.f * yy + 4.f * zz - xx) + SH_C3_3 * SHC(12) * -3.f * 2.f * yz +            \
-                            SH_C3_4 * SHC(13) * -2.f * xy + SH_C3_5 * SHC(14) * -2.f * yz + SH_C3_6 * SHC(15) * -3.f * 2.f * xy; \
-                    dRdz += SH_C3_1 * SHC(10) * xy + SH_C3_2 * SHC(11) * 4.f * 2.f * yz +                                      \
-                            SH_C3_3 * SHC(12) * 3.f * (2.f * zz - xx - yy) + SH_C3_4 * SHC(13) * 4.f * 2.f * xz +              \
-                            SH_C3_5 * SHC(14) * (xx - yy);                                                                      \
-                }                                                                                                               \
-            }                                                                                                                   \
-        }                                                                                                                       \
-    } while (0)
-
 template <int K>
 __device__ __forceinline__ void wave_store_rows(float *__restrict__ dst , const int rows_valid, const float (&v)[K],
                                                 float *scratch , const int lane) {
@@ -77,13 +51,14 @@
     __builtin_amdgcn_fence(__ATOMIC_ACQ_REL, "workgroup");
 }
 
+constexpr int JAC_WAVES = 5;
 struct ChainArgs {
     GeometryAdam A;
     float *g_conf_flat, *g_small, *det_partials;
     uint32_t *arrived;
 };
-template <bool HAS_SH, bool HAS_COV, bool STAGE_IN, bool STAGE_OUT, bool DEG0 = false, bool CHAIN = false, bool DEPTH = false>
-__global__ void __launch_bounds__(256, DEG0 ? (CHAIN ? 4 : 6) : 3) preprocess_backward_kernel(
+template <bool HAS_SH, bool HAS_COV, bool STAGE_IN, bool STAGE_OUT, bool DEG0 = false, bool CHAIN = false, bool DEPTH = false, bool JAC = false>
+__global__ void __launch_bounds__(256, DEG0 ? (CHAIN ? 4 : 6) : JAC && !CHAIN ? JAC_WAVES : 3) preprocess_backward_kernel(
     int P, int D_in, int M, const float *__restrict__ means3D, const float *__restrict__ scales, float scale_modifier,
     const float *__restrict__ rotations, const float *__restrict__ shs, const float *__restrict__ cov3D_precomp,
     const float *__restrict__ viewmatrix, const float *__restrict__ projmatrix, const float *__restrict__ campos, int W, int H,
@@ -94,7 +69,7 @@
     float *__restrict__ dL_dcolors_precomp , float *__restrict__ dL_dmeans3D,
     float *__restrict__ dL_dscales, float *__restrict__ dL_drot, float *__restrict__ dL_dsh, float *__restrict__ dL_dcov3D,
     const PreXform pre ,
-    const ChainArgs ch , const float *__restrict__ dz_g
+    const ChainArgs ch , const float *__restrict__ dz_g , const float *__restrict__ shjac
 #ifdef DAS3R_EXPERIMENTS
     , unsigned long long *__restrict__ trace
 #endif
@@ -103,7 +78,9 @@
     constexpr unsigned long long *trace = nullptr;
 #endif
     BLK_STAMP(trace, 6, 0)
-    __shared__ float4 sh_lds[(STAGE_IN || STAGE_OUT) ? 256 * 13 : 1];
+    static_assert(!(JAC && (STAGE_IN || DEG0)), "JAC replaces the SH row at degree >= 2");
+    constexpr int LDS_ROWS = JAC ? 128 : 256;
+    __shared__ float4 sh_lds[(STAGE_IN || STAGE_OUT) ? LDS_ROWS * 13 : 1];
     const int idx = blockIdx.x * blockDim.x + threadIdx.x;
     const int D = DEG0 ? 0 : D_in;
     const int ic = idx < P ? idx : P - 1;
@@ -112,6 +89,9 @@
     float3 mean_in, sc_in = make_float3(0.f, 0.f, 0.f);
     float4 q_in = make_float4(0.f, 0.f, 0.f, 0.f);
     float c3_in[6] = {0.f, 0.f, 0.f, 0.f, 0.f, 0.f};
+    float jac[JAC ? 9 : 1];
+#pragma unroll
+    for (int j = 0; j < (JAC ? 9 : 0); j++) jac[j] = shjac[(size_t)j * P + ic];
     float raw_x = 0.f, raw_y = 0.f, raw_z = 0.f, raw_s0 = 0.f, raw_s1 = 0.f, raw_s2 = 0.f, raw_o = 0.f, raw_c = 0.f;
     float4 raw_q = make_float4(0.f, 0.f, 0.f, 0.f);
     long long raw_ci = 0;
@@ -145,7 +125,8 @@
     const size_t blk4 = (size_t)blockIdx.x * 256 * 12;
     const size_t limit4 = (size_t)P * 12 > blk4 ? (size_t)P * 12 - blk4 : 0;
     constexpr bool LDS_GATHER = STAGE_OUT;
-    constexpr int CHUNK_ROWS = 1020;
+    constexpr int CHUNK_ROWS = JAC ? 738 : 1020;
+    constexpr int CHUNK_LOADS = JAC ? 7 : 9;
     float acc[9];
 #pragma unroll
     for (int q = 0; q < 9; q++) acc[q] = 0.f;
@@ -198,15 +179,15 @@
                 head = (int)((reinterpret_cast<uintptr_t>(src) & 15u) >> 2);
                 const float4 *src4 = reinterpret_cast<const float4 *>(src - head);
                 const int n4 = (head + n9 + 3) >> 2;
-                float4 w[9];
-#pragma unroll
-                for (int i = 0; i < 9; i++) {
+                float4 w[CHUNK_LOADS];
+#pragma unroll
+                for (int i = 0; i < CHUNK_LOADS; i++) {
                     const int f = i * 256 + (int)threadIdx.x;
                     w[i] = src4[f < n4 ? f : n4 - 1];
                 }
                 if (!sh_requested) request_sh();
 #pragma unroll
-                for (int i = 0; i < 9; i++) {
+                for (int i = 0; i < CHUNK_LOADS; i++) {
                     const int f = i * 256 + (int)threadIdx.x;
                     if (f < n4) buf4[f] = w[i];
                 }
@@ -251,6 +232,9 @@
     float o_col[3] = {0.f, 0.f, 0.f}, o_sh0[3] = {0.f, 0.f, 0.f};
     static_assert(!CHAIN || (XPOSE && HAS_SH && !HAS_COV), "the chained backward: unstaged SH layouts, scales + rotations");
     float o_rot[4] = {0.f, 0.f, 0.f, 0.f}, o_op = 0.f;
+    constexpr bool HALVES = JAC && STAGE_OUT;
+    float h_dir[3] = {0.f, 0.f, 0.f}, h_g[3] = {0.f, 0.f, 0.f};
+    int h_nk = 0;
 
     if (idx < P) {
         const bool visible = ntiles_g > 0;
@@ -393,9 +377,17 @@
 #pragma unroll
                 for (int c = 0; c < 3; c++) g[c] = ((cl >> c) & 1) ? 0.f : acc[c];
                 sh_basis(D, x, y, z, basis);
+                if (HALVES) h_dir[0] = x, h_dir[1] = y, h_dir[2] = z;
                 float ddir[3] = {0.f, 0.f, 0.f};
                 if (D > 0) {
-                    if (STAGE_IN) {
+                    if (JAC) {
+#pragma unroll
+                        for (int c = 0; c < 3; c++) {
+                            ddir[0] += jac[3 * c] * g[c];
+                            ddir[1] += jac[3 * c + 1] * g[c];
+                            ddir[2] += jac[3 * c + 2] * g[c];
+                        }
+                    } else if (STAGE_IN) {
                         float shl[48];
 #pragma unroll
                         for (int i = 0; i < 12; i++) {
@@ -494,7 +486,11 @@
         } else if (!HAS_COV) reinterpret_cast<float4 *>(dL_drot)[idx] = make_float4(drot[0], drot[1], drot[2], drot[3]);
         if (HAS_SH) {
             const int nk = visible ? (D + 1) * (D + 1) : 0;
-            if (STAGE_OUT) {
+            if (HALVES) {
+#pragma unroll
+                for (int c = 0; c < 3; c++) h_g[c] = g[c];
+                h_nk = nk;
+            } else if (STAGE_OUT) {
 #pragma unroll
                 for (int i = 0; i < 12; i++) {
                     float o[4];
@@ -530,7 +526,34 @@
         else if (M == 1) wave_store_rows<3>(dL_dsh + 3 * (size_t)wave_first, rows_valid, o_sh0, xp, lane);
     }
     BLK_STAMP(trace, 6, 5)
-    if (STAGE_OUT) {
+    if (HALVES) {
+        float4 *dst = reinterpret_cast<float4 *>(dL_dsh) + blk4;
+#pragma unroll
+        for (int h = 0; h < 2; h++) {
+            if (h) __syncthreads();
+            if ((int)(threadIdx.x >> 7) == h && idx < P) {
+                float h_basis[16];
+                sh_basis(D, h_dir[0], h_dir[1], h_dir[2], h_basis);
+#pragma unroll
+                for (int i = 0; i < 12; i++) {
+                    float o[4];
+#pragma unroll
+                    for (int e = 0; e < 4; e++) {
+                        const int f = 4 * i + e, k = f / 3, c = f - 3 * k;
+                        o[e] = k < h_nk ? h_basis[k] * h_g[c] : 0.f;
+                    }
+                    sh_lds[(threadIdx.x & 127) * 13 + i] = make_float4(o[0], o[1], o[2], o[3]);
+                }
+            }
+            __syncthreads();
+            const size_t base = (size_t)h * 128 * 12;
+#pragma unroll
+            for (int i = 0; i < 6; i++) {
+                const int f = i * 256 + threadIdx.x;
+                if (base + f < limit4) dst[base + f] = sh_lds[(f / 12) * 13 + (f % 12)];
+            }
+        }
+    } else if (STAGE_OUT) {
         __syncthreads();
         float4 *dst = reinterpret_cast<float4 *>(dL_dsh) + blk4;
 #pragma unroll
@@ -610,7 +633,8 @@
     const size_t cap_rows = L.capacity > 0 ? (size_t)L.capacity : 1;
     const uint8_t *exists = quad_rows ? reinterpret_cast<const uint8_t *>(partial) + align_up(cap_rows * 4 * 12 * sizeof(float)) : nullptr;
     const bool stage_out = has_sh && a->M == 16 && ((uintptr_t)g->dL_dshs & 15) == 0 && !nostage;
-    const bool stage_in = stage_out && a->sh_degree >= 2 && ((uintptr_t)in->shs & 15) == 0;
+    const bool jac = has_sh && L.g_shjac != 0;
+    const bool stage_in = stage_out && a->sh_degree >= 2 && ((uintptr_t)in->shs & 15) == 0 && !jac;
 #ifdef DAS3R_EXPERIMENTS
 #define PB_TRACE_ARG , wg_trace()
 #else
@@ -622,7 +646,7 @@
         a->viewmatrix, a->projmatrix, a->campos, a->image_width, a->image_height, a->tanfovx, a->tanfovy,                    \
         (const uint32_t *)(geom + L.pub.tiles_touched), (const uint8_t *)(geom + L.pub.clamped), partial, exists,        \
         (const uint32_t *)(geom + L.g_off_by_gid), g->dL_dmeans2D, g->dL_dopacities, g->dL_dcolors_precomp, g->dL_dmeans3D,  \
-        g->dL_dscales, g->dL_drotations, g->dL_dshs, g->dL_dcov3D, pre, ch, dz PB_TRACE_ARG
+        g->dL_dscales, g->dL_drotations, g->dL_dshs, g->dL_dcov3D, pre, ch, dz, jac ? (const float *)(geom + L.g_shjac) : nullptr PB_TRACE_ARG
     ChainArgs ch;
     memset(&ch, 0, sizeof(ch));
     if (g->chain) {
@@ -648,17 +672,27 @@
         ch.g_conf_flat = c->g_conf_flat; ch.g_small = c->g_small;
         ch.det_partials = chain_scratch(s, (size_t)grid.x, &ch.arrived);
     }
-#define LAUNCH6(SH, COV, SI, SO, D0, CH)                                                                             \
-    do {                                                                                                             \
-        if (dz) DAS3R_LAUNCH((preprocess_backward_kernel<SH, COV, SI, SO, D0, CH, true>), grid, block, 0, s, ARGS); \
-        else DAS3R_LAUNCH((preprocess_backward_kernel<SH, COV, SI, SO, D0, CH>), grid, block, 0, s, ARGS);          \
+#define LAUNCH7(SH, COV, SI, SO, D0, CH, J)                                                                                \
+    do {                                                                                                                   \
+        if (dz) DAS3R_LAUNCH((preprocess_backward_kernel<SH, COV, SI, SO, D0, CH, true, J>), grid, block, 0, s, ARGS);    \
+        else DAS3R_LAUNCH((preprocess_backward_kernel<SH, COV, SI, SO, D0, CH, false, J>), grid, block, 0, s, ARGS);      \
     } while (0)
+#define LAUNCH6(SH, COV, SI, SO, D0, CH) LAUNCH7(SH, COV, SI, SO, D0, CH, false)
 #define LAUNCH(SH, COV, SI, SO) LAUNCH6(SH, COV, SI, SO, false, false)
 #define LAUNCH0(SH, COV) LAUNCH6(SH, COV, false, false, true, false)
     const bool deg0 = a->sh_degree == 0 && !stage_out;
     if (g->chain) {
         if (deg0) LAUNCH6(true, false, false, false, true, true);
+        else if (jac) LAUNCH7(true, false, false, false, false, true, true);
         else LAUNCH6(true, false, false, false, false, true);
+    } else if (jac) {
+        if (has_cov) {
+            if (stage_out) LAUNCH7(true, true, false, true, false, false, true);
+            else LAUNCH7(true, true, false, false, false, false, true);
+        } else {
+            if (stage_out) LAUNCH7(true, false, false, true, false, false, true);
+            else LAUNCH7(true, false, false, false, false, false, true);
+        }
     } else if (has_sh && !has_cov) {
         if (stage_in) LAUNCH(true, false, true, true);
         else if (stage_out) LAUNCH(true, false, false, true);
@@ -677,6 +711,7 @@
 #undef LAUNCH
 #undef LAUNCH0
 #undef LAUNCH6
+#undef LAUNCH7
 #undef ARGS
     KERNEL_CHECK(s, a->debug, "preprocess_backward");
     return DAS3R_OK;
diff --git a/das3r_amd/csrc/splat_math.h b/das3r_amd/csrc/splat_math.h
--- a/das3r_amd/csrc/splat_math.h
+++ b/das3r_amd/csrc/splat_math.h
@@ -146,6 +146,32 @@
     return make_float3(out[0], out[1], out[2]);
 }
 
+#define SH_DDIR(SHC, dRdx, dRdy, dRdz)                                                                                          \
+    do {                                                                                                                        \
+        dRdx = 0.f; dRdy = 0.f; dRdz = 0.f;                                                                                     \
+        if (D > 0) {                                                                                                            \
+            dRdx = -SH_C1 * SHC(3);                                                                                             \
+            dRdy = -SH_C1 * SHC(1);                                                                                             \
+            dRdz = SH_C1 * SHC(2);                                                                                              \
+            if (D > 1) {                                                                                                        \
+                dRdx += SH_C2_0 * y * SHC(4) + SH_C2_2 * 2.f * -x * SHC(6) + SH_C2_3 * z * SHC(7) + SH_C2_4 * 2.f * x * SHC(8); \
+                dRdy += SH_C2_0 * x * SHC(4) + SH_C2_1 * z * SHC(5) + SH_C2_2 * 2.f * -y * SHC(6) + SH_C2_4 * 2.f * -y * SHC(8); \
+                dRdz += SH_C2_1 * y * SHC(5) + SH_C2_2 * 2.f * 2.f * z * SHC(6) + SH_C2_3 * x * SHC(7);                       \
+                if (D > 2) {                                                                                                    \
+                    dRdx += SH_C3_0 * SHC(9) * 3.f * 2.f * xy + SH_C3_1 * SHC(10) * yz + SH_C3_2 * SHC(11) * -2.f * xy +       \
+                            SH_C3_3 * SHC(12) * -3.f * 2.f * xz + SH_C3_4 * SHC(13) * (-3.f * xx + 4.f * zz - yy) +            \
+                            SH_C3_5 * SHC(14) * 2.f * xz + SH_C3_6 * SHC(15) * 3.f * (xx - yy);                                \
+                    dRdy += SH_C3_0 * SHC(9) * 3.f * (xx - yy) + SH_C3_1 * SHC(10) * xz +                                      \
+                            SH_C3_2 * SHC(11) * (-3.f * yy + 4.f * zz - xx) + SH_C3_3 * SHC(12) * -3.f * 2.f * yz +            \
+                            SH_C3_4 * SHC(13) * -2.f * xy + SH_C3_5 * SHC(14) * -2.f * yz + SH_C3_6 * SHC(15) * -3.f * 2.f * xy; \
+                    dRdz += SH_C3_1 * SHC(10) * xy + SH_C3_2 * SHC(11) * 4.f * 2.f * yz +                                      \
+                            SH_C3_3 * SHC(12) * 3.f * (2.f * zz - xx - yy) + SH_C3_4 * SHC(13) * 4.f * 2.f * xz +              \
+                            SH_C3_5 * SHC(14) * (xx - yy);                                                                      \
+                }                                                                                                               \
+            }                                                                                                                   \
+        }                                                                                                                       \
+    } while (0)
+
 __device__ __forceinline__ bool sh_vec_ok(const float *row, const int D, const int M) {
     const int n3 = 3 * (D + 1) * (D + 1);
     return (((uintptr_t)row & 15) == 0) && (((n3 + 3) & ~3) <= 3 * M);
@@ -160,15 +186,17 @@
     return make_float3(fmaxf(r.x, 0.f), fmaxf(r.y, 0.f), fmaxf(r.z, 0.f));
 }
 
-__device__ __forceinline__ float3 sh_to_rgb(const int D, const int M, const float *__restrict__ row, const float3 p,
-                                            const float *campos, uint8_t &clamp_bits) {
-    float sh[48];
-    load_sh_row(row, D, sh_vec_ok(row, D, M), sh);
+__device__ __forceinline__ void sh_ddir_regs(const int D, const float sh[48], const float3 p, const float *campos, float J[9]) {
     const float dx = p.x - campos[0], dy = p.y - campos[1], dz = p.z - campos[2];
     const float inv = 1.f / sqrtf(dx * dx + dy * dy + dz * dz);
-    const float3 r = sh_eval(D, sh, dx * inv, dy * inv, dz * inv);
-    clamp_bits = (uint8_t)((r.x < 0.f ? 1 : 0) | (r.y < 0.f ? 2 : 0) | (r.z < 0.f ? 4 : 0));
-    return make_float3(fmaxf(r.x, 0.f), fmaxf(r.y, 0.f), fmaxf(r.z, 0.f));
-}
-
-}
+    const float x = dx * inv, y = dy * inv, z = dz * inv;
+    const float xx = x * x, yy = y * y, zz = z * z, xy = x * y, yz = y * z, xz = x * z;
+#pragma unroll
+    for (int c = 0; c < 3; c++) {
+#define SHC_REG(k) sh[(k) * 3 + c]
+        SH_DDIR(SHC_REG, J[3 * c], J[3 * c + 1], J[3 * c + 2]);
+#undef SHC_REG
+    }
+}
+
+}
diff --git a/das3r_amd/offline.py b/das3r_amd/offline.py
--- a/das3r_amd/offline.py
+++ b/das3r_amd/offline.py
@@ -108,7 +108,7 @@
     pre.conf_flat, pre.mask_index = conf.data_ptr(), None
     pre.R, pre.t, pre.Lq = st.mats.data_ptr(), st.mats.data_ptr() + 36, st.mats.data_ptr() + 48
     rs = _settings(view, model, pipe, background, 1.0, dev)
-    res = _forward_full(rs, xyz, st.packed_sh(model), st.e, op, sc, rot, st.e, pre=pre, invdepth=invdepth)
+    res = _forward_full(rs, xyz, st.packed_sh(model), st.e, op, sc, rot, st.e, pre=pre, invdepth=invdepth, no_backward=True)
     check_forward(res[6], dev)
     return (res[1], res[2], res[7]) if invdepth else (res[1], res[2])
 
diff --git a/das3r_amd/rasterizer.py b/das3r_amd/rasterizer.py
--- a/das3r_amd/rasterizer.py
+++ b/das3r_amd/rasterizer.py
@@ -167,7 +167,8 @@
     return _forward_full(rs, means3D, sh, colors_precomp, opacities, scales, rotations, cov3Ds_precomp, exact=True)[:6]
 
 
-def _forward_full(rs, means3D, sh, colors_precomp, opacities, scales, rotations, cov3Ds_precomp, exact=False, pre=None, invdepth=False):
+def _forward_full(rs, means3D, sh, colors_precomp, opacities, scales, rotations, cov3Ds_precomp, exact=False, pre=None, invdepth=False,
+                  no_backward=False):
     lib = _lib.load()
     device = means3D.device
     if device.type != "cuda":
@@ -199,6 +200,7 @@
     inv = torch.empty(1, H, W, dtype=torch.float32, device=device) if invdepth else None
     o.out_invdepth = _ptr(inv)
     saved = _lib.RasterSaved()
+    saved.flags = _lib.NO_BACKWARD_IN_FLAG if no_backward else 0
     with _on_device(device):
         rc = lib.das3r_raster_forward(C.byref(a), C.byref(i), C.byref(o), alloc.fns["geom"], alloc.fns["binning"],
                                       alloc.fns["img"], None, C.byref(saved), _stream(device))
@@ -289,11 +291,18 @@
 
 
 def rasterize_gaussians(means3D, means2D, sh, colors_precomp, opacities, scales, rotations, cov3Ds_precomp, raster_settings):
-    return _RasterizeGaussians.apply(means3D, means2D, sh, colors_precomp, opacities, scales, rotations, cov3Ds_precomp,
-                                     raster_settings)
+    return _apply(_RasterizeGaussians, means3D, means2D, sh, colors_precomp, opacities, scales, rotations, cov3Ds_precomp, raster_settings)
 
 
 _last = threading.local()
+
+
+def _apply(fn, *args):
+    _last.no_backward = not (torch.is_grad_enabled() and any(torch.is_tensor(t) and t.requires_grad for t in args))
+    try:
+        return fn.apply(*args)
+    finally:
+        _last.no_backward = False
 
 
 class _RasterizeGaussians(torch.autograd.Function):
@@ -312,16 +321,17 @@
         rotations = _prep(rotations, device, "rotations")
         cov3Ds_precomp = _prep(cov3Ds_precomp, device, "cov3D_precomp")
         args = (raster_settings, means3D, sh, colors_precomp, opacities, scales, rotations, cov3Ds_precomp)
+        no_backward = getattr(_last, "no_backward", False)
         if raster_settings.debug:
             cpu_args = cpu_deep_copy_tuple(args)
             try:
-                res = _forward_full(*args, invdepth=invdepth)
+                res = _forward_full(*args, invdepth=invdepth, no_backward=no_backward)
             except Exception as ex:
                 torch.save(cpu_args, "snapshot_fw.dump")
                 print("\nAn error occured in forward. Please forward snapshot_fw.dump for debugging.")
                 raise ex
         else:
-            res = _forward_full(*args, invdepth=invdepth)
+            res = _forward_full(*args, invdepth=invdepth, no_backward=no_backward)
         num_rendered, color, radii, geomBuffer, binningBuffer, imgBuffer, capacity = res[:7]
         ctx.raster_settings = raster_settings
         ctx.num_rendered = num_rendered
@@ -416,8 +426,8 @@
             cov3D_precomp = e
         _last.capacity = None
         if return_invdepth:
-            color, radii, invdepth = _RasterizeGaussiansInvDepth.apply(means3D, means2D, shs, colors_precomp, opacities, scales, rotations,
-                                                                       cov3D_precomp, raster_settings)
+            color, radii, invdepth = _apply(_RasterizeGaussiansInvDepth, means3D, means2D, shs, colors_precomp, opacities, scales, rotations,
+                                            cov3D_precomp, raster_settings)
         else:
             color, radii = rasterize_gaussians(means3D, means2D, shs, colors_precomp, opacities, scales, rotations, cov3D_precomp,
                                                raster_settings)
```

Measured after the change: 1147 Msplats/s (median of 6 runs). 1.04x the previous value.
